# ctu-vras/pcl-augmentation

Hardware: NVIDIA B200
Metric: augmented scans/sec (120k-pt KITTI scan, placement + occlusion + insertion) (higher is better)
Workload: dtype f64

## Files before the change

### pcl_augmentation_b200/csrc/r3d_common.cuh

```cuda
#pragma once
#include <cuda_runtime.h>
#include <stdint.h>

#define R3D_EMPTY_U64 0xFFFFFFFFFFFFFFFFull
#define R3D_MAX_CLASSES 16
#define R3D_MAX_SURFACE 8
#define R3D_NUM_RADII 50

namespace r3d {

constexpr double kPi = 3.141592653589793;
constexpr double kTwoPi = 6.283185307179586;
constexpr double kEmptyRange = 500.0;

__device__ __forceinline__ double mul(double a, double b) { return __dmul_rn(a, b); }
__device__ __forceinline__ double add(double a, double b) { return __dadd_rn(a, b); }
__device__ __forceinline__ double sub(double a, double b) { return __dsub_rn(a, b); }

__device__ __forceinline__ double range3(double x, double y, double z) {
    return sqrt(add(add(mul(x, x), mul(y, y)), mul(z, z)));
}
__device__ __forceinline__ double azimuth(double x, double y) { return add(atan2(y, x), kPi); }
__device__ __forceinline__ double elevation(double z, double r) { return acos(__ddiv_rn(z, r)); }

__device__ __forceinline__ double az_mod(double az) { return az >= kTwoPi ? sub(az, kTwoPi) : az; }

struct ImageGeom {
    int rows, cols;
    int pix_stride;
    double min_el, max_el;
    double d_el, d_az;
};

__host__ __device__ __forceinline__ ImageGeom make_geom(int rows, int cols, int pix_stride, double max_el, double min_el) {
    ImageGeom g;
    g.rows = rows; g.cols = cols; g.pix_stride = pix_stride;
    g.min_el = min_el; g.max_el = max_el;
    g.d_el = (max_el - min_el) / (double)rows;
    g.d_az = kTwoPi / (double)cols;
    return g;
}

__device__ __forceinline__ int trunc_to_int(double v) {
    if (!(v > -2147483000.0 && v < 2147483000.0)) return INT_MIN;
    return (int)v;
}
__device__ __forceinline__ int bin_row(const ImageGeom& g, double el) {
    return trunc_to_int(__ddiv_rn(sub(sub(el, g.min_el), 0.00001), g.d_el));
}
__device__ __forceinline__ int bin_col(const ImageGeom& g, double az) {
    return trunc_to_int(__ddiv_rn(az_mod(az), g.d_az));
}

struct FastGeom { float inv_d_az, inv_d_el, el0, err_az, err_el; };
__device__ __forceinline__ FastGeom make_fast_geom(const ImageGeom& g) {
    FastGeom f;
    f.inv_d_az = (float)(1.0 / g.d_az); f.inv_d_el = (float)(1.0 / g.d_el);
    f.el0 = (float)(g.min_el + 0.00001);
    f.err_az = 6e-6f * f.inv_d_az + 5e-7f * (float)g.cols + 1e-5f;
    f.err_el = 6e-6f * f.inv_d_el + 5e-7f * (float)g.rows + 1e-5f;
    if (!(f.err_az < 0.25f)) f.err_az = 2.0f;
    if (!(f.err_el < 0.25f)) f.err_el = 2.0f;
    return f;
}
__device__ __forceinline__ bool fast_bin(float t, float err, int nbins, int& bin) {
    const float f = floorf(t), fr = t - f;
    if (!(fr > err && fr < 1.0f - err && t > err && t < (float)nbins - err)) return false;
    bin = (int)f;
    return true;
}
__device__ __forceinline__ bool fast_col(float inv_d_az, float err_az, int cols, float x, float y, int& col) {
    return fast_bin((atan2f(y, x) + 3.14159274f) * inv_d_az, err_az, cols, col);
}
__device__ __forceinline__ bool fast_row(const FastGeom& f, int rows, float z, float r, int& row) {
    const float t = z / r;
    if (!(fabsf(t) <= 0.9f)) return false;
    return fast_bin((acosf(t) - f.el0) * f.inv_d_el, f.err_el, rows, row);
}

struct Box {
    double cx, cy, cz;
    double m[9];
    double length, width, height;
    double reach;
};

struct BoxTest {
    double c0x, c0y, c0z, hi0, lo0;
    double c1x, c1y, c1z, hi1, lo1;
    double c2x, c2y, c2z, hi2, lo2;
};

__device__ __forceinline__ BoxTest make_box_test(const Box& b) {
    BoxTest t;
    const double* m = b.m;
    t.c0x = m[0]; t.c0y = m[3]; t.c0z = m[6];
    t.c1x = m[1]; t.c1y = m[4]; t.c1z = m[7];
    t.c2x = m[2]; t.c2y = m[5]; t.c2z = m[8];
    const double L = b.length, W = b.width, H = b.height;
    t.hi0 = add(add(mul(t.c0x, add(b.cx, __ddiv_rn(mul(t.c0x, L), 2.0))), mul(t.c0y, add(b.cy, __ddiv_rn(mul(t.c0y, L), 2.0)))),
                mul(t.c0z, add(b.cz, __ddiv_rn(mul(t.c0z, L), 2.0))));
    t.lo0 = add(add(mul(t.c0x, sub(b.cx, __ddiv_rn(mul(t.c0x, L), 2.0))), mul(t.c0y, sub(b.cy, __ddiv_rn(mul(t.c0y, L), 2.0)))),
                mul(t.c0z, sub(b.cz, __ddiv_rn(mul(t.c0z, L), 2.0))));
    t.hi1 = add(add(mul(t.c1x, add(b.cx, __ddiv_rn(mul(t.c1x, W), 2.0))), mul(t.c1y, add(b.cy, __ddiv_rn(mul(t.c1y, W), 2.0)))),
                mul(t.c1z, add(b.cz, __ddiv_rn(mul(t.c1z, W), 2.0))));
    t.lo1 = add(add(mul(t.c1x, sub(b.cx, __ddiv_rn(mul(t.c1x, W), 2.0))), mul(t.c1y, sub(b.cy, __ddiv_rn(mul(t.c1y, W), 2.0)))),
                mul(t.c1z, sub(b.cz, __ddiv_rn(mul(t.c1z, W), 2.0))));
    t.hi2 = add(add(mul(t.c2x, add(b.cx, mul(t.c2x, H))), mul(t.c2y, add(b.cy, mul(t.c2y, H)))),
                mul(t.c2z, add(b.cz, mul(t.c2z, H))));
    t.lo2 = add(add(mul(t.c2x, sub(b.cx, mul(t.c2x, 0.0))), mul(t.c2y, sub(b.cy, mul(t.c2y, 0.0)))),
                mul(t.c2z, sub(b.cz, mul(t.c2z, 0.0))));
    return t;
}

__device__ __forceinline__ bool inside_box(const BoxTest& t, double x, double y, double z) {
    const double a0 = add(add(mul(t.c0x, x), mul(t.c0y, y)), mul(t.c0z, z));
    if (!(a0 < t.hi0) || !(a0 > t.lo0)) return false;
    const double a1 = add(add(mul(t.c1x, x), mul(t.c1y, y)), mul(t.c1z, z));
    if (!(a1 < t.hi1) || !(a1 > t.lo1)) return false;
    const double a2 = add(add(mul(t.c2x, x), mul(t.c2y, y)), mul(t.c2z, z));
    return (a2 < t.hi2) && (a2 > t.lo2);
}

struct YawBox {
    double cx, cy;
    double m00, m10;
    double m01;
};

__device__ __forceinline__ YawBox make_yaw_box(double c0x, double c0y, double a, double b, double c, double s) {
    YawBox y;
    y.cx = sub(mul(c, c0x), mul(s, c0y));
    y.cy = add(mul(s, c0x), mul(c, c0y));
    y.m00 = sub(mul(a, c), mul(b, s));
    y.m10 = add(mul(b, c), mul(a, s));
    y.m01 = -add(mul(a, s), mul(b, c));
    return y;
}

__device__ __forceinline__ Box yaw_box_to_box(const YawBox& y, double cz, double L, double W, double H) {
    Box b;
    b.cx = y.cx; b.cy = y.cy; b.cz = cz;
    b.m[0] = y.m00; b.m[1] = y.m01; b.m[2] = 0.0;
    b.m[3] = y.m10; b.m[4] = y.m00; b.m[5] = 0.0;
    b.m[6] = 0.0;   b.m[7] = 0.0;   b.m[8] = 1.0;
    b.length = L; b.width = W; b.height = H; b.reach = 0.0;
    return b;
}

__device__ __forceinline__ unsigned long long dbl_bits(double v) { return (unsigned long long)__double_as_longlong(v); }
__device__ __forceinline__ double bits_dbl(unsigned long long b) { return __longlong_as_double((long long)b); }

__device__ __forceinline__ float4 ldg_f4(const float4* p) { return __ldg(p); }

}
```

### pcl_augmentation_b200/csrc/r3d_engine.cu

```cuda
#include "r3d_engine_kernels.cuh"
#include "r3d_host.h"
#include "r3d_resident.h"

#include <cmath>
#include <chrono>
#include <cstdlib>
#include <thread>
#include <cstring>
#include <map>
#include <string>
#include <vector>

using namespace r3d;

#define R3D_MAX_SUB 16

namespace {

enum KernelId {
    KID_INGEST, KID_CTRL, KID_UPDATE, KID_CLEAR, KID_PROJECT, KID_CLOSEFILL, KID_ADJUST, KID_ONMAP, KID_HEIGHT, KID_COLLIDE,
    KID_GRID, KID_OCCL, KID_SELECT, KID_OUT, KID_MINMAX, KID_PROJECT0, KID_CLOSEFILL0, KID_CLEAR0, KID_MINMAX0, KID_WALK, KID_PREP, KID_SCATTER,
    KID_COUNT
};
const char* kKernelNames[KID_COUNT] = {
    "ingest_spherical", "ctrl", "update_mask_patch", "clear_images", "project_zbuffer", "close_fill", "adjust_map",
    "onmap", "road_level", "collide", "index_build", "occlusion_count", "select_emit", "compact_output", "minmax_elevation",
    "project_zbuffer_full", "close_fill_full", "clear_images_full", "minmax_elevation_full",
    "scan_walk", "walk_prepare",
    "scatter_project"};

template <class T>
struct DevBuf {
    T* p = nullptr;
    size_t n = 0;
    int alloc(size_t count) {
        release();
        n = count;
        if (count == 0) return R3D_OK;
        cudaError_t err = cudaMalloc((void**)&p, count * sizeof(T));
        if (err != cudaSuccess) { p = nullptr; return r3d_fail_cuda(err, "cudaMalloc"); }
        return R3D_OK;
    }
    void release() { if (p) cudaFree(p); p = nullptr; n = 0; }
    ~DevBuf() { release(); }
};

}

struct r3d_engine {
    r3d_engine_cfg cfg;
    EngineDev dev;
    cudaStream_t stream = nullptr;
    int n_scans = 0;
    int max_n0 = 0;
    int n_sms = 148;
    int device = 0;
    int n_sub = 4;
    cudaStream_t sub_stream[R3D_MAX_SUB] = {nullptr};
    cudaEvent_t sub_done[R3D_MAX_SUB] = {nullptr};
    cudaEvent_t ev_armed = nullptr;
    cudaEvent_t ev_wait = nullptr;
    struct Sub { int b0, n, round; bool done; long long left; unsigned seq_base; EngineDev d; cudaStream_t st; };
    Sub sub[R3D_MAX_SUB];
    struct RoundGraph { cudaGraphExec_t exec = nullptr; EngineDev d; int ns = 0, chunks_all = 0, task_ctas = 0, sel_pts = 0, kernels = 0; };
    RoundGraph round_graph[R3D_MAX_SUB];
    bool use_graphs = true, capturing = false;
    bool fresh = false;
    bool walked = false;
    bool staged = false;
    bool run_active = false;
    int run_nsub = 0, run_done = 0, run_rounds = 0;
    bool objects_set = false, yaw_set = false, batch_loaded = false, ran = false;
    int last_rounds = 0;
    DevBuf<float4> xyzi, out_xyzi, gpts, apts;
    DevBuf<unsigned long long> sel_keys;
    DevBuf<double> sel_r, tail_x, tail_y, tail_z, r, el, smooth, poses, obj_x, obj_y, obj_z, cos_k, sin_k, radii_sq, cand_level,
        inserted_box;
    DevBuf<float> tail_i, obj_i, check, out_check;
    DevBuf<unsigned> label, dmask, vmask, occ_win, unplaceable, obj_label, out_label, tickets;
    DevBuf<unsigned short> col, cand_list, label16, out_label16;
    DevBuf<unsigned char> label1;
    DevBuf<long long> pt_off;
    DevBuf<int> chunk_cnt, pix, gate_update, gate_try, gate_apply, gate_full, gate_patch, cf_rect, col_off, col_idx, acell, active_count, far_arr, od_map_dims, counts, perms, class_list_off,
        class_list, radii_ok, cand_v, gcell, n_list, feas, occ_pix, sel_pix, inserted, n0_arr, nbox0_arr, work_cnt, full_list, cf_tasks, need2, occ_far;
    DevBuf<unsigned> occ_cnt;
    DevBuf<unsigned> round_ctl;
    DevBuf<unsigned char> alive, od_maps, ss_map, cand_flags, gnear, gscratch;
    DevBuf<unsigned long long> zraw, obj_raw, stats;
    DevBuf<long long> od_map_off, out_count, out_off, check_off;
    DevBuf<ScanState> st;
    DevBuf<Box> boxes, boxes0;
    DevBuf<BoxTest> box_tests;
    DevBuf<ObjBox> obj, try_obj;
    DevBuf<ClassCfg> classes;
    CUtensorMap zraw_tmap;
    bool zraw_tmap_ok = false;
    std::vector<Box> h_boxes;
    std::vector<int> h_nbox0;
    unsigned long long* h_words = nullptr;
    unsigned long long* d_words = nullptr;
    unsigned seq = 0;
    long long* h_offsets = nullptr;
    SchedulePolicy policy;
    bool policy_set = false;
    int* h_idx = nullptr;
    cudaEvent_t ev_idx = nullptr;
    DevBuf<int> idx_dev, n_ins_dev;
    DevBuf<float> box7;
    bool from_store = false;
    std::vector<int> batch_idx;
    r3d_world_aug world_pol;
    bool world_on = false, world_loaded = false;
    DevBuf<float> world;
    DevBuf<float> obj_dims3;
    DevBuf<int> class_target;
    const int* kept_src = nullptr;
    std::vector<int> kept;
    bool profile = false;
    double prof_ms[KID_COUNT] = {0};
    int64_t prof_launches[KID_COUNT] = {0};
    std::vector<std::pair<int, std::pair<cudaEvent_t, cudaEvent_t>>> pending_events;
    std::vector<cudaEvent_t> event_pool;
};

namespace {

__global__ void k_box_tests(const Box* boxes, BoxTest* tests, int n) {
    const int i = blockIdx.x * blockDim.x + threadIdx.x;
    if (i < n) tests[i] = make_box_test(boxes[i]);
}
__global__ void k_widen_labels(const unsigned short* src, const long long* pt_off, unsigned* label, int P, int n_scans) {
    const int b = blockIdx.y;
    if (b >= n_scans) return;
    const long long o = pt_off[b] - pt_off[0];
    const int cnt = (int)(pt_off[b + 1] - pt_off[b]);
    const int p0 = blockIdx.x * CHUNK;
    for (int p = p0 + threadIdx.x; p < min(p0 + CHUNK, cnt); p += blockDim.x) label[(size_t)b * P + p] = src[o + p];
}
__global__ void k_expand_label_bits(const unsigned char* bits, const long long* pt_off, unsigned* label, int P, int n_scans,
                                    unsigned road_label) {
    const int b = blockIdx.y;
    if (b >= n_scans) return;
    const long long o = pt_off[b] - pt_off[0];
    const int cnt = (int)(pt_off[b + 1] - pt_off[b]);
    const int p0 = blockIdx.x * CHUNK;
    const unsigned other = road_label == 1u ? 2u : 1u;
    for (int p = p0 + threadIdx.x; p < min(p0 + CHUNK, cnt); p += blockDim.x) {
        const long long i = o + p;
        label[(size_t)b * P + p] = ((bits[i >> 3] >> (i & 7)) & 1u) ? road_label : other;
    }
}
__global__ void k_narrow_labels(const unsigned* src, unsigned short* dst, long long n) {
    for (long long i = blockIdx.x * (long long)blockDim.x + threadIdx.x; i < n; i += (long long)gridDim.x * blockDim.x) dst[i] = (unsigned short)src[i];
}
__global__ void k_set_round(unsigned* round_ctl, unsigned seq_base) { round_ctl[0] = 0u; round_ctl[1] = seq_base; }
__global__ void k_fill_u64(unsigned long long* p, size_t n, unsigned long long v) {
    for (size_t i = blockIdx.x * (size_t)blockDim.x + threadIdx.x; i < n; i += (size_t)gridDim.x * blockDim.x) p[i] = v;
}

struct Launcher {
    r3d_engine* eng;
    int kid;
    cudaStream_t st;
    cudaEvent_t a = nullptr, b = nullptr;
    Launcher(r3d_engine* e, int k, cudaStream_t stream = nullptr) : eng(e), kid(k), st(stream ? stream : e->stream) {
        if (eng->profile) {
            a = get_event(); b = get_event();
            cudaEventRecord(a, st);
        }
    }
    cudaEvent_t get_event() {
        if (!eng->event_pool.empty()) { cudaEvent_t ev = eng->event_pool.back(); eng->event_pool.pop_back(); return ev; }
        cudaEvent_t ev; cudaEventCreate(&ev); return ev;
    }
    ~Launcher() {
        if (eng->capturing) return;
        r3d_count_launch();
        eng->prof_launches[kid] += 1;
        if (eng->profile) {
            cudaEventRecord(b, st);
            eng->pending_events.push_back({kid, {a, b}});
        }
    }
};

void drain_events(r3d_engine* eng) {
    for (auto& pe : eng->pending_events) {
        float ms = 0.f;
        cudaEventSynchronize(pe.second.second);
        cudaEventElapsedTime(&ms, pe.second.first, pe.second.second);
        eng->prof_ms[pe.first] += ms;
        eng->event_pool.push_back(pe.second.first);
        eng->event_pool.push_back(pe.second.second);
    }
    eng->pending_events.clear();
}

size_t occl_smem_bytes(const EngineDev& d) { return (size_t)d.dwords * sizeof(unsigned) + (size_t)(d.K + 2) * sizeof(unsigned short); }
constexpr int SEL_SMEM_PTS = 4096;
int next_pow2(int v) { int p = 1; while (p < v) p <<= 1; return p; }
size_t select_smem_bytes(int max_pts) {
    return (size_t)next_pow2(max_pts) * 8 + (size_t)max_pts * 8 + (size_t)SEL_TILE_PX * 8 + (size_t)max_pts * 4 +
           2 * (size_t)(SEL_TILE_PX / 32) * 4 + 16;
}

}

#define TRY(x) do { int _rc = (x); if (_rc != R3D_OK) return _rc; } while (0)

static cudaError_t engine_wait(r3d_engine* eng) {
    if (!eng->ev_wait) {
        cudaError_t e = cudaEventCreateWithFlags(&eng->ev_wait, cudaEventBlockingSync | cudaEventDisableTiming);
        if (e != cudaSuccess) return e;
    }
    cudaError_t e = cudaEventRecord(eng->ev_wait, eng->stream);
    if (e != cudaSuccess) return e;
    return cudaEventSynchronize(eng->ev_wait);
}

typedef CUresult (*EncodeTiledFn)(CUtensorMap*, CUtensorMapDataType, cuuint32_t, void*, const cuuint64_t*, const cuuint64_t*,
                                  const cuuint32_t*, const cuuint32_t*, CUtensorMapInterleave, CUtensorMapSwizzle,
                                  CUtensorMapL2promotion, CUtensorMapFloatOOBfill);
static bool make_zraw_tensor_map(CUtensorMap* tm, void* base, int W, int H, int B) {
    if (getenv("R3D_NO_TMA") || (W & 1) || ((uintptr_t)base & 15)) return false;
    void* fn = nullptr;
    cudaDriverEntryPointQueryResult q;
    if (cudaGetDriverEntryPoint("cuTensorMapEncodeTiled", &fn, cudaEnableDefault, &q) != cudaSuccess || q != cudaDriverEntryPointSuccess || !fn) {
        cudaGetLastError();
        return false;
    }
    const cuuint64_t dims[3] = {(cuuint64_t)W, (cuuint64_t)H, (cuuint64_t)B};
    const cuuint64_t strides[2] = {(cuuint64_t)W * 8, (cuuint64_t)W * H * 8};
    const cuuint32_t box[3] = {(cuuint32_t)CF_SW, (cuuint32_t)CF_SH, 1u};
    const cuuint32_t estr[3] = {1u, 1u, 1u};
    return ((EncodeTiledFn)fn)(tm, CU_TENSOR_MAP_DATA_TYPE_UINT64, 3, base, dims, strides, box, estr, CU_TENSOR_MAP_INTERLEAVE_NONE,
                               CU_TENSOR_MAP_SWIZZLE_NONE, CU_TENSOR_MAP_L2_PROMOTION_NONE, CU_TENSOR_MAP_FLOAT_OOB_FILL_NONE) == CUDA_SUCCESS;
}

extern "C" int r3d_engine_create(const r3d_engine_cfg* cfg, r3d_engine** out) {
    if (!cfg || !out) return r3d_fail(R3D_ERR_ARG, "r3d_engine_create: null argument");
    if (cfg->rows <= 0 || cfg->cols <= 0 || cfg->cols > 65535 || cfg->yaw_steps <= 0 || cfg->n_classes <= 0 ||
        cfg->n_classes > R3D_MAX_CLASSES || cfg->max_scans <= 0 || cfg->max_points <= 0 || cfg->max_inserted <= 0 ||
        cfg->max_tries <= 0 || cfg->max_events <= 0 || cfg->max_boxes <= 0 || (cfg->task != 0 && cfg->task != 1))
        return r3d_fail(R3D_ERR_ARG, "r3d_engine_create: bad configuration");
    if (cfg->task == 1 && (cfg->map_window <= 0 || cfg->map_window % 32 != 0))
        return r3d_fail(R3D_ERR_ARG, "r3d_engine_create: map_window must be a positive multiple of 32");
    int count = 0;
    if (cudaGetDeviceCount(&count) != cudaSuccess || count == 0)
        return r3d_fail(R3D_ERR_CUDA, "r3d_engine_create: no CUDA device (this library has no CPU fallback)");
    r3d_engine* eng = new r3d_engine();
    eng->cfg = *cfg;
    R3D_CUDA(cudaGetDevice(&eng->device));
    int prio_least = 0, prio_greatest = 0;
    R3D_CUDA(cudaDeviceGetStreamPriorityRange(&prio_least, &prio_greatest));
    R3D_CUDA(cudaStreamCreateWithPriority(&eng->stream, cudaStreamNonBlocking, prio_least));
    eng->n_sub = (cfg->flags >> 8) & 31;
    eng->use_graphs = !(cfg->flags & 2);
    eng->staged = (cfg->flags & 8) != 0;
    if (const char* env = getenv("R3D_STAGED")) eng->staged = atoi(env) != 0;
    if (const char* env = getenv("R3D_GRAPHS")) eng->use_graphs = atoi(env) != 0;
    if (const char* env = getenv("R3D_SUBBATCHES")) eng->n_sub = atoi(env);
    if (eng->n_sub <= 0) eng->n_sub = 4;
    eng->n_sub = std::min(eng->n_sub, R3D_MAX_SUB);
    for (int i = 0; i < R3D_MAX_SUB; ++i) {
        R3D_CUDA(cudaStreamCreateWithPriority(&eng->sub_stream[i], cudaStreamNonBlocking, prio_greatest));
        R3D_CUDA(cudaEventCreateWithFlags(&eng->sub_done[i], cudaEventDisableTiming));
    }
    R3D_CUDA(cudaEventCreateWithFlags(&eng->ev_armed, cudaEventDisableTiming));
    EngineDev& d = eng->dev;
    memset(&d, 0, sizeof(d));
    d.task = cfg->task; d.rows = cfg->rows; d.cols = cfg->cols; d.hw = cfg->rows * cfg->cols; d.K = cfg->yaw_steps;
    d.max_tries = cfg->max_tries; d.n_classes = cfg->n_classes; d.B = cfg->max_scans; d.max_points = cfg->max_points;
    d.max_inserted = cfg->max_inserted + (16 - (cfg->max_points + cfg->max_inserted) % 16) % 16;
    d.P = cfg->max_points + d.max_inserted; d.max_boxes = cfg->max_boxes;
    d.max_events = cfg->max_events; d.road_label = cfg->road_label; d.n_road_indexes = cfg->n_road_indexes;
    d.map_window = cfg->task == 1 ? cfg->map_window : 32; d.dwords = (d.hw + 31) / 32;
    for (int i = 0; i < R3D_MAX_SURFACE; ++i) d.road_indexes[i] = cfg->road_indexes[i];
    d.step_rad = 2.0 * 3.14159265358979323846 / (double)cfg->yaw_steps;
    d.grid_cell = cfg->grid_cell > 0 ? cfg->grid_cell : 0.5;
    d.grid_inv_cell = (float)(1.0 / d.grid_cell);
    d.G = 2 * (cfg->grid_half > 0 ? cfg->grid_half : 200);
    d.force_full = (cfg->flags & 1) ? 1 : 0;
    const size_t B = d.B, P = d.P, K1 = d.K + 1, HW = d.hw;
    TRY(eng->xyzi.alloc(B * d.max_points)); TRY(eng->tail_x.alloc(B * d.max_inserted)); TRY(eng->tail_y.alloc(B * d.max_inserted));
    TRY(eng->tail_z.alloc(B * d.max_inserted)); TRY(eng->tail_i.alloc(B * d.max_inserted)); TRY(eng->label.alloc(B * P));
    TRY(eng->r.alloc(B * P)); TRY(eng->el.alloc(B * P)); TRY(eng->col.alloc(B * P)); TRY(eng->pix.alloc(B * P));
    TRY(eng->alive.alloc(B * P)); TRY(eng->zraw.alloc(B * HW)); TRY(eng->obj_raw.alloc(B * HW)); TRY(eng->smooth.alloc(B * HW));
    eng->zraw_tmap_ok = make_zraw_tensor_map(&eng->zraw_tmap, eng->zraw.p, d.cols, d.rows, (int)B);
    TRY(eng->dmask.alloc(B * d.dwords)); TRY(eng->vmask.alloc(B * d.dwords)); TRY(eng->st.alloc(B));
    TRY(eng->gate_update.alloc(B)); TRY(eng->gate_try.alloc(B)); TRY(eng->gate_apply.alloc(B)); TRY(eng->gate_full.alloc(B));
    TRY(eng->gate_patch.alloc(B)); TRY(eng->cf_rect.alloc(B * 4)); TRY(eng->active_count.alloc(R3D_MAX_SUB * 64 * 2));
    TRY(eng->round_ctl.alloc(R3D_MAX_SUB * 32));
    d.cf_tiles_x = (d.cols + CF_TW - 1) / CF_TW;
    d.cf_tiles = d.cf_tiles_x * ((d.rows + CF_TH - 1) / CF_TH);
    TRY(eng->work_cnt.alloc(B * 4)); TRY(eng->full_list.alloc(B)); TRY(eng->cf_tasks.alloc(B * (size_t)d.cf_tiles));
    R3D_CUDA(cudaMemset(eng->work_cnt.p, 0, B * 4 * sizeof(int)));
    TRY(eng->need2.alloc(B));
    R3D_CUDA(cudaMemset(eng->need2.p, 0, B * sizeof(int)));
    d.cand_window = (cfg->flags & 4) ? 0 : 48;
    if (const char* env = getenv("R3D_WINDOW")) d.cand_window = std::max(0, atoi(env));
    if (d.task != 0) d.cand_window = 0;
    TRY(eng->far_arr.alloc(B)); TRY(eng->boxes.alloc(B * d.max_boxes)); TRY(eng->box_tests.alloc(B * d.max_boxes));
    TRY(eng->boxes0.alloc(B * d.max_boxes));
    TRY(eng->poses.alloc(B * 16)); TRY(eng->occ_win.alloc(B * ((size_t)d.map_window * d.map_window / 32)));
    TRY(eng->counts.alloc(B * d.n_classes)); TRY(eng->cos_k.alloc(K1)); TRY(eng->sin_k.alloc(K1));
    TRY(eng->radii_sq.alloc(R3D_NUM_RADII)); TRY(eng->radii_ok.alloc(R3D_NUM_RADII)); TRY(eng->classes.alloc(R3D_MAX_CLASSES));
    TRY(eng->cand_flags.alloc(B * K1)); TRY(eng->cand_level.alloc(B * K1)); TRY(eng->cand_v.alloc(B * K1));
    TRY(eng->cand_list.alloc(B * K1)); TRY(eng->n_list.alloc(B)); TRY(eng->tickets.alloc(B * 4));
    R3D_CUDA(cudaMemset(eng->tickets.p, 0, B * 4 * sizeof(unsigned)));
    TRY(eng->feas.alloc(B * d.K)); TRY(eng->inserted.alloc(B * d.max_events * 4)); TRY(eng->inserted_box.alloc(B * d.max_events * 8));
    TRY(eng->check.alloc(B * d.max_inserted * 5)); TRY(eng->out_count.alloc(B)); TRY(eng->out_off.alloc(B + 1));
    TRY(eng->check_off.alloc(B + 1)); TRY(eng->out_xyzi.alloc(B * P)); TRY(eng->out_label.alloc(B * P));
    TRY(eng->out_check.alloc(B * d.max_inserted * 5)); TRY(eng->n0_arr.alloc(B)); TRY(eng->nbox0_arr.alloc(B));
    TRY(eng->gcell.alloc(B * (size_t)d.G * d.G)); TRY(eng->gpts.alloc(B * d.max_points));
    TRY(eng->gnear.alloc(B * (size_t)d.G * d.G)); TRY(eng->gscratch.alloc(B * (size_t)d.G * d.G));
    TRY(eng->col_off.alloc(B * (size_t)(d.cols + 1))); TRY(eng->col_idx.alloc(B * d.max_points));
    TRY(eng->acell.alloc(B * (size_t)d.G * d.G)); TRY(eng->apts.alloc(B * d.max_points));
    TRY(eng->try_obj.alloc(B));
    d.max_chunks = (d.P + CHUNK - 1) / CHUNK;
    TRY(eng->chunk_cnt.alloc(B * (size_t)d.max_chunks));
    { int dev = 0; cudaGetDevice(&dev); cudaDeviceGetAttribute(&eng->n_sms, cudaDevAttrMultiProcessorCount, dev); }
    TRY(eng->od_map_off.alloc(B * 2 + 1)); TRY(eng->od_map_dims.alloc(B * 8)); TRY(eng->stats.alloc(R3D_N_STATS));
    R3D_CUDA(cudaMemset(eng->stats.p, 0, R3D_N_STATS * sizeof(unsigned long long)));
    TRY(eng->occ_far.alloc(B * (OCC_FAR_CAP + 1)));
    if (cfg->task == 1) TRY(eng->occ_cnt.alloc(B * (size_t)d.map_window * d.map_window));
    R3D_CUDA(cudaMemset(eng->occ_far.p, 0xFF, B * (OCC_FAR_CAP + 1) * sizeof(int)));
    R3D_CUDA(cudaHostAlloc((void**)&eng->h_words, R3D_MAX_SUB * 64 * sizeof(unsigned long long), cudaHostAllocMapped));
    memset(eng->h_words, 0, R3D_MAX_SUB * 64 * sizeof(unsigned long long));
    R3D_CUDA(cudaHostGetDevicePointer((void**)&eng->d_words, eng->h_words, 0));
    R3D_CUDA(cudaMallocHost((void**)&eng->h_offsets, (2 * (B + 1) + 1) * sizeof(long long)));
    std::vector<ClassCfg> cls(R3D_MAX_CLASSES);
    for (int c = 0; c < R3D_MAX_CLASSES; ++c) {
        const r3d_class_cfg& s = cfg->classes[c];
        cls[c].min_points = s.min_points; cls[c].map_sel = s.map_sel; cls[c].map_ok_mask = s.map_ok_mask;
        cls[c].pedestrian = s.pedestrian; cls[c].n_surface = std::min(std::max(s.n_surface, 0), R3D_MAX_SURFACE);
        for (int i = 0; i < R3D_MAX_SURFACE; ++i) cls[c].surface[i] = s.surface[i];
        cls[c].ok_slots = 0u;
    }
    d.n_surf_all = 0;
    for (int c = 0; c < cfg->n_classes; ++c)
        for (int i = 0; i < cls[c].n_surface; ++i) {
            int slot = -1;
            for (int j = 0; j < d.n_surf_all; ++j) if (d.surf_all[j] == cls[c].surface[i]) slot = j;
            if (slot < 0) {
                if (d.n_surf_all >= 15) return r3d_fail(R3D_ERR_CAPACITY, "r3d_engine_create: more than 15 distinct surface labels");
                slot = d.n_surf_all; d.surf_all[d.n_surf_all++] = cls[c].surface[i];
            }
            cls[c].ok_slots |= 1u << slot;
        }
    if (d.max_points + d.max_inserted > (1 << APT_IDX_BITS)) return r3d_fail(R3D_ERR_CAPACITY, "r3d_engine_create: more than 2^27 points per scan");
    R3D_CUDA(cudaMemcpy(eng->classes.p, cls.data(), cls.size() * sizeof(ClassCfg), cudaMemcpyHostToDevice));
    R3D_CUDA(cudaMemcpy(eng->radii_sq.p, cfg->radii_sq, sizeof(cfg->radii_sq), cudaMemcpyHostToDevice));
    R3D_CUDA(cudaMemcpy(eng->radii_ok.p, cfg->radii_ok, sizeof(cfg->radii_ok), cudaMemcpyHostToDevice));
    k_fill_u64<<<148 * 4, 256, 0, eng->stream>>>(eng->obj_raw.p, B * HW, R3D_EMPTY_U64); r3d_count_launch();
    R3D_CUDA(cudaMemsetAsync(eng->dmask.p, 0, B * d.dwords * sizeof(unsigned), eng->stream));
    R3D_CUDA(cudaStreamSynchronize(eng->stream));
    d.xyzi = eng->xyzi.p; d.tail_x = eng->tail_x.p; d.tail_y = eng->tail_y.p; d.tail_z = eng->tail_z.p; d.tail_i = eng->tail_i.p;
    d.label = eng->label.p; d.r = eng->r.p; d.el = eng->el.p; d.col = eng->col.p; d.pix = eng->pix.p; d.alive = eng->alive.p;
    d.zraw = eng->zraw.p; d.obj_raw = eng->obj_raw.p; d.smooth = eng->smooth.p; d.dmask = eng->dmask.p; d.vmask = eng->vmask.p;
    d.st = eng->st.p; d.gate_update = eng->gate_update.p; d.gate_try = eng->gate_try.p; d.gate_apply = eng->gate_apply.p;
    d.gate_full = eng->gate_full.p; d.gate_patch = eng->gate_patch.p; d.cf_rect = eng->cf_rect.p;
    d.work_cnt = eng->work_cnt.p; d.full_list = eng->full_list.p; d.cf_tasks = eng->cf_tasks.p; d.need2 = eng->need2.p;
    d.active_count = eng->active_count.p; d.far_arr = eng->far_arr.p; d.boxes = eng->boxes.p; d.box_tests = eng->box_tests.p;
    d.poses = eng->poses.p; d.occ_win = eng->occ_win.p; d.counts = eng->counts.p; d.cos_k = eng->cos_k.p; d.sin_k = eng->sin_k.p;
    d.radii_sq = eng->radii_sq.p; d.radii_ok = eng->radii_ok.p; d.classes = eng->classes.p; d.cand_flags = eng->cand_flags.p;
    d.cand_level = eng->cand_level.p; d.cand_list = eng->cand_list.p; d.n_list = eng->n_list.p; d.tickets = eng->tickets.p;
    d.cand_v = eng->cand_v.p; d.feas = eng->feas.p; d.inserted = eng->inserted.p; d.inserted_box = eng->inserted_box.p;
    d.check = eng->check.p; d.out_count = eng->out_count.p; d.out_off = eng->out_off.p; d.check_off = eng->check_off.p;
    d.out_xyzi = eng->out_xyzi.p; d.out_label = eng->out_label.p; d.out_check = eng->out_check.p;
    d.gcell = eng->gcell.p; d.gpts = eng->gpts.p; d.gnear = eng->gnear.p; d.gscratch = eng->gscratch.p;
    d.col_off = eng->col_off.p; d.col_idx = eng->col_idx.p; d.acell = eng->acell.p; d.apts = eng->apts.p;
    d.try_obj = eng->try_obj.p; d.chunk_cnt = eng->chunk_cnt.p;
    d.od_map_off = eng->od_map_off.p; d.od_map_dims = eng->od_map_dims.p; d.stats = eng->stats.p; d.occ_far = eng->occ_far.p; d.occ_cnt = eng->occ_cnt.p;
    *out = eng;
    return R3D_OK;
}

extern "C" int r3d_engine_destroy(r3d_engine* eng) {
    if (eng) cudaSetDevice(eng->device);
    if (!eng) return R3D_OK;
    cudaStreamSynchronize(eng->stream);
    drain_events(eng);
    for (cudaEvent_t ev : eng->event_pool) cudaEventDestroy(ev);
    if (eng->h_words) cudaFreeHost(eng->h_words);
    if (eng->h_offsets) cudaFreeHost(eng->h_offsets);
    for (int i = 0; i < R3D_MAX_SUB; ++i) {
        if (eng->sub_stream[i]) { cudaStreamSynchronize(eng->sub_stream[i]); cudaStreamDestroy(eng->sub_stream[i]); }
        if (eng->sub_done[i]) cudaEventDestroy(eng->sub_done[i]);
    }
    if (eng->ev_armed) cudaEventDestroy(eng->ev_armed);
    if (eng->ev_wait) cudaEventDestroy(eng->ev_wait);
    if (eng->ev_idx) cudaEventDestroy(eng->ev_idx);
    if (eng->h_idx) cudaFreeHost(eng->h_idx);
    for (int i = 0; i < R3D_MAX_SUB; ++i) if (eng->round_graph[i].exec) cudaGraphExecDestroy(eng->round_graph[i].exec);
    cudaStreamDestroy(eng->stream);
    delete eng;
    return R3D_OK;
}

extern "C" int r3d_engine_set_yaw_tables(r3d_engine* eng, const double* cos_k, const double* sin_k) {
    if (eng) cudaSetDevice(eng->device);
    if (!eng || !cos_k || !sin_k) return r3d_fail(R3D_ERR_ARG, "r3d_engine_set_yaw_tables: null argument");
    const size_t n = (size_t)eng->dev.K + 1;
    R3D_CUDA(cudaMemcpy(eng->cos_k.p, cos_k, n * sizeof(double), cudaMemcpyHostToDevice));
    R3D_CUDA(cudaMemcpy(eng->sin_k.p, sin_k, n * sizeof(double), cudaMemcpyHostToDevice));
    eng->yaw_set = true;
    return R3D_OK;
}

extern "C" int r3d_engine_set_objects(r3d_engine* eng, const r3d_object_db* db) {
    if (eng) cudaSetDevice(eng->device);
    if (!eng || !db || db->n_objects <= 0) return r3d_fail(R3D_ERR_ARG, "r3d_engine_set_objects: bad argument");
    EngineDev& d = eng->dev;
    const int n = db->n_objects;
    const int64_t total = db->point_offsets[n];
    std::vector<double> x(total), y(total), z(total);
    std::vector<float> in(total);
    std::vector<unsigned> lab(total);
    for (int64_t i = 0; i < total; ++i) {
        const double* p = db->points5 + i * 5;
        x[i] = p[0]; y[i] = p[1]; z[i] = p[2]; in[i] = (float)p[3]; lab[i] = (unsigned)p[4];
    }
    std::vector<ObjBox> ob(n);
    int max_pts = 1;
    for (int o = 0; o < n; ++o) {
        const double* bx = db->boxes + (size_t)o * 8;
        ObjBox& t = ob[o];
        t.cx = bx[0]; t.cy = bx[1]; t.cz = bx[2]; t.a = bx[3]; t.b = bx[4];
        t.length = bx[5]; t.width = bx[6]; t.height = bx[7];
        t.rho = std::hypot(t.cx, t.cy); t.psi0 = std::atan2(t.cy, t.cx);
        t.reach = 0.5 * std::hypot(t.length, t.width) + 0.05;
        t.cls = db->class_index[o];
        t.first = (int)db->point_offsets[o]; t.count = (int)(db->point_offsets[o + 1] - db->point_offsets[o]);
        t.pad = 0;
        t.eu0 = t.ev0 = t.ez0 = 1e300; t.eu1 = t.ev1 = t.ez1 = -1e300;
        for (int i = t.first; i < t.first + t.count; ++i) {
            const double dx = x[i] - t.cx, dy = y[i] - t.cy;
            const double u = dx * t.a + dy * t.b, v = -dx * t.b + dy * t.a, w = z[i] - t.cz;
            t.eu0 = std::min(t.eu0, u); t.eu1 = std::max(t.eu1, u); t.ev0 = std::min(t.ev0, v); t.ev1 = std::max(t.ev1, v);
            t.ez0 = std::min(t.ez0, w); t.ez1 = std::max(t.ez1, w);
        }
        t.eu0 -= 1e-6; t.ev0 -= 1e-6; t.ez0 -= 1e-6; t.eu1 += 1e-6; t.ev1 += 1e-6; t.ez1 += 1e-6;
        if (t.cls < 0 || t.cls >= d.n_classes) return r3d_fail(R3D_ERR_ARG, "r3d_engine_set_objects: class index out of range");
        max_pts = std::max(max_pts, t.count);
    }
    if (max_pts > 32768) return r3d_fail(R3D_ERR_CAPACITY, "r3d_engine_set_objects: a cut object has more than 32768 points");
    d.max_obj_points = max_pts; d.n_objects = n;
    TRY(eng->obj_x.alloc(total)); TRY(eng->obj_y.alloc(total)); TRY(eng->obj_z.alloc(total)); TRY(eng->obj_i.alloc(total));
    TRY(eng->obj_label.alloc(total)); TRY(eng->obj.alloc(n)); TRY(eng->class_list_off.alloc(d.n_classes + 1));
    const int nl = db->class_list_offsets[d.n_classes];
    TRY(eng->class_list.alloc(std::max(nl, 1)));
    TRY(eng->unplaceable.alloc((size_t)d.B * ((n + 31) / 32)));
    TRY(eng->occ_pix.alloc((size_t)d.B * OCC_G * max_pts)); TRY(eng->sel_pix.alloc((size_t)d.B * max_pts));
    R3D_CUDA(cudaMemcpy(eng->obj_x.p, x.data(), total * sizeof(double), cudaMemcpyHostToDevice));
    R3D_CUDA(cudaMemcpy(eng->obj_y.p, y.data(), total * sizeof(double), cudaMemcpyHostToDevice));
    R3D_CUDA(cudaMemcpy(eng->obj_z.p, z.data(), total * sizeof(double), cudaMemcpyHostToDevice));
    R3D_CUDA(cudaMemcpy(eng->obj_i.p, in.data(), total * sizeof(float), cudaMemcpyHostToDevice));
    R3D_CUDA(cudaMemcpy(eng->obj_label.p, lab.data(), total * sizeof(unsigned), cudaMemcpyHostToDevice));
    R3D_CUDA(cudaMemcpy(eng->obj.p, ob.data(), n * sizeof(ObjBox), cudaMemcpyHostToDevice));
    R3D_CUDA(cudaMemcpy(eng->class_list_off.p, db->class_list_offsets, (d.n_classes + 1) * sizeof(int), cudaMemcpyHostToDevice));
    R3D_CUDA(cudaMemcpy(eng->class_list.p, db->class_list, nl * sizeof(int), cudaMemcpyHostToDevice));
    d.obj_x = eng->obj_x.p; d.obj_y = eng->obj_y.p; d.obj_z = eng->obj_z.p; d.obj_i = eng->obj_i.p; d.obj_label = eng->obj_label.p;
    d.obj = eng->obj.p; d.class_list_off = eng->class_list_off.p; d.class_list = eng->class_list.p;
    d.unplaceable = eng->unplaceable.p; d.occ_pix = eng->occ_pix.p; d.sel_pix = eng->sel_pix.p;
    const size_t sel_smem = select_smem_bytes(std::min(max_pts, SEL_SMEM_PTS));
    d.sel_key_cap = next_pow2(max_pts);
    if (max_pts > std::min(SEL_SMEM_PTS, walk_od::WALK_SEL_PTS)) {
        TRY(eng->sel_keys.alloc((size_t)d.B * d.sel_key_cap)); TRY(eng->sel_r.alloc((size_t)d.B * max_pts));
    }
    d.sel_keys = eng->sel_keys.p; d.sel_r = eng->sel_r.p;
    R3D_CUDA(cudaFuncSetAttribute(k_select_emit, cudaFuncAttributeMaxDynamicSharedMemorySize, (int)sel_smem));
    R3D_CUDA(cudaFuncSetAttribute(k_occl_count, cudaFuncAttributeMaxDynamicSharedMemorySize, (int)occl_smem_bytes(d)));
    if (onmap_smem_bytes(d.K) > 100 * 1024) return r3d_fail(R3D_ERR_CAPACITY, "r3d_engine_set_objects: too many yaw steps for the placement kernel's shared memory");
    R3D_CUDA(cudaFuncSetAttribute(k_onmap, cudaFuncAttributeMaxDynamicSharedMemorySize, (int)onmap_smem_bytes(d.K)));
    if (grid_near_smem(d.G) > 200 * 1024) return r3d_fail(R3D_ERR_CAPACITY, "r3d_engine_set_objects: road-level grid too large for shared memory");
    R3D_CUDA(cudaFuncSetAttribute(k_grid_near_bits, cudaFuncAttributeMaxDynamicSharedMemorySize, (int)grid_near_smem(d.G)));
    if (std::max(walk_od::walk_smem_layout(d.K, d.dwords).total, walk_ss::walk_smem_layout(d.K, d.dwords).total) > 200 * 1024)
        return r3d_fail(R3D_ERR_CAPACITY, "r3d_engine_set_objects: range image / yaw steps too large for the walker's shared memory");
    R3D_CUDA(cudaFuncSetAttribute(walk_od::k_scan_walk, cudaFuncAttributeMaxDynamicSharedMemorySize, (int)walk_od::walk_smem_layout(d.K, d.dwords).total));
    R3D_CUDA(cudaFuncSetAttribute(walk_ss::k_scan_walk, cudaFuncAttributeMaxDynamicSharedMemorySize, (int)walk_ss::walk_smem_layout(d.K, d.dwords).total));
    eng->objects_set = true;
    return R3D_OK;
}

extern "C" int r3d_engine_set_ss_map(r3d_engine* eng, const uint8_t* map, int32_t size_x, int32_t size_y, int64_t move_x,
                                     int64_t move_y) {
    if (eng) cudaSetDevice(eng->device);
    if (!eng || !map || size_x <= 0 || size_y <= 0) return r3d_fail(R3D_ERR_ARG, "r3d_engine_set_ss_map: bad argument");
    TRY(eng->ss_map.alloc((size_t)size_x * size_y));
    R3D_CUDA(cudaMemcpy(eng->ss_map.p, map, (size_t)size_x * size_y, cudaMemcpyHostToDevice));
    eng->dev.ss_map = eng->ss_map.p; eng->dev.ss_sx = size_x; eng->dev.ss_sy = size_y;
    eng->dev.ss_move_x = move_x; eng->dev.ss_move_y = move_y;
    return R3D_OK;
}

static int arm_batch(r3d_engine* eng, bool ingest) {
    eng->run_active = false;
    EngineDev& d = eng->dev;
    const int n = eng->n_scans;
    cudaStream_t st = eng->stream;
    k_reset_state<<<(n + 127) / 128, 128, 0, st>>>(d, n, eng->n0_arr.p, eng->nbox0_arr.p); r3d_count_launch();
    R3D_CUDA(cudaMemsetAsync(eng->dmask.p, 0, (size_t)n * d.dwords * sizeof(unsigned), st));
    const int chunks = (eng->max_n0 + CHUNK - 1) / CHUNK;
    if (ingest) {
        R3D_CUDA(cudaMemsetAsync(eng->gcell.p, 0, (size_t)n * d.G * d.G * sizeof(int), st));
        R3D_CUDA(cudaMemsetAsync(eng->col_off.p, 0, (size_t)n * (d.cols + 1) * sizeof(int), st));
        R3D_CUDA(cudaMemsetAsync(eng->acell.p, 0, (size_t)n * d.G * d.G * sizeof(int), st));
        { Launcher l(eng, KID_INGEST); k_ingest_count<<<dim3(chunks, n), STREAM_THREADS, 0, st>>>(d, n); }
        {
            Launcher l(eng, KID_GRID);
            k_bucket_scan3<<<dim3(n, 3), 1024, 0, st>>>(d, n);
        }
        { Launcher l(eng, KID_SCATTER); k_scatter_project<<<dim3(chunks, n), STREAM_THREADS, 0, st>>>(d, n); }
        {
            Launcher l(eng, KID_GRID);
            k_grid_near_bits<<<n, NEAR_THREADS, grid_near_smem(d.G), st>>>(d, n);
        }
        eng->fresh = true;
    } else {
        eng->fresh = false;
        k_reset_alive<<<dim3(std::max(chunks, 1), n), 256, 0, st>>>(d, n); r3d_count_launch();
        const size_t slots = (size_t)n * d.max_boxes;
        R3D_CUDA(cudaMemcpyAsync(eng->boxes.p, eng->boxes0.p, slots * sizeof(Box), cudaMemcpyDeviceToDevice, st));
        k_box_tests<<<(int)((slots + 127) / 128), 128, 0, st>>>(eng->boxes.p, eng->box_tests.p, (int)slots);
        r3d_count_launch();
    }
    eng->ran = false;
    return r3d_check_launch("arm_batch");
}

extern "C" int r3d_engine_load_batch(r3d_engine* eng, const r3d_batch* bt) {
    if (eng) cudaSetDevice(eng->device);
    if (!eng || !bt) return r3d_fail(R3D_ERR_ARG, "r3d_engine_load_batch: null argument");
    if (!eng->objects_set || !eng->yaw_set) return r3d_fail(R3D_ERR_ARG, "r3d_engine_load_batch: set objects and yaw tables first");
    EngineDev& d = eng->dev;
    const int n = bt->n_scans;
    if (n <= 0 || n > d.B) return r3d_fail(R3D_ERR_CAPACITY, "r3d_engine_load_batch: n_scans exceeds max_scans");
    if (!bt->point_offsets || !bt->xyzi || (!bt->labels && !bt->labels16 && !bt->labels1) || !bt->counts || !bt->perms || bt->n_events <= 0)
        return r3d_fail(R3D_ERR_ARG, "r3d_engine_load_batch: missing arrays");
    if (d.task == 1 && (!bt->poses || !d.ss_map)) return r3d_fail(R3D_ERR_ARG, "r3d_engine_load_batch: semseg needs poses and the map");
    if (d.task == 0 && (!bt->maps || !bt->map_offsets || !bt->map_dims)) return r3d_fail(R3D_ERR_ARG, "r3d_engine_load_batch: OD needs maps");
    cudaStream_t st = eng->stream;
    std::vector<int> n0(n), nb(n);
    eng->max_n0 = 0;
    for (int s = 0; s < n; ++s) {
        const int64_t cnt = bt->point_offsets[s + 1] - bt->point_offsets[s];
        if (cnt <= 0 || cnt > d.max_points) return r3d_fail(R3D_ERR_CAPACITY, "r3d_engine_load_batch: scan larger than max_points (or empty)");
        n0[s] = (int)cnt; eng->max_n0 = std::max(eng->max_n0, (int)cnt);
        nb[s] = bt->box_offsets ? bt->box_offsets[s + 1] - bt->box_offsets[s] : 0;
        if (nb[s] > d.max_boxes) return r3d_fail(R3D_ERR_CAPACITY, "r3d_engine_load_batch: too many scene boxes");
    }
    eng->n_scans = n;
    eng->h_boxes.assign((size_t)n * d.max_boxes, Box());
    for (int s = 0; s < n; ++s)
        for (int j = 0; j < nb[s]; ++j) {
            const double* src = bt->boxes + ((size_t)bt->box_offsets[s] + j) * R3D_BOX_DOUBLES;
            Box& b = eng->h_boxes[(size_t)s * d.max_boxes + j];
            b.cx = src[0]; b.cy = src[1]; b.cz = src[2];
            for (int i = 0; i < 9; ++i) b.m[i] = src[3 + i];
            b.length = src[12]; b.width = src[13]; b.height = src[14]; b.reach = src[15];
        }
    eng->h_nbox0 = nb;
    R3D_CUDA(cudaMemcpyAsync(eng->boxes.p, eng->h_boxes.data(), eng->h_boxes.size() * sizeof(Box), cudaMemcpyHostToDevice, st));
    R3D_CUDA(cudaMemcpyAsync(eng->boxes0.p, eng->boxes.p, eng->h_boxes.size() * sizeof(Box), cudaMemcpyDeviceToDevice, st));
    k_box_tests<<<(int)((eng->h_boxes.size() + 127) / 128), 128, 0, st>>>(eng->boxes.p, eng->box_tests.p, (int)eng->h_boxes.size());
    r3d_count_launch();
    R3D_CUDA(cudaMemcpyAsync(eng->n0_arr.p, n0.data(), n * sizeof(int), cudaMemcpyHostToDevice, st));
    R3D_CUDA(cudaMemcpyAsync(eng->nbox0_arr.p, nb.data(), n * sizeof(int), cudaMemcpyHostToDevice, st));
    if (d.task == 0) {
        const int64_t bytes = bt->map_offsets[(size_t)n * 2];
        if ((size_t)bytes > eng->od_maps.n) TRY(eng->od_maps.alloc((size_t)bytes));
        R3D_CUDA(cudaMemcpyAsync(eng->od_maps.p, bt->maps, (size_t)bytes, cudaMemcpyHostToDevice, st));
        R3D_CUDA(cudaMemcpyAsync(eng->od_map_off.p, bt->map_offsets, ((size_t)n * 2 + 1) * sizeof(long long), cudaMemcpyHostToDevice, st));
        R3D_CUDA(cudaMemcpyAsync(eng->od_map_dims.p, bt->map_dims, (size_t)n * 8 * sizeof(int), cudaMemcpyHostToDevice, st));
        d.od_maps = eng->od_maps.p;
    } else {
        R3D_CUDA(cudaMemcpyAsync(eng->poses.p, bt->poses, (size_t)n * 16 * sizeof(double), cudaMemcpyHostToDevice, st));
    }
    for (int sc = 0; sc < n; ++sc) {
        long long want = 0;
        for (int c = 0; c < d.n_classes; ++c) want += std::max(bt->counts[(size_t)sc * d.n_classes + c], 0);
        if (want + 1 > d.max_events)
            return r3d_fail(R3D_ERR_CAPACITY, "r3d_engine_load_batch: a scan's schedule asks for more objects than max_events - 1 "
                                              "(create the engine with max_events = objects per scan + 1)");
    }
    R3D_CUDA(cudaMemcpyAsync(eng->counts.p, bt->counts, (size_t)n * d.n_classes * sizeof(int), cudaMemcpyHostToDevice, st));
    const size_t nperm = (size_t)n * bt->n_events * d.n_classes * d.max_tries;
    if (nperm > eng->perms.n) TRY(eng->perms.alloc(nperm));
    R3D_CUDA(cudaMemcpyAsync(eng->perms.p, bt->perms, nperm * sizeof(int), cudaMemcpyHostToDevice, st));
    d.perms = eng->perms.p; d.n_perm_events = bt->n_events;
    bool uniform = true;
    for (int s = 1; s < n; ++s) uniform &= n0[s] == n0[0];
    const bool packed = bt->labels == nullptr;
    const bool bits = packed && bt->labels16 == nullptr;
    if (bits && (d.task != 0 || bt->point_offsets[0] != 0))
        return r3d_fail(R3D_ERR_ARG, "r3d_engine_load_batch: labels1 (one Road bit per point) is for object detection batches that start at point 0");
    if (packed) {
        const size_t total = (size_t)(bt->point_offsets[n] - bt->point_offsets[0]);
        if ((size_t)n + 1 > eng->pt_off.n) TRY(eng->pt_off.alloc((size_t)d.B + 1));
        if (bits) {
            const size_t nbytes = (total + 7) / 8;
            if (nbytes > eng->label1.n) TRY(eng->label1.alloc(nbytes));
            R3D_CUDA(cudaMemcpyAsync(eng->label1.p, bt->labels1, nbytes, cudaMemcpyHostToDevice, st));
        } else {
            if (total > eng->label16.n) TRY(eng->label16.alloc(total));
            R3D_CUDA(cudaMemcpyAsync(eng->label16.p, bt->labels16 + bt->point_offsets[0], total * sizeof(unsigned short), cudaMemcpyHostToDevice, st));
        }
        R3D_CUDA(cudaMemcpyAsync(eng->pt_off.p, bt->point_offsets, ((size_t)n + 1) * sizeof(long long), cudaMemcpyHostToDevice, st));
    }
    if (uniform) {
        R3D_CUDA(cudaMemcpy2DAsync(eng->xyzi.p, (size_t)d.max_points * sizeof(float4), bt->xyzi + bt->point_offsets[0] * 4,
                                   (size_t)n0[0] * sizeof(float4), (size_t)n0[0] * sizeof(float4), n, cudaMemcpyHostToDevice, st));
        if (!packed)
            R3D_CUDA(cudaMemcpy2DAsync(eng->label.p, (size_t)d.P * sizeof(unsigned), bt->labels + bt->point_offsets[0],
                                       (size_t)n0[0] * sizeof(unsigned), (size_t)n0[0] * sizeof(unsigned), n, cudaMemcpyHostToDevice, st));
    } else {
        for (int s = 0; s < n; ++s) {
            const int64_t o = bt->point_offsets[s];
            R3D_CUDA(cudaMemcpyAsync(eng->xyzi.p + (size_t)s * d.max_points, bt->xyzi + o * 4, (size_t)n0[s] * sizeof(float4), cudaMemcpyHostToDevice, st));
            if (!packed)
                R3D_CUDA(cudaMemcpyAsync(eng->label.p + (size_t)s * d.P, bt->labels + o, (size_t)n0[s] * sizeof(unsigned), cudaMemcpyHostToDevice, st));
        }
    }
    if (packed) {
        const int chunks = (eng->max_n0 + CHUNK - 1) / CHUNK;
        if (bits) k_expand_label_bits<<<dim3(chunks, n), STREAM_THREADS, 0, st>>>(eng->label1.p, eng->pt_off.p, eng->label.p, d.P, n, (unsigned)d.road_label);
        else k_widen_labels<<<dim3(chunks, n), STREAM_THREADS, 0, st>>>(eng->label16.p, eng->pt_off.p, eng->label.p, d.P, n);
        r3d_count_launch();
    }
    eng->batch_loaded = true;
    eng->from_store = false;
    eng->world_loaded = false;
    d.world = nullptr;
    return arm_batch(eng, true);
}

extern "C" int r3d_engine_set_schedule_policy(r3d_engine* eng, int32_t random, int32_t number_of_object, const int32_t* fixed_counts) {
    if (eng) cudaSetDevice(eng->device);
    if (!eng || (random && number_of_object < 0) || (!random && !fixed_counts))
        return r3d_fail(R3D_ERR_ARG, "r3d_engine_set_schedule_policy: bad argument");
    SchedulePolicy p;
    memset(&p, 0, sizeof(p));
    p.random = random ? 1 : 0;
    p.number_of_object = random ? number_of_object : 0;
    for (int c = 0; !random && c < eng->dev.n_classes; ++c) {
        if (fixed_counts[c] < 0) return r3d_fail(R3D_ERR_ARG, "r3d_engine_set_schedule_policy: negative class count");
        p.fixed[c] = fixed_counts[c];
    }
    eng->policy = p;
    eng->policy_set = true;
    return R3D_OK;
}

extern "C" int r3d_engine_load_resident(r3d_engine* eng, const r3d_resident_store* s, const int32_t* indices, int32_t n,
                                        uint64_t seed, uint64_t epoch) {
    if (eng) cudaSetDevice(eng->device);
    if (!eng || !s || !indices) return r3d_fail(R3D_ERR_ARG, "r3d_engine_load_resident: null argument");
    if (!eng->objects_set || !eng->yaw_set) return r3d_fail(R3D_ERR_ARG, "r3d_engine_load_resident: set objects and yaw tables first");
    if (!eng->policy_set) return r3d_fail(R3D_ERR_ARG, "r3d_engine_load_resident: set the schedule policy first");
    EngineDev& d = eng->dev;
    if (n <= 0 || n > d.B) return r3d_fail(R3D_ERR_CAPACITY, "r3d_engine_load_resident: n_scans exceeds max_scans");
    if (s->n_scans <= 0 || !s->xyzi || ((uintptr_t)s->xyzi & 15) || !s->labels || !s->point_offsets || !s->box_offsets ||
        !s->h_point_offsets || !s->h_box_offsets || (!s->boxes && s->h_box_offsets[s->n_scans] > 0))
        return r3d_fail(R3D_ERR_ARG, "r3d_engine_load_resident: missing store arrays");
    if (d.task == 1 && (!s->poses || !d.ss_map)) return r3d_fail(R3D_ERR_ARG, "r3d_engine_load_resident: semseg needs poses and the map");
    if (d.task == 0 && (!s->maps || !s->map_offsets || !s->map_dims)) return r3d_fail(R3D_ERR_ARG, "r3d_engine_load_resident: OD needs maps");
    std::vector<int> nb(n);
    int max_n0 = 0;
    for (int b = 0; b < n; ++b) {
        const int i = indices[b];
        if (i < 0 || i >= s->n_scans) return r3d_fail(R3D_ERR_ARG, "r3d_engine_load_resident: index out of range");
        const int64_t cnt = s->h_point_offsets[i + 1] - s->h_point_offsets[i];
        if (cnt <= 0 || cnt > d.max_points) return r3d_fail(R3D_ERR_CAPACITY, "r3d_engine_load_resident: scan larger than max_points (or empty)");
        max_n0 = std::max(max_n0, (int)cnt);
        nb[b] = s->h_box_offsets[i + 1] - s->h_box_offsets[i];
        if (nb[b] > d.max_boxes) return r3d_fail(R3D_ERR_CAPACITY, "r3d_engine_load_resident: too many scene boxes");
    }
    long long want = eng->policy.number_of_object;
    if (!eng->policy.random) { want = 0; for (int c = 0; c < d.n_classes; ++c) want += eng->policy.fixed[c]; }
    if (want + 1 > d.max_events)
        return r3d_fail(R3D_ERR_CAPACITY, "r3d_engine_load_resident: a scan's schedule asks for more objects than max_events - 1 "
                                          "(create the engine with max_events = objects per scan + 1)");
    const size_t nperm = (size_t)d.B * d.max_events * d.n_classes * d.max_tries;
    if (nperm > eng->perms.n) TRY(eng->perms.alloc(nperm));
    if (!eng->h_idx) {
        R3D_CUDA(cudaMallocHost((void**)&eng->h_idx, (size_t)d.B * sizeof(int)));
        R3D_CUDA(cudaEventCreateWithFlags(&eng->ev_idx, cudaEventDisableTiming));
        TRY(eng->idx_dev.alloc(d.B));
    }
    if (eng->world_on && !eng->world.p) TRY(eng->world.alloc((size_t)d.B * 8));
    cudaStream_t st = eng->stream;
    R3D_CUDA(cudaEventSynchronize(eng->ev_idx));
    memcpy(eng->h_idx, indices, (size_t)n * sizeof(int));
    R3D_CUDA(cudaMemcpyAsync(eng->idx_dev.p, eng->h_idx, (size_t)n * sizeof(int), cudaMemcpyHostToDevice, st));
    R3D_CUDA(cudaEventRecord(eng->ev_idx, st));
    eng->n_scans = n;
    eng->max_n0 = max_n0;
    eng->h_nbox0 = nb;
    const int* idx = eng->idx_dev.p;
    const int od = d.task == 0;
    launch_gather_points(*s, idx, n, max_n0, eng->xyzi.p, d.max_points, eng->label.p, d.P, od, (unsigned)d.road_label, st);
    launch_gather_meta(*s, idx, n, od, eng->n0_arr.p, eng->nbox0_arr.p, eng->od_map_off.p, eng->od_map_dims.p, eng->poses.p,
                       eng->boxes.p, eng->boxes0.p, d.max_boxes, st);
    const int slots = n * d.max_boxes;
    k_box_tests<<<(slots + 127) / 128, 128, 0, st>>>(eng->boxes.p, eng->box_tests.p, slots);
    r3d_count_launch();
    if (od) d.od_maps = s->maps;
    d.perms = eng->perms.p; d.n_perm_events = d.max_events;
    launch_draw_schedule(idx, n, d.max_events, d.n_classes, d.max_tries, d.class_list_off, eng->policy, seed, epoch, eng->counts.p,
                         eng->perms.p, st);
    if (eng->world_on) launch_draw_world(idx, n, eng->world_pol, seed, epoch, eng->world.p, st);
    d.world = eng->world_on ? eng->world.p : nullptr;
    eng->world_loaded = eng->world_on;
    eng->from_store = true;
    eng->batch_idx.assign(indices, indices + n);
    TRY(r3d_check_launch("r3d_engine_load_resident"));
    eng->batch_loaded = true;
    return arm_batch(eng, true);
}

extern "C" int r3d_engine_set_ss_map_device(r3d_engine* eng, const uint8_t* map, int32_t size_x, int32_t size_y, int64_t move_x,
                                            int64_t move_y) {
    if (eng) cudaSetDevice(eng->device);
    if (!eng || !map || size_x <= 0 || size_y <= 0) return r3d_fail(R3D_ERR_ARG, "r3d_engine_set_ss_map_device: bad argument");
    eng->dev.ss_map = map; eng->dev.ss_sx = size_x; eng->dev.ss_sy = size_y;
    eng->dev.ss_move_x = move_x; eng->dev.ss_move_y = move_y;
    return R3D_OK;
}

extern "C" int r3d_engine_schedule_read(r3d_engine* eng, int32_t* counts, int32_t* perms, int32_t* n_events) {
    if (eng) cudaSetDevice(eng->device);
    if (!eng || !counts || !n_events || !eng->batch_loaded) return r3d_fail(R3D_ERR_ARG, "r3d_engine_schedule_read: bad argument or no batch");
    const EngineDev& d = eng->dev;
    R3D_CUDA(engine_wait(eng));
    const size_t n = (size_t)eng->n_scans;
    R3D_CUDA(cudaMemcpy(counts, d.counts, n * d.n_classes * sizeof(int), cudaMemcpyDeviceToHost));
    if (perms) R3D_CUDA(cudaMemcpy(perms, d.perms, n * d.n_perm_events * d.n_classes * d.max_tries * sizeof(int), cudaMemcpyDeviceToHost));
    *n_events = d.n_perm_events;
    return R3D_OK;
}

extern "C" int r3d_engine_reset_batch(r3d_engine* eng) {
    if (eng) cudaSetDevice(eng->device);
    if (!eng || !eng->batch_loaded) return r3d_fail(R3D_ERR_ARG, "r3d_engine_reset_batch: no batch loaded");
    return arm_batch(eng, false);
}

extern "C" int r3d_engine_rearm_batch(r3d_engine* eng, int from_raw_points) {
    if (eng) cudaSetDevice(eng->device);
    if (!eng || !eng->batch_loaded) return r3d_fail(R3D_ERR_ARG, "r3d_engine_rearm_batch: no batch loaded");
    if (!from_raw_points) return arm_batch(eng, false);
    const size_t slots = (size_t)eng->n_scans * eng->dev.max_boxes;
    R3D_CUDA(cudaMemcpyAsync(eng->boxes.p, eng->boxes0.p, slots * sizeof(Box), cudaMemcpyDeviceToDevice, eng->stream));
    k_box_tests<<<(int)((slots + 127) / 128), 128, 0, eng->stream>>>(eng->boxes.p, eng->box_tests.p, (int)slots);
    r3d_count_launch();
    return arm_batch(eng, true);
}

static EngineDev sub_view(const EngineDev& d, int b0) {
    if (b0 == 0) return d;
    EngineDev v = d;
    const size_t b = (size_t)b0;
    const size_t gg = (size_t)d.G * d.G, k1 = (size_t)d.K + 1, ww = (size_t)d.map_window * d.map_window / 32;
#define R3D_OFF(field, stride) if (d.field) v.field = d.field + b * (size_t)(stride)
    R3D_OFF(gcell, gg); R3D_OFF(gpts, d.max_points); R3D_OFF(gnear, gg); R3D_OFF(gscratch, gg); R3D_OFF(acell, gg); R3D_OFF(apts, d.max_points);
    R3D_OFF(xyzi, d.max_points); R3D_OFF(tail_x, d.max_inserted); R3D_OFF(tail_y, d.max_inserted);
    R3D_OFF(tail_z, d.max_inserted); R3D_OFF(tail_i, d.max_inserted); R3D_OFF(label, d.P); R3D_OFF(r, d.P); R3D_OFF(el, d.P);
    R3D_OFF(col, d.P); R3D_OFF(pix, d.P); R3D_OFF(alive, d.P); R3D_OFF(zraw, d.hw); R3D_OFF(obj_raw, d.hw);
    R3D_OFF(smooth, d.hw); R3D_OFF(dmask, d.dwords); R3D_OFF(vmask, d.dwords); R3D_OFF(st, 1); R3D_OFF(gate_update, 1);
    R3D_OFF(gate_try, 1); R3D_OFF(gate_apply, 1); R3D_OFF(gate_full, 1); R3D_OFF(gate_patch, 1); R3D_OFF(cf_rect, 4);
    R3D_OFF(work_cnt, 4); R3D_OFF(full_list, 1); R3D_OFF(cf_tasks, d.cf_tiles); R3D_OFF(need2, 1);
    R3D_OFF(col_off, d.cols + 1); R3D_OFF(col_idx, d.max_points); R3D_OFF(far_arr, 1); R3D_OFF(boxes, d.max_boxes);
    R3D_OFF(box_tests, d.max_boxes); R3D_OFF(od_map_off, 2); R3D_OFF(od_map_dims, 8); R3D_OFF(poses, 16); R3D_OFF(occ_win, ww);
    R3D_OFF(counts, d.n_classes); R3D_OFF(perms, (size_t)d.n_perm_events * d.n_classes * d.max_tries);
    R3D_OFF(unplaceable, (d.n_objects + 31) / 32); R3D_OFF(try_obj, 1); R3D_OFF(cand_flags, k1); R3D_OFF(cand_level, k1);
    R3D_OFF(cand_v, k1); R3D_OFF(cand_list, k1); R3D_OFF(n_list, 1); R3D_OFF(tickets, 4); R3D_OFF(feas, d.K);
    R3D_OFF(occ_pix, (size_t)OCC_G * d.max_obj_points); R3D_OFF(sel_pix, d.max_obj_points);
    R3D_OFF(sel_keys, d.sel_key_cap); R3D_OFF(sel_r, d.max_obj_points); R3D_OFF(inserted, (size_t)d.max_events * 4);
    R3D_OFF(inserted_box, (size_t)d.max_events * 8); R3D_OFF(check, (size_t)d.max_inserted * 5); R3D_OFF(chunk_cnt, d.max_chunks);
    R3D_OFF(out_count, 1); R3D_OFF(occ_far, OCC_FAR_CAP + 1); R3D_OFF(occ_cnt, (size_t)d.map_window * d.map_window);
#undef R3D_OFF
    return v;
}

extern "C" int r3d_engine_run_until(r3d_engine* eng, int stop_at, int* still_running);

extern "C" int r3d_engine_run(r3d_engine* eng) { return r3d_engine_run_until(eng, 0, nullptr); }

static int run_walker(r3d_engine* eng) {
    const EngineDev& d = eng->dev;
    const int n = eng->n_scans;
    cudaStream_t st = eng->stream;
    const int chunks0 = (eng->max_n0 + CHUNK - 1) / CHUNK;
    const int chunks_all = (eng->max_n0 + d.max_inserted + CHUNK - 1) / CHUNK;
#ifndef R3D_FULL_Y
#define R3D_FULL_Y 32
#endif
    const int full_y = std::min(n, R3D_FULL_Y);
    const bool fresh = eng->fresh;
    eng->fresh = false;
    { Launcher l(eng, KID_PREP); walk_od::k_walk_prepare<<<std::min((n * d.cf_tiles + 255) / 256, eng->n_sms * 4), 256, 0, st>>>(d, n, fresh ? 0 : 1); }
    if (!fresh) {
        { Launcher l(eng, KID_MINMAX0); k_minmax<<<dim3(chunks0, full_y), STREAM_THREADS, 0, st>>>(d, n); }
        { Launcher l(eng, KID_CLEAR0); k_clear_images<<<dim3(32, full_y), STREAM_THREADS, 0, st>>>(d, n); }
        { Launcher l(eng, KID_PROJECT0); k_project<<<dim3(chunks0, full_y), STREAM_THREADS, 0, st>>>(d, n); }
    }
    {
        Launcher l(eng, KID_CLOSEFILL0);
        const int cf_grid = std::min(n * d.cf_tiles, eng->n_sms * 4);
        if (eng->zraw_tmap_ok) {
            k_close_fill_tma<<<cf_grid, CF_THREADS, 0, st>>>(eng->zraw_tmap, d.rows, d.cols, (int64_t)d.hw, d.smooth, d.far_arr, d.cf_tasks,
                                                              d.work_cnt + 1);
        } else if ((d.cols & 1) == 0 && ((uintptr_t)d.zraw & 15) == 0) {
            k_close_fill_raw_pipelined<<<cf_grid, CF_THREADS, 0, st>>>(d.zraw, d.rows, d.cols, (int64_t)d.hw, d.smooth, d.far_arr, d.cf_tasks,
                                                                        d.work_cnt + 1);
        } else {
            RawImage in{d.zraw};
            k_close_fill_tasks<RawImage><<<cf_grid, CF_THREADS, 0, st>>>(in, d.rows, d.cols, (int64_t)d.hw, d.smooth, d.far_arr, d.cf_tasks,
                                                                         d.work_cnt + 1);
        }
    }
    if (d.task == 1) {
        R3D_CUDA(cudaMemsetAsync(eng->occ_win.p, 0, (size_t)n * ((size_t)d.map_window * d.map_window / 32) * sizeof(unsigned), st));
        R3D_CUDA(cudaMemsetAsync(eng->occ_cnt.p, 0, (size_t)n * (size_t)d.map_window * d.map_window * sizeof(unsigned), st));
        Launcher l(eng, KID_ADJUST); k_adjust_map<<<dim3(chunks0, n), STREAM_THREADS, 0, st>>>(d, n, 1);
    }
    {
        Launcher l(eng, KID_WALK);
        if (d.task == 1) walk_ss::k_scan_walk<<<n, walk_ss::WALK_THREADS, walk_ss::walk_smem_layout(d.K, d.dwords).total, st>>>(d, n);
        else walk_od::k_scan_walk<<<n, walk_od::WALK_THREADS, walk_od::walk_smem_layout(d.K, d.dwords).total, st>>>(d, n);
    }
    {
        Launcher l(eng, KID_OUT);
        k_out_count<<<dim3(chunks_all, n), STREAM_THREADS, 0, st>>>(d, n);
        k_out_offsets<<<1, 1024, 0, st>>>(d, n, chunks_all);
        if (d.world) k_out_write<true><<<dim3(chunks_all, n), STREAM_THREADS, 0, st>>>(d, n);
        else k_out_write<false><<<dim3(chunks_all, n), STREAM_THREADS, 0, st>>>(d, n);
        r3d_count_launch(2);
    }
    R3D_CUDA(cudaMemcpyAsync(eng->h_offsets, eng->out_off.p, (n + 1) * sizeof(long long), cudaMemcpyDeviceToHost, st));
    R3D_CUDA(cudaMemcpyAsync(eng->h_offsets + (d.B + 1), eng->check_off.p, (n + 1) * sizeof(long long), cudaMemcpyDeviceToHost, st));
    R3D_CUDA(cudaMemcpyAsync(eng->h_offsets + 2 * (d.B + 1), eng->stats.p + 8, sizeof(long long), cudaMemcpyDeviceToHost, st));
    eng->ran = true; eng->walked = true;
    return r3d_check_launch("r3d_engine_run");
}

extern "C" int r3d_engine_run_until(r3d_engine* eng, int stop_at, int* still_running) {
    if (eng) cudaSetDevice(eng->device);
    if (!eng || !eng->batch_loaded) return r3d_fail(R3D_ERR_ARG, "r3d_engine_run: no batch loaded");
    if (still_running) *still_running = 0;
    if (!eng->staged) return run_walker(eng);
    eng->walked = false;
    const EngineDev& d0 = eng->dev;
    const int n = eng->n_scans;
    cudaStream_t st = eng->stream;
    const int P_live = eng->max_n0 + d0.max_inserted;
    const int chunks_all = (P_live + CHUNK - 1) / CHUNK;
    const int sel_pts = std::min(d0.max_obj_points, SEL_SMEM_PTS);
    const size_t sel_smem = select_smem_bytes(sel_pts);
    const int key_cap = next_pow2(sel_pts);
    const size_t onmap_smem = onmap_smem_bytes(d0.K);
    const int max_rounds = d0.max_events * (3 * d0.max_tries + 2) + 8;
    typedef r3d_engine::Sub Sub;
    Sub* sub = eng->sub;
    if (!eng->run_active) {
        eng->run_nsub = std::max(1, std::min(eng->n_sub, n));
        eng->run_done = 0; eng->run_rounds = 0;
        R3D_CUDA(cudaEventRecord(eng->ev_armed, st));
        for (int i = 0; i < eng->run_nsub; ++i) {
            Sub& s = sub[i];
            s.b0 = (int)((long long)n * i / eng->run_nsub); s.n = (int)((long long)n * (i + 1) / eng->run_nsub) - s.b0;
            s.round = 0; s.done = false; s.left = s.n; s.d = sub_view(d0, s.b0); s.st = eng->sub_stream[i];
            s.d.active_count = eng->active_count.p + (size_t)i * 128;
            s.d.host_word = eng->d_words + (size_t)i * 64;
            s.d.round_ctl = eng->round_ctl.p + (size_t)i * 32;
            if (eng->seq > 0xF0000000u) eng->seq = 0;
            s.seq_base = eng->seq + 1; eng->seq += (unsigned)max_rounds + 8u;
            R3D_CUDA(cudaStreamWaitEvent(s.st, eng->ev_armed, 0));
            R3D_CUDA(cudaMemsetAsync(s.d.active_count, 0, 128 * sizeof(int), s.st));
            k_set_round<<<1, 1, 0, s.st>>>(s.d.round_ctl, s.seq_base); r3d_count_launch();
        }
        eng->run_active = true;
    }
    const int nsub = eng->run_nsub;
    int& n_done = eng->run_done;
    int& rounds_max = eng->run_rounds;
    const int task_ctas = std::max(eng->n_sms, eng->n_sms * TASK_CTAS_PER_SM / nsub);
    const int ahead = 3;
    auto poll_round = [&](int i, int round, long long& left) -> int {
        volatile unsigned long long* w = eng->h_words + (size_t)i * 64 + (round & 63);
        const unsigned long long v = *w;
        if ((unsigned)(v >> 32) == sub[i].seq_base + (unsigned)round) { left = (long long)(v & 0xffffffffull); return 1; }
        return 0;
    };
    auto launch_round = [&](const EngineDev& d, int ns, cudaStream_t ss, bool r0) {
        const size_t pref_smem = (size_t)(ns + 1) * sizeof(int);
#ifndef R3D_FULL_Y
#define R3D_FULL_Y 32
#endif
        const int full_y = std::min(ns, R3D_FULL_Y);
        const int cf_grid = std::min(ns * d.cf_tiles, eng->n_sms * 8);
        { Launcher l(eng, KID_CTRL, ss); k_ctrl<<<ns, 32, 0, ss>>>(d, ns); }
        { Launcher l(eng, KID_UPDATE, ss); k_update<<<dim3(UPDATE_G, ns), UPDATE_THREADS, 0, ss>>>(d, ns); }
        { Launcher l(eng, r0 ? KID_MINMAX0 : KID_MINMAX, ss); k_minmax<<<dim3(chunks_all, full_y), STREAM_THREADS, 0, ss>>>(d, ns); }
        { Launcher l(eng, r0 ? KID_CLEAR0 : KID_CLEAR, ss); k_clear_images<<<dim3(32, full_y), STREAM_THREADS, 0, ss>>>(d, ns); }
        { Launcher l(eng, r0 ? KID_PROJECT0 : KID_PROJECT, ss); k_project<<<dim3(chunks_all, full_y), STREAM_THREADS, 0, ss>>>(d, ns); }
        {
            Launcher l(eng, r0 ? KID_CLOSEFILL0 : KID_CLOSEFILL, ss);
            if ((d.cols & 1) == 0 && ((uintptr_t)d.zraw & 15) == 0) {
                k_close_fill_raw_pipelined<<<std::min(cf_grid, eng->n_sms * 4), CF_THREADS, 0, ss>>>(d.zraw, d.rows, d.cols, (int64_t)d.hw, d.smooth, d.far_arr,
                                                                           d.cf_tasks, d.work_cnt + 1);
            } else {
                RawImage in{d.zraw};
                k_close_fill_tasks<RawImage><<<cf_grid, CF_THREADS, 0, ss>>>(in, d.rows, d.cols, (int64_t)d.hw, d.smooth, d.far_arr,
                                                                             d.cf_tasks, d.work_cnt + 1);
            }
        }
        if (d.task == 1) { Launcher l(eng, KID_ADJUST, ss); k_adjust_map<<<dim3(chunks_all, ns), STREAM_THREADS, 0, ss>>>(d, ns); }
        { Launcher l(eng, KID_ONMAP, ss); k_onmap<<<ns, TRY_THREADS, onmap_smem, ss>>>(d, ns); }
        const int ph = d.cand_window > 0 ? 1 : 0;
// ... 457 lines not shown
```

### pcl_augmentation_b200/csrc/r3d_engine.cuh

```cuda
#pragma once
#include "r3d_common.cuh"
#include "../../include/real3d_b200.h"

namespace r3d {

enum : int { PH_INIT = 0, PH_AFTER_TRY = 1, PH_DONE = 2, PH_ERROR = 3 };
enum : unsigned { CF_ONMAP = 1u, CF_HOK = 2u };
constexpr int APT_IDX_BITS = 27;
constexpr unsigned APT_IDX_MASK = (1u << APT_IDX_BITS) - 1u, APT_SLOT_NONE = 15u;

struct ClassCfg {
    int min_points, map_sel;
    unsigned map_ok_mask;
    int pedestrian, n_surface;
    int surface[R3D_MAX_SURFACE];
    unsigned ok_slots;
};

struct ObjBox {
    double cx, cy, cz;
    double a, b;
    double length, width, height;
    double rho, psi0;
    double reach;
    double eu0, eu1, ev0, ev1, ez0, ez1;
    int cls, first, count, pad;
};

struct ScanState {
    int n0, n_tail, tail_before, n_boxes;
    int phase, status;
    int remaining[R3D_MAX_CLASSES];
    int inserted_class, timeout, start_idx, end_idx, s_idx, event;
    int cur_class, cur_obj;
    int try_active, need_project, apply_flag, dirty, scene_changed;
    int n_feasible, found_rank, chosen_rot, accepted, chosen_v;
    int n_inserted, n_check;
    int far_flag;
    int first, extreme_removed;
    int d_r0, d_r1, d_c0, d_c1;
    unsigned long long new_min_bits, new_max_bits;
    int win_x0, win_y0;
    unsigned long long min_el_bits, max_el_bits;
    ImageGeom geom;
    long long walk_cycles;
    int walk_tries, walk_pad;
};

struct EngineDev {
    int task, rows, cols, hw, K, max_tries, n_classes;
    int B, max_points, max_inserted, P, max_boxes, max_events, max_obj_points;
    int road_label, n_road_indexes, map_window, dwords, n_objects, n_perm_events;
    int road_indexes[R3D_MAX_SURFACE];
    int n_surf_all, surf_all[15];
    double step_rad;
    int G;
    float grid_inv_cell;
    double grid_cell;
    int* gcell;
    float4* gpts;
    unsigned char* gnear;
    unsigned char* gscratch;
    int* acell;
    float4* apts;
    const float4* xyzi;
    double *tail_x, *tail_y, *tail_z;
    float* tail_i;
    unsigned* label;
    double *r, *el;
    unsigned short* col;
    int* pix;
    unsigned char* alive;
    unsigned long long *zraw, *obj_raw;
    double* smooth;
    unsigned *dmask, *vmask;
    ScanState* st;
    int *gate_update, *gate_try, *gate_apply, *gate_full, *gate_patch;
    int* cf_rect;
    int cand_window;
    int* need2;
    int* work_cnt;
    int* full_list;
    int* cf_tasks;
    int cf_tiles, cf_tiles_x;
    int force_full;
    int *col_off, *col_idx;
    int* active_count;
    unsigned long long* host_word;
    unsigned* round_ctl;
    unsigned long long* stats;
    int* far_arr;
    Box* boxes;
    BoxTest* box_tests;
    const unsigned char* od_maps;
    const long long* od_map_off;
    const int* od_map_dims;
    const unsigned char* ss_map;
    int ss_sx, ss_sy;
    long long ss_move_x, ss_move_y;
    const double* poses;
    unsigned* occ_win;
    unsigned* occ_cnt;
    int* occ_far;
    const int* counts;
    const int* perms;
    unsigned* unplaceable;
    const ObjBox* obj;
    ObjBox* try_obj;
    const double *obj_x, *obj_y, *obj_z;
    const float* obj_i;
    const unsigned* obj_label;
    const int* class_list_off;
    const int* class_list;
    const double *cos_k, *sin_k;
    const double* radii_sq;
    const int* radii_ok;
    const ClassCfg* classes;
    unsigned char* cand_flags;
    double* cand_level;
    int* cand_v;
    unsigned short* cand_list;
    int* n_list;
    unsigned* tickets;
    int* feas;
    int* occ_pix;
    int* sel_pix;
    unsigned long long* sel_keys;
    double* sel_r;
    int sel_key_cap;
    int* inserted;
    double* inserted_box;
    float* check;
    int* chunk_cnt;
    int max_chunks;
    long long* out_count;
    long long* out_off;
    long long* check_off;
    float4* out_xyzi;
    unsigned* out_label;
    float* out_check;
    const float* world;
};

struct WorldXf { bool fx, fy; float c, s, k; };
__device__ __forceinline__ WorldXf world_xf(const float* w) {
    return WorldXf{w[0] != 0.f, w[1] != 0.f, w[3], w[4], w[5]};
}
__device__ __forceinline__ void world_point(const WorldXf& t, float& x, float& y, float& z) {
    const float x1 = t.fy ? -x : x, y1 = t.fx ? -y : y;
    x = __fmul_rn(__fsub_rn(__fmul_rn(t.c, x1), __fmul_rn(t.s, y1)), t.k);
    y = __fmul_rn(__fadd_rn(__fmul_rn(t.s, x1), __fmul_rn(t.c, y1)), t.k);
    z = __fmul_rn(z, t.k);
}

#define R3D_N_STATS 40
#ifndef R3D_OCC_G
#define R3D_OCC_G 8
#endif
constexpr int OCC_G = R3D_OCC_G;
constexpr int OCC_FAR_CAP = 63;
constexpr double kFix = 1099511627776.0;

__device__ __forceinline__ void occ_far_clear(const EngineDev& e, int b, int tid) {
    if (tid <= OCC_FAR_CAP) e.occ_far[(size_t)b * (OCC_FAR_CAP + 1) + tid] = tid == 0 ? 0 : -1;
}

__device__ __forceinline__ void load_xyz(const EngineDev& e, int b, int p, int n0, double& x, double& y, double& z) {
    if (p < n0) {
        const float4 v = __ldg(&e.xyzi[(size_t)b * e.max_points + p]);
        x = (double)v.x; y = (double)v.y; z = (double)v.z;
    } else {
        const size_t t = (size_t)b * e.max_inserted + (p - n0);
        x = e.tail_x[t]; y = e.tail_y[t]; z = e.tail_z[t];
    }
}

}
```

### pcl_augmentation_b200/csrc/r3d_k_ingest.cuh

```cuda
__global__ void k_reset_alive(EngineDev e, int n_scans) {
    const int b = blockIdx.y;
    if (b >= n_scans) return;
    const int n0 = e.st[b].n0;
    const size_t base = (size_t)b * e.P;
    for (int p = blockIdx.x * blockDim.x + threadIdx.x; p < n0; p += gridDim.x * blockDim.x) e.alive[base + p] = 1;
}

__global__ void k_reset_state(EngineDev e, int n_scans, const int* n0_arr, const int* nbox0_arr) {
    const int b = blockIdx.x * blockDim.x + threadIdx.x;
    if (b >= n_scans) return;
    ScanState& s = e.st[b];
    s.n0 = n0_arr[b]; s.n_tail = 0; s.tail_before = 0; s.n_boxes = nbox0_arr[b];
    s.phase = PH_INIT; s.status = 0;
    s.inserted_class = -1;
    for (int c = 0; c < R3D_MAX_CLASSES; ++c) s.remaining[c] = c < e.n_classes ? e.counts[b * e.n_classes + c] : 0;
    for (int c = e.n_classes - 1; c >= 0; --c) if (s.remaining[c] > 0) s.inserted_class = c;
    s.timeout = 0; s.start_idx = 0; s.end_idx = 0; s.s_idx = 0; s.event = 0;
    s.cur_class = 0; s.cur_obj = -1;
    s.try_active = 0; s.need_project = 0; s.apply_flag = 0; s.dirty = 0; s.scene_changed = 1;
    s.n_feasible = 0; s.found_rank = INT_MAX; s.chosen_rot = 0; s.accepted = 0; s.chosen_v = 0;
    s.n_inserted = 0; s.n_check = 0; s.far_flag = 0;
    s.first = 1; s.extreme_removed = 0; s.d_r0 = 0; s.d_r1 = -1; s.d_c0 = 0; s.d_c1 = -1;
    s.new_min_bits = R3D_EMPTY_U64; s.new_max_bits = 0ull;
    s.min_el_bits = R3D_EMPTY_U64; s.max_el_bits = 0ull;
    if (e.task == 1) {
        const double* T = e.poses + (size_t)b * 16;
        s.win_x0 = (int)(T[3] - (double)e.ss_move_x) - e.map_window / 2;
        s.win_y0 = (int)(T[7] - (double)e.ss_move_y) - e.map_window / 2;
    } else { s.win_x0 = 0; s.win_y0 = 0; }
    const int uw = (e.n_objects + 31) / 32;
    for (int w = 0; w < uw; ++w) e.unplaceable[(size_t)b * uw + w] = 0u;
}
```

### pcl_augmentation_b200/csrc/r3d_k_occlusion.cuh

```cuda
struct ObjProj { double x, y, z, r, el; int pix, col; };
__device__ __forceinline__ ObjProj project_obj_point(const EngineDev& e, const ObjBox& ob, const ImageGeom& g, int i,
                                                     double c, double sn, double dz, ScanState& s) {
    ObjProj o;
    const double x0 = e.obj_x[ob.first + i], y0 = e.obj_y[ob.first + i];
    o.x = sub(mul(c, x0), mul(sn, y0));
    o.y = add(mul(sn, x0), mul(c, y0));
    o.z = add(e.obj_z[ob.first + i], dz);
    o.r = range3(o.x, o.y, o.z);
    o.el = elevation(o.z, o.r);
    const int row = bin_row(g, o.el);
    o.col = bin_col(g, azimuth(o.x, o.y));
    o.pix = -1;
    if (row >= 0 && row < g.rows) {
        if (o.col < 0 || o.col >= g.cols) set_error(s, R3D_ERR_ASSERT);
        else o.pix = row * g.cols + o.col;
    }
    return o;
}

struct ObjPix { double r; int pix; };
__device__ __forceinline__ ObjPix project_obj_pix(const EngineDev& e, const ObjBox& ob, const ImageGeom& g, const FastGeom& fg, int i,
                                                  double c, double sn, double dz, ScanState& s) {
    ObjPix o;
    const double x0 = e.obj_x[ob.first + i], y0 = e.obj_y[ob.first + i];
// ... 185 lines not shown
    const double level = e.cand_level[cb + k];
    const double dz = sub(level, ob.cz);
    unsigned* dm = e.dmask + (size_t)b * e.dwords;
    const double* smooth = e.smooth + (size_t)b * e.hw;
    const int t0 = s.n_tail, chk0 = s.n_check, nbox0 = s.n_boxes, nins0 = s.n_inserted, n0 = s.n0;
    if (s.d_r1 >= s.d_r0 && s.d_c1 >= s.d_c0) {
        const int nw = (s.d_c1 >> 5) - (s.d_c0 >> 5) + 2, nrow = s.d_r1 - s.d_r0 + 1;
        for (int i = threadIdx.x; i < nrow * nw; i += blockDim.x) {
            const int r = s.d_r0 + i / nw;
            const int w = ((r * e.cols + s.d_c0) >> 5) + i % nw;
            if (w <= ((r * e.cols + s.d_c1) >> 5)) dm[w] = 0u;
        }
    }
    __syncthreads();
    {
        int r_lo = INT_MAX, r_hi = -1, c_lo = INT_MAX, c_hi = -1;
        for (int i = threadIdx.x; i < ob.count; i += blockDim.x) {
            const ObjProj o = project_obj_point(e, ob, g, i, c, sn, dz, s);
            s_pix[i] = o.pix; s_r[i] = o.r;
            if (o.pix < 0) continue;
            const int pr = o.pix / W, pc = o.pix % W;
            r_lo = min(r_lo, pr); r_hi = max(r_hi, pr); c_lo = min(c_lo, pc); c_hi = max(c_hi, pc);
        }
        for (int o = 16; o > 0; o >>= 1) {
            r_lo = min(r_lo, __shfl_xor_sync(0xffffffffu, r_lo, o)); r_hi = max(r_hi, __shfl_xor_sync(0xffffffffu, r_hi, o));
            c_lo = min(c_lo, __shfl_xor_sync(0xffffffffu, c_lo, o)); c_hi = max(c_hi, __shfl_xor_sync(0xffffffffu, c_hi, o));
        }
        if ((threadIdx.x & 31) == 0) {
            atomicMin(&s_rect[0], r_lo); atomicMax(&s_rect[1], r_hi); atomicMin(&s_rect[2], c_lo); atomicMax(&s_rect[3], c_hi);
        }
    }
    __syncthreads();
    const bool any_px = s_rect[1] >= 0;
    const int wr0 = any_px ? max(s_rect[0] - 2, 0) : 0, wr1 = any_px ? min(s_rect[1] + 2, H - 1) : -1;
    const int wc0 = any_px ? max(s_rect[2] - 1, 0) : 0, wc1 = any_px ? min(s_rect[3] + 1, W - 1) : -1;
    const int nr = wr1 - wr0 + 1, nc = wc1 - wc0 + 1;
    const bool in_smem = any_px && nr * nc <= SEL_TILE_PX;
    if (threadIdx.x == 0 && any_px) atomicAdd(&e.stats[in_smem ? 4 : 5], 1ull);
    if (in_smem) {
        const int npx = nr * nc;
        for (int i = threadIdx.x; i < npx; i += blockDim.x) s_tile[i] = R3D_EMPTY_U64;
        for (int i = threadIdx.x; i < (npx + 31) / 32; i += blockDim.x) { s_dil[i] = 0u; s_vis[i] = 0u; }
        __syncthreads();
        for (int i = threadIdx.x; i < ob.count; i += blockDim.x) {
            const int pix = s_pix[i];
            if (pix < 0) continue;
            const int pr = pix / W, pc = pix % W;
            atomicMin(&s_tile[(pr - wr0) * nc + (pc - wc0)], dbl_bits(s_r[i]));
            for (int dr = -2; dr <= 2; ++dr)
                for (int dc = -1; dc <= 1; ++dc) {
                    const int r1 = pr + dr, c1 = pc + dc;
                    if (r1 < 0 || r1 >= H || c1 < 0 || c1 >= W) continue;
                    const int q = (r1 - wr0) * nc + (c1 - wc0);
                    atomicOr(&s_dil[q >> 5], 1u << (q & 31));
                }
        }
        __syncthreads();
        for (int lq = threadIdx.x; lq < npx; lq += blockDim.x) {
            if (!(s_dil[lq >> 5] & (1u << (lq & 31)))) continue;
            const int r = wr0 + lq / nc, cc = wc0 + lq % nc;
            double val;
            if (tile_pixel_value(s_tile, s_dil, H, W, wr0, wc0, nr, nc, r, cc, val) && val < smooth[r * W + cc]) {
                atomicOr(&s_vis[lq >> 5], 1u << (lq & 31));
                const int q = r * W + cc;
                atomicOr(&dm[q >> 5], 1u << (q & 31));
            }
        }
        __syncthreads();
        for (int i = threadIdx.x; i < ob.count; i += blockDim.x) {
            const int pix = s_pix[i];
            if (pix < 0) continue;
            const int lq = (pix / W - wr0) * nc + (pix % W - wc0);
            if (s_vis[lq >> 5] & (1u << (lq & 31))) {
                const int slot = atomicAdd(&s_nvis, 1);
                s_keys[slot] = ((unsigned long long)(unsigned)pix << 32) | (unsigned)i;
            }
        }
    } else if (any_px) {
        unsigned long long* raw = e.obj_raw + (size_t)b * e.hw;
        unsigned* vm = e.vmask + (size_t)b * e.dwords;
        for (int i = threadIdx.x; i < e.dwords; i += blockDim.x) vm[i] = 0u;
        __syncthreads();
        for (int i = threadIdx.x; i < ob.count; i += blockDim.x) {
            const int pix = s_pix[i];
            if (pix < 0) continue;
            atomicMin(&raw[pix], dbl_bits(s_r[i]));
            const int pr = pix / W, pc = pix % W;
            for (int dr = -2; dr <= 2; ++dr)
                for (int dc = -1; dc <= 1; ++dc) {
                    const int r1 = pr + dr, c1 = pc + dc;
                    if (r1 < 0 || r1 >= H || c1 < 0 || c1 >= W) continue;
                    const int q = r1 * W + c1;
                    atomicOr(&vm[q >> 5], 1u << (q & 31));
                }
        }
        __threadfence_block();
        __syncthreads();
        for (int t = threadIdx.x; t < ob.count * 15; t += blockDim.x) {
            const int i = t / 15, o = t % 15;
            const int pix = s_pix[i];
            if (pix < 0) continue;
            const int r = pix / W + (o / 3 - 2), cc = pix % W + (o % 3 - 1);
            if (r < 0 || r >= H || cc < 0 || cc >= W) continue;
            const int q = r * W + cc;
            double val;
            if (obj_pixel_value(raw, vm, H, W, r, cc, val) && val < smooth[q]) atomicOr(&dm[q >> 5], 1u << (q & 31));
        }
        __threadfence_block();
        __syncthreads();
        for (int i = threadIdx.x; i < ob.count; i += blockDim.x) {
            const int pix = s_pix[i];
            if (pix >= 0 && (dm[pix >> 5] & (1u << (pix & 31)))) {
                const int slot = atomicAdd(&s_nvis, 1);
                s_keys[slot] = ((unsigned long long)(unsigned)pix << 32) | (unsigned)i;
            }
            if (pix >= 0) raw[pix] = R3D_EMPTY_U64;
        }
    }
    __syncthreads();
    const int nvis = s_nvis;
    if (accepted) {
        if (e.try_obj[b].count <= q.pts) {
            unsigned long long* sorted = reinterpret_cast<unsigned long long*>(s_r);
            for (int j = threadIdx.x; j < nvis; j += blockDim.x) {
                const unsigned long long key = s_keys[j];
                int rank = 0;
                for (int i = 0; i < nvis; ++i) rank += s_keys[i] < key;
                sorted[rank] = key;
            }
            __syncthreads();
            s_keys = sorted;
        } else {
            int np2 = 1;
            while (np2 < nvis) np2 <<= 1;
            for (int i = nvis + threadIdx.x; i < np2; i += blockDim.x) s_keys[i] = R3D_EMPTY_U64;
            __syncthreads();
            bitonic_sort_u64(s_keys, np2);
        }
        if (t0 + nvis > e.max_inserted || nbox0 + 1 > e.max_boxes || nins0 + 1 > e.max_events) {
            __syncthreads();
            if (threadIdx.x == 0) { set_error(s, R3D_ERR_CAPACITY); s.phase = PH_ERROR; }
        } else {
            const size_t base = (size_t)b * e.P + n0 + t0;
            const size_t tb = (size_t)b * e.max_inserted + t0;
            const size_t chk = ((size_t)b * e.max_inserted + chk0) * 5;
            for (int j = threadIdx.x; j < nvis; j += blockDim.x) {
                const int i = (int)(s_keys[j] & 0xffffffffull);
                const ObjProj o = project_obj_point(e, ob, g, i, c, sn, dz, s);
                e.tail_x[tb + j] = o.x; e.tail_y[tb + j] = o.y; e.tail_z[tb + j] = o.z;
                const float inten = e.obj_i[ob.first + i];
                const unsigned lab = e.obj_label[ob.first + i];
                e.tail_i[tb + j] = inten;
                e.label[base + j] = lab;
                e.r[base + j] = o.r; e.el[base + j] = o.el;
                atomicMin(&s_el[0], dbl_bits(o.el)); atomicMax(&s_el[1], dbl_bits(o.el));
                e.col[base + j] = (unsigned short)o.col;
                e.pix[base + j] = o.pix;
                e.alive[base + j] = 1;
                float* ck = e.check + chk + (size_t)j * 5;
                ck[0] = (float)o.x; ck[1] = (float)o.y; ck[2] = (float)o.z; ck[3] = inten; ck[4] = (float)lab;
            }
            __syncthreads();
            if (threadIdx.x == 0) {
                int* rec = e.inserted + ((size_t)b * e.max_events + nins0) * 4;
                rec[0] = s.cur_obj; rec[1] = k; rec[2] = ob.cls; rec[3] = nvis;
                const YawBox yb = make_yaw_box(ob.cx, ob.cy, ob.a, ob.b, c, sn);
                double* ib = e.inserted_box + ((size_t)b * e.max_events + nins0) * 8;
                ib[0] = yb.cx; ib[1] = yb.cy; ib[2] = level; ib[3] = yb.m00; ib[4] = yb.m10;
                ib[5] = ob.length; ib[6] = ob.width; ib[7] = ob.height;
                Box bx = yaw_box_to_box(yb, level, ob.length, ob.width, ob.height);
                bx.reach = ob.reach;
                e.boxes[(size_t)b * e.max_boxes + nbox0] = bx;
                e.box_tests[(size_t)b * e.max_boxes + nbox0] = make_box_test(bx);
                s.n_boxes = nbox0 + 1; s.n_inserted = nins0 + 1;
                s.tail_before = t0; s.n_tail = t0 + nvis; s.n_check = chk0 + nvis;
                s.new_min_bits = s_el[0]; s.new_max_bits = s_el[1];
            }
        }
    }
    if (threadIdx.x == 0) {
        s.accepted = accepted ? 1 : 0; s.chosen_rot = k; s.chosen_v = nvis;
        s.d_r0 = wr0; s.d_r1 = wr1; s.d_c0 = wc0; s.d_c1 = wc1;
        if (!accepted) { s.new_min_bits = R3D_EMPTY_U64; s.new_max_bits = 0ull; }
    }
}

__global__ void __launch_bounds__(512) k_select_emit(EngineDev e, int n_scans, int key_cap, int smem_pts) {
    const int b = blockIdx.x;
    if (b >= n_scans || !e.gate_try[b]) return;
    ScanState& s = e.st[b];
    const int nf = s.n_feasible;
    if (nf == 0) return;
    extern __shared__ unsigned long long s_dyn[];
    const bool accepted = s.found_rank < nf;
    const int rank = accepted ? s.found_rank : nf - 1;
    select_emit_body(e, b, s, e.feas[(size_t)b * e.K + rank], accepted, sel_scratch(s_dyn, key_cap, smem_pts, SEL_TILE_PX));
}
```

### pcl_augmentation_b200/csrc/r3d_k_prepass.cuh

```cuda
__device__ __forceinline__ void agg_count(int* arr, int key, bool active) {
    const unsigned act = __ballot_sync(0xffffffffu, active);
    if (!active) return;
    const unsigned peers = __match_any_sync(act, key);
    if ((int)(threadIdx.x & 31) == __ffs(peers) - 1) atomicAdd(&arr[key], __popc(peers));
}
__device__ __forceinline__ int agg_slot(int* arr, int key, bool active) {
    const unsigned act = __ballot_sync(0xffffffffu, active);
    if (!active) return -1;
    const unsigned peers = __match_any_sync(act, key);
    const int lane = threadIdx.x & 31, leader = __ffs(peers) - 1;
    int base = 0;
    if (lane == leader) base = atomicAdd(&arr[key], __popc(peers));
    base = __shfl_sync(peers, base, leader);
    return base + __popc(peers & ((1u << lane) - 1u));
}

struct AggTicket { unsigned peers; int base; };
__device__ __forceinline__ AggTicket agg_issue(int* arr, int key, bool active) {
    AggTicket t{0u, 0};
    const unsigned act = __ballot_sync(0xffffffffu, active);
    if (active) {
        t.peers = __match_any_sync(act, key);
        if ((int)(threadIdx.x & 31) == __ffs(t.peers) - 1) t.base = atomicAdd(&arr[key], __popc(t.peers));
    }
    return t;
}
__device__ __forceinline__ int agg_finish(const AggTicket& t) {
    if (!t.peers) return -1;
    const int base = __shfl_sync(t.peers, t.base, __ffs(t.peers) - 1);
    return base + __popc(t.peers & ((1u << (threadIdx.x & 31)) - 1u));
}

__device__ __forceinline__ bool grids_exclusive(const EngineDev& e) {
    return e.task == 0 && e.n_surf_all == 1 && e.surf_all[0] == e.road_label;
}
__device__ __forceinline__ void agg_count2(int* arr_a, int* arr_g, int gc, int which) {
    const unsigned act = __ballot_sync(0xffffffffu, which >= 0);
    if (which < 0) return;
    const unsigned peers = __match_any_sync(act, gc * 2 + which);
    if ((int)(threadIdx.x & 31) == __ffs(peers) - 1) atomicAdd(&(which ? arr_g : arr_a)[gc], __popc(peers));
}
__device__ __forceinline__ AggTicket agg_issue2(int* arr_a, int* arr_g, int gc, int which) {
    AggTicket t{0u, 0};
    const unsigned act = __ballot_sync(0xffffffffu, which >= 0);
    if (which >= 0) {
        t.peers = __match_any_sync(act, gc * 2 + which);
        if ((int)(threadIdx.x & 31) == __ffs(t.peers) - 1) t.base = atomicAdd(&(which ? arr_g : arr_a)[gc], __popc(t.peers));
    }
    return t;
}

__global__ void __launch_bounds__(STREAM_THREADS) k_ingest_count(EngineDev e, int n_scans) {
    const int b = blockIdx.y;
    if (b >= n_scans) return;
    ScanState& s = e.st[b];
    const int n0 = s.n0;
    const int p0 = blockIdx.x * CHUNK;
    {
        unsigned long long* z = e.zraw + (size_t)b * e.hw;
        const int per = (e.hw + gridDim.x - 1) / gridDim.x;
        for (int i = blockIdx.x * per + threadIdx.x; i < min((int)(blockIdx.x + 1) * per, e.hw); i += STREAM_THREADS) z[i] = R3D_EMPTY_U64;
    }
    if (p0 >= n0) return;
    const double d_az = kTwoPi / (double)e.cols;
    const float inv_d_az = (float)(1.0 / d_az);
    float err_az = 6e-6f * inv_d_az + 5e-7f * (float)e.cols + 1e-5f;
    if (!(err_az < 0.25f)) err_az = 2.0f;
    const size_t base = (size_t)b * e.P;
    int* cell = e.gcell + (size_t)b * e.G * e.G;
    int* acell = e.acell + (size_t)b * e.G * e.G;
    int* coff = e.col_off + (size_t)b * (e.cols + 1);
    unsigned long long lmin = R3D_EMPTY_U64, lmax = 0ull;
    const bool excl = grids_exclusive(e);
    const float4* __restrict__ src = e.xyzi + (size_t)b * e.max_points;
    const int q_end = min(p0 + CHUNK, n0);
    float4 vn = make_float4(1.f, 0.f, 0.f, 0.f);
    unsigned labn = 0u;
    if (p0 + (int)threadIdx.x < n0) { vn = __ldg(&src[p0 + threadIdx.x]); labn = e.label[base + p0 + threadIdx.x]; }
    for (int q = p0; q < q_end; q += STREAM_THREADS) {
        const int p = q + threadIdx.x;
        const bool in = p < n0;
        const float4 v = vn;
        const unsigned lab = labn;
        {
            const int pn = p + STREAM_THREADS;
            vn = make_float4(1.f, 0.f, 0.f, 0.f); labn = 0u;
            if (q + STREAM_THREADS < q_end && pn < n0) { vn = __ldg(&src[pn]); labn = e.label[base + pn]; }
        }
        const double x = v.x, y = v.y, z = v.z;
        const double r = range3(x, y, z);
        const double el = elevation(z, r);
        int c;
        if (!fast_col(inv_d_az, err_az, e.cols, v.x, v.y, c)) c = trunc_to_int(__ddiv_rn(az_mod(azimuth(x, y)), d_az));
        const int cc = max(0, min(c, e.cols - 1));
        if (in) {
            if (!(r > 0.0) || c < 0 || c >= e.cols) set_error(s, R3D_ERR_ASSERT);
            e.r[base + p] = r;
            e.el[base + p] = el;
            e.col[base + p] = (unsigned short)cc;
            e.alive[base + p] = 1;
            const unsigned long long bits = dbl_bits(el);
            lmin = min(lmin, bits); lmax = max(lmax, bits);
        }
        const int gc = grid_coord(e, v.y) * e.G + grid_coord(e, v.x);
        const bool in_a = in && !(e.task == 0 && lab == (unsigned)e.road_label);
        const bool in_g = in && (double)v.z > -3.0 && any_surface_label(e, lab);
        if (excl) agg_count2(acell, cell, gc, in_g ? 1 : (in_a ? 0 : -1));
        else { agg_count(acell, gc, in_a); agg_count(cell, gc, in_g); }
        agg_count(coff, cc, in);
    }
    __shared__ unsigned long long s_min[STREAM_THREADS / 32], s_max[STREAM_THREADS / 32];
    for (int o = 16; o > 0; o >>= 1) {
        lmin = min(lmin, __shfl_xor_sync(0xffffffffu, lmin, o));
        lmax = max(lmax, __shfl_xor_sync(0xffffffffu, lmax, o));
    }
    if ((threadIdx.x & 31) == 0) { s_min[threadIdx.x >> 5] = lmin; s_max[threadIdx.x >> 5] = lmax; }
    __syncthreads();
    if (threadIdx.x == 0) {
        for (int w = 1; w < STREAM_THREADS / 32; ++w) { lmin = min(lmin, s_min[w]); lmax = max(lmax, s_max[w]); }
        if (lmax >= lmin) { atomicMin(&s.min_el_bits, lmin); atomicMax(&s.max_el_bits, lmax); }
    }
}

__global__ void __launch_bounds__(1024) k_bucket_scan3(EngineDev e, int n_scans) {
    const size_t gg = (size_t)e.G * e.G;
    if (blockIdx.y == 0) bucket_scan_body(e.gcell, gg, (int)gg, n_scans);
    else if (blockIdx.y == 1) bucket_scan_body(e.acell, gg, (int)gg, n_scans);
    else bucket_scan_body(e.col_off, (size_t)e.cols + 1, e.cols, n_scans);
}

__global__ void __launch_bounds__(STREAM_THREADS) k_scatter_project(EngineDev e, int n_scans) {
    const int b = blockIdx.y;
    if (b >= n_scans) return;
    ScanState& s = e.st[b];
    const int n0 = s.n0;
    const int p0 = blockIdx.x * CHUNK;
    if (blockIdx.x == 0 && threadIdx.x == 0) {
        e.far_arr[b] = 0;
        if (s.min_el_bits == R3D_EMPTY_U64) set_error(s, R3D_ERR_ASSERT);
        s.geom = make_geom(e.rows, e.cols, e.cols, bits_dbl(s.max_el_bits), bits_dbl(s.min_el_bits));
    }
    if (p0 >= n0) return;
    const ImageGeom g = make_geom(e.rows, e.cols, e.cols, bits_dbl(s.max_el_bits), bits_dbl(s.min_el_bits));
    const size_t base = (size_t)b * e.P;
    int* cell = e.gcell + (size_t)b * e.G * e.G;
    int* acell = e.acell + (size_t)b * e.G * e.G;
    int* coff = e.col_off + (size_t)b * (e.cols + 1);
    float4* out = e.gpts + (size_t)b * e.max_points;
    float4* aout = e.apts + (size_t)b * e.max_points;
    int* cidx = e.col_idx + (size_t)b * e.max_points;
    unsigned long long* z = e.zraw + (size_t)b * e.hw;
    static_assert(CHUNK % (2 * STREAM_THREADS) == 0, "two points per thread and iteration");
    const bool excl = grids_exclusive(e);
    for (int q = p0; q < min(p0 + CHUNK, n0); q += 2 * STREAM_THREADS) {
        int p[2], col[2], gc[2], which[2];
        bool in[2];
        float4 v[2];
        unsigned lab[2];
        double el[2], r[2];
#pragma unroll
        for (int u = 0; u < 2; ++u) {
            p[u] = q + u * STREAM_THREADS + threadIdx.x;
            in[u] = p[u] < n0;
            v[u] = make_float4(1.f, 0.f, 0.f, 0.f); lab[u] = 0u; col[u] = 0; el[u] = 0.0; r[u] = 0.0;
            if (in[u]) {
                v[u] = __ldg(&e.xyzi[(size_t)b * e.max_points + p[u]]); lab[u] = e.label[base + p[u]]; col[u] = e.col[base + p[u]];
                el[u] = e.el[base + p[u]]; r[u] = e.r[base + p[u]];
            }
        }
        AggTicket ta[2], tg[2], tc[2];
#pragma unroll
        for (int u = 0; u < 2; ++u) {
            gc[u] = grid_coord(e, v[u].y) * e.G + grid_coord(e, v[u].x);
            const bool in_a = in[u] && !(e.task == 0 && lab[u] == (unsigned)e.road_label);
            const bool in_g = in[u] && (double)v[u].z > -3.0 && any_surface_label(e, lab[u]);
            if (excl) {
                which[u] = in_g ? 1 : (in_a ? 0 : -1);
                ta[u] = agg_issue2(acell, cell, gc[u], which[u]);
                tg[u] = AggTicket{0u, 0};
            } else {
                which[u] = -1;
                ta[u] = agg_issue(acell, gc[u], in_a);
                tg[u] = agg_issue(cell, gc[u], in_g);
            }
            tc[u] = agg_issue(coff, col[u], in[u]);
        }
#pragma unroll
        for (int u = 0; u < 2; ++u) {
            int pix = -1;
            if (in[u]) {
                const int row = bin_row(g, el[u]);
                if (row < 0 || row >= g.rows) set_error(s, R3D_ERR_ASSERT);
                else { pix = row * g.cols + col[u]; atomicMin(&z[pix], dbl_bits(r[u])); }
                e.pix[base + p[u]] = pix;
            }
        }
#pragma unroll
        for (int u = 0; u < 2; ++u) {
            const int sa = agg_finish(ta[u]);
            if (sa >= 0) {
                if (which[u] == 1) out[sa] = make_float4(v[u].x, v[u].y, v[u].z, __uint_as_float(lab[u]));
                else aout[sa] = make_float4(v[u].x, v[u].y, v[u].z, apt_tag(e, lab[u], p[u]));
            }
            const int sg = agg_finish(tg[u]);
            if (sg >= 0) out[sg] = make_float4(v[u].x, v[u].y, v[u].z, __uint_as_float(lab[u]));
            const int sc = agg_finish(tc[u]);
            if (sc >= 0) cidx[sc] = p[u];
        }
    }
}

constexpr int NEAR_THREADS = 1024;
__host__ __device__ __forceinline__ size_t grid_near_smem(int G) {
    const int wpr = (G + 31) / 32;
    return (size_t)G * G + 2 * (size_t)(G + 2) * wpr * 4;
}
__global__ void __launch_bounds__(NEAR_THREADS) k_grid_near_bits(EngineDev e, int n_scans) {
    const int b = blockIdx.x, G = e.G;
    if (b >= n_scans) return;
    extern __shared__ __align__(16) unsigned char s_near[];
    const int wpr = (G + 31) / 32, nwords = G * wpr;
    unsigned char* s_dist = s_near;
    unsigned* s_a = reinterpret_cast<unsigned*>(s_near + (((size_t)G * G + 15) & ~(size_t)15));
    unsigned* s_b = s_a + (size_t)(G + 2) * wpr;
    const int* cell = e.gcell + (size_t)b * G * G;
    const int tid = threadIdx.x, lane = tid & 31, warp = tid >> 5, nwarps = NEAR_THREADS / 32;
    for (int i = tid; i < (G + 2) * wpr; i += NEAR_THREADS) { s_a[i] = 0u; s_b[i] = 0u; }
    for (int i = tid; i < G * G / 4; i += NEAR_THREADS) reinterpret_cast<unsigned*>(s_dist)[i] = 0x01010101u * (unsigned)NEAR_CAP;
    for (int i = (G * G / 4) * 4 + tid; i < G * G; i += NEAR_THREADS) s_dist[i] = (unsigned char)NEAR_CAP;
    __syncthreads();
    for (int u = warp; u < nwords; u += nwarps) {
        const int y = u / wpr, x = (u % wpr) * 32 + lane;
        bool occ = false;
        if (x < G) { const int q = y * G + x; occ = cell[q] > (q > 0 ? cell[q - 1] : 0); }
        const unsigned m = __ballot_sync(0xffffffffu, occ);
        if (lane == 0) s_a[(size_t)(y + 1) * wpr + u % wpr] = m;
        if (occ) s_dist[y * G + x] = 0;
    }
    __syncthreads();
    unsigned* cur = s_a;
    unsigned* nxt = s_b;
    for (int d = 1; d < NEAR_CAP; ++d) {
        for (int u = tid; u < nwords; u += NEAR_THREADS) {
            const int y = u / wpr, w = u % wpr;
            unsigned acc = 0u;
#pragma unroll
            for (int dy = 0; dy <= 2; ++dy) {
                const unsigned* row = cur + (size_t)(y + dy) * wpr;
                const unsigned m = row[w];
                acc |= m | (m << 1) | (m >> 1) | (w > 0 ? row[w - 1] >> 31 : 0u) | (w + 1 < wpr ? row[w + 1] << 31 : 0u);
            }
            if (w == wpr - 1 && (G & 31)) acc &= (1u << (G & 31)) - 1u;
            const unsigned old = cur[(size_t)(y + 1) * wpr + w];
            nxt[(size_t)(y + 1) * wpr + w] = acc;
            unsigned fresh = acc & ~old;
            while (fresh) {
                const int bit = __ffs(fresh) - 1; fresh &= fresh - 1;
                const int x = w * 32 + bit;
                if (x < G) s_dist[y * G + x] = (unsigned char)d;
            }
        }
        __syncthreads();
        unsigned* t = cur; cur = nxt; nxt = t;
    }
    unsigned char* out = e.gnear + (size_t)b * G * G;
    if ((((size_t)b * G * G) & 15) == 0 && (G * G) % 16 == 0) {
        for (int i = tid; i < G * G / 16; i += NEAR_THREADS) reinterpret_cast<uint4*>(out)[i] = reinterpret_cast<const uint4*>(s_dist)[i];
    } else {
        for (int i = tid; i < G * G; i += NEAR_THREADS) out[i] = s_dist[i];
    }
}
```

### pcl_augmentation_b200/csrc/r3d_k_update_project.cuh

```cuda
__device__ __forceinline__ bool pix_removed(const EngineDev& e, int b, const ScanState& s, int pix) {
    if (pix < 0) return false;
    if (e.dmask[(size_t)b * e.dwords + (pix >> 5)] & (1u << (pix & 31))) return true;
    return e.far_arr[b] && e.smooth[(size_t)b * e.hw + pix] > kEmptyRange;
}

constexpr int UPDATE_THREADS = 256;
#ifndef R3D_UPDATE_G
#define R3D_UPDATE_G 8
#endif
constexpr int UPDATE_G = R3D_UPDATE_G;
__device__ __forceinline__ bool last_block_done(unsigned* ticket, unsigned n_blocks) {
    __shared__ bool s_last;
    __threadfence();
    __syncthreads();
    if (threadIdx.x == 0) s_last = atomicAdd(ticket, 1u) == n_blocks - 1;
    __syncthreads();
    if (s_last) __threadfence();
    return s_last;
}

__device__ __forceinline__ void adjust_map_point(const EngineDev& e, int b, ScanState& s, const double* T, int p, int delta = 0,
                                                 bool ignore_alive = false);

template <bool OCC_COUNTS = false>
__device__ __forceinline__ bool apply_vis_mask(const EngineDev& e, int b, ScanState& s, int tid, int nthr) {
    const double* T = e.poses + (size_t)b * 16;
    const size_t base = (size_t)b * e.P;
    bool extreme = false;
    const int* off = e.col_off + (size_t)b * (e.cols + 1);
    const int* idx = e.col_idx + (size_t)b * e.max_points;
    int c0 = s.d_c0, c1 = s.d_c1;
    if (e.far_arr[b]) { c0 = 0; c1 = e.cols - 1; }
    const unsigned long long lo = s.min_el_bits, hi = s.max_el_bits;
    if (c1 >= c0) {
        const int beg = c0 > 0 ? off[c0 - 1] : 0, end = off[c1];
        for (int i = beg + tid; i < end; i += 4 * nthr) {
            int p[4], px[4];
#pragma unroll
            for (int u = 0; u < 4; ++u) p[u] = i + u * nthr < end ? idx[i + u * nthr] : -1;
#pragma unroll
            for (int u = 0; u < 4; ++u) px[u] = (p[u] >= 0 && e.alive[base + p[u]]) ? e.pix[base + p[u]] : -1;
#pragma unroll
            for (int u = 0; u < 4; ++u)
                if (px[u] >= 0 && pix_removed(e, b, s, px[u])) {
                    e.alive[base + p[u]] = 0;
                    if (OCC_COUNTS) adjust_map_point(e, b, s, T, p[u], -1, true);
                    const unsigned long long bits = dbl_bits(e.el[base + p[u]]);
                    extreme |= bits == lo || bits == hi;
                }
        }
    }
    for (int t = tid; t < s.tail_before; t += nthr) {
        const int p = s.n0 + t;
        if (e.alive[base + p] && pix_removed(e, b, s, e.pix[base + p])) {
            e.alive[base + p] = 0;
            if (OCC_COUNTS) adjust_map_point(e, b, s, T, p, -1, true);
            const unsigned long long bits = dbl_bits(e.el[base + p]);
            extreme |= bits == lo || bits == hi;
        }
    }
    return extreme;
}

__global__ void __launch_bounds__(UPDATE_THREADS) k_update(EngineDev e, int n_scans) {
    const int b = blockIdx.y;
    if (b >= n_scans) return;
    const int do_apply = e.gate_apply[b], do_update = e.gate_update[b];
    if (!do_apply && !do_update) {
        if (blockIdx.x == 0 && threadIdx.x == 0) {
            e.gate_full[b] = 0; e.gate_patch[b] = 0;
            int* r = e.cf_rect + (size_t)b * 4; r[0] = 0; r[1] = -1; r[2] = 0; r[3] = -1;
        }
        return;
    }
    ScanState& s = e.st[b];
    const size_t base = (size_t)b * e.P;
    const int tid = blockIdx.x * UPDATE_THREADS + threadIdx.x, nthr = UPDATE_G * UPDATE_THREADS;
    const bool extreme = do_apply && apply_vis_mask(e, b, s, tid, nthr);
    if (__syncthreads_or(extreme) && threadIdx.x == 0) atomicOr(&s.extreme_removed, 1);
    if (!last_block_done(&e.tickets[(size_t)b * 4 + 0], UPDATE_G)) return;
    __shared__ int s_patch;
    if (threadIdx.x == 0) {
        int full = 0, patch = 0;
        int* rect = e.cf_rect + (size_t)b * 4;
        rect[0] = 0; rect[1] = -1; rect[2] = 0; rect[3] = -1;
        if (do_update) {
            const bool extended = s.new_min_bits < s.min_el_bits || s.new_max_bits > s.max_el_bits;
            full = s.first || *(volatile int*)&s.extreme_removed || extended || e.far_arr[b] || e.force_full;
            patch = !full;
            if (full) {
                s.min_el_bits = R3D_EMPTY_U64; s.max_el_bits = 0ull;
                rect[0] = 0; rect[1] = e.rows - 1; rect[2] = 0; rect[3] = e.cols - 1;
            } else {
                rect[0] = max(s.d_r0 - 4, 0); rect[1] = min(s.d_r1 + 4, e.rows - 1);
                rect[2] = max(s.d_c0 - 2, 0); rect[3] = min(s.d_c1 + 2, e.cols - 1);
            }
            s.first = 0;
            s.new_min_bits = R3D_EMPTY_U64; s.new_max_bits = 0ull;
            atomicAdd(&e.stats[full ? 0 : 3], 1ull);
        }
        s.extreme_removed = 0;
        e.gate_full[b] = full; e.gate_patch[b] = patch;
        s_patch = patch;
        if (full) e.full_list[atomicAdd(&e.work_cnt[0], 1)] = b;
        if (rect[1] >= rect[0] && rect[3] >= rect[2]) {
            const int ty0 = rect[0] / CF_TH, ty1 = rect[1] / CF_TH, tx0 = rect[2] / CF_TW, tx1 = rect[3] / CF_TW;
            const int nt = (ty1 - ty0 + 1) * (tx1 - tx0 + 1);
            int* task = e.cf_tasks + atomicAdd(&e.work_cnt[1], nt);
            for (int ty = ty0; ty <= ty1; ++ty)
                for (int tx = tx0; tx <= tx1; ++tx) *task++ = b * e.cf_tiles + ty * e.cf_tiles_x + tx;
        }
    }
    __syncthreads();
    if (do_update && e.task == 1) {
        const int ww = e.map_window * e.map_window / 32;
        unsigned* o = e.occ_win + (size_t)b * ww;
        for (int i = threadIdx.x; i < ww; i += UPDATE_THREADS) o[i] = 0u;
        occ_far_clear(e, b, threadIdx.x);
    }
    if (!s_patch) return;
    unsigned long long* z = e.zraw + (size_t)b * e.hw;
    const unsigned* dm = e.dmask + (size_t)b * e.dwords;
    if (s.d_r1 >= s.d_r0 && s.d_c1 >= s.d_c0) {
        const int nw = (s.d_c1 >> 5) - (s.d_c0 >> 5) + 2, nrow = s.d_r1 - s.d_r0 + 1;
        for (int i = threadIdx.x; i < nrow * nw; i += UPDATE_THREADS) {
            const int r = s.d_r0 + i / nw;
            const int w = ((r * e.cols + s.d_c0) >> 5) + i % nw;
            if (w > ((r * e.cols + s.d_c1) >> 5)) continue;
            unsigned m = dm[w];
            while (m) { const int bit = __ffs(m) - 1; m &= m - 1; z[(w << 5) + bit] = R3D_EMPTY_U64; }
        }
    }
    __syncthreads();
    if (s.apply_flag)
        for (int p = s.n0 + s.tail_before + threadIdx.x; p < s.n0 + s.n_tail; p += UPDATE_THREADS)
            if (e.alive[base + p]) atomicMin(&z[e.pix[base + p]], dbl_bits(e.r[base + p]));
}

__global__ void __launch_bounds__(STREAM_THREADS) k_minmax(EngineDev e, int n_scans) {
    __shared__ unsigned long long s_min[STREAM_THREADS / 32], s_max[STREAM_THREADS / 32];
    const int n_full = e.work_cnt[0];
    for (int li = blockIdx.y; li < n_full; li += gridDim.y) {
    const int b = e.full_list[li];
    ScanState& s = e.st[b];
    const int n = s.n0 + s.n_tail;
    const int p0 = blockIdx.x * CHUNK;
    if (p0 >= n) continue;
    const size_t base = (size_t)b * e.P;
    unsigned long long lmin = R3D_EMPTY_U64, lmax = 0ull;
    for (int p = p0 + threadIdx.x; p < min(p0 + CHUNK, n); p += STREAM_THREADS) {
        if (e.alive[base + p]) {
            const unsigned long long bits = dbl_bits(e.el[base + p]);
            lmin = min(lmin, bits); lmax = max(lmax, bits);
        }
    }
    for (int o = 16; o > 0; o >>= 1) {
        lmin = min(lmin, __shfl_xor_sync(0xffffffffu, lmin, o));
        lmax = max(lmax, __shfl_xor_sync(0xffffffffu, lmax, o));
    }
    if ((threadIdx.x & 31) == 0) { s_min[threadIdx.x >> 5] = lmin; s_max[threadIdx.x >> 5] = lmax; }
    __syncthreads();
    if (threadIdx.x == 0) {
        for (int w = 1; w < STREAM_THREADS / 32; ++w) { lmin = min(lmin, s_min[w]); lmax = max(lmax, s_max[w]); }
        if (lmax >= lmin) { atomicMin(&s.min_el_bits, lmin); atomicMax(&s.max_el_bits, lmax); }
    }
    __syncthreads();
    }
}

__global__ void __launch_bounds__(STREAM_THREADS) k_clear_images(EngineDev e, int n_scans) {
    const int n_full = e.work_cnt[0];
    for (int li = blockIdx.y; li < n_full; li += gridDim.y) {
        const int b = e.full_list[li];
        ScanState& s = e.st[b];
        if (blockIdx.x == 0 && threadIdx.x == 0) {
            e.far_arr[b] = 0;
            if (s.min_el_bits == R3D_EMPTY_U64) { set_error(s, R3D_ERR_ASSERT); }
            s.geom = make_geom(e.rows, e.cols, e.cols, bits_dbl(s.max_el_bits), bits_dbl(s.min_el_bits));
        }
        unsigned long long* z = e.zraw + (size_t)b * e.hw;
        for (int i = blockIdx.x * blockDim.x + threadIdx.x; i < e.hw; i += gridDim.x * blockDim.x) z[i] = R3D_EMPTY_U64;
    }
}

__global__ void __launch_bounds__(STREAM_THREADS) k_project(EngineDev e, int n_scans) {
    const int n_full = e.work_cnt[0];
    for (int li = blockIdx.y; li < n_full; li += gridDim.y) {
    const int b = e.full_list[li];
    ScanState& s = e.st[b];
    const int n = s.n0 + s.n_tail;
    const int p0 = blockIdx.x * CHUNK;
    if (p0 >= n) continue;
    const ImageGeom g = make_geom(e.rows, e.cols, e.cols, bits_dbl(s.max_el_bits), bits_dbl(s.min_el_bits));
    const size_t base = (size_t)b * e.P;
    unsigned long long* z = e.zraw + (size_t)b * e.hw;
    auto one = [&](bool alive, double el, unsigned col, double r) -> int {
        if (!alive) return -1;
        const int row = bin_row(g, el);
        if (row < 0 || row >= g.rows) { set_error(s, R3D_ERR_ASSERT); return -1; }
        const int pix = row * g.cols + (int)col;
        atomicMin(&z[pix], dbl_bits(r));
        return pix;
    };
#pragma unroll 2
    for (int it = 0; it < CHUNK / (STREAM_THREADS * 4); ++it) {
        const int p = p0 + it * STREAM_THREADS * 4 + threadIdx.x * 4;
        if (p >= n) break;
        if (p + 3 < n) {
            const uchar4 a = *reinterpret_cast<const uchar4*>(e.alive + base + p);
            if (!(a.x | a.y | a.z | a.w)) continue;
            const double2 e01 = *reinterpret_cast<const double2*>(e.el + base + p);
            const double2 e23 = *reinterpret_cast<const double2*>(e.el + base + p + 2);
            const ushort4 c = *reinterpret_cast<const ushort4*>(e.col + base + p);
            const double2 r01 = *reinterpret_cast<const double2*>(e.r + base + p);
            const double2 r23 = *reinterpret_cast<const double2*>(e.r + base + p + 2);
            int4 px;
            px.x = one(a.x, e01.x, c.x, r01.x); px.y = one(a.y, e01.y, c.y, r01.y);
            px.z = one(a.z, e23.x, c.z, r23.x); px.w = one(a.w, e23.y, c.w, r23.y);
            *reinterpret_cast<int4*>(e.pix + base + p) = px;
        } else {
            for (int q = p; q < n; ++q) e.pix[base + q] = one(e.alive[base + q], e.el[base + q], e.col[base + q], e.r[base + q]);
        }
    }
    }
}

struct RawImage {
    const unsigned long long* raw;
    __device__ void load(int64_t i, double& v, uint8_t& o) const {
        const unsigned long long b = raw[i];
        const bool hit = b != R3D_EMPTY_U64;
        v = hit ? bits_dbl(b) : kEmptyRange;
        o = hit ? 3 : 0;
    }
    __device__ double lab(int64_t i) const { return raw[i] != R3D_EMPTY_U64 ? 1.0 : -1.0; }
};

__device__ __forceinline__ void adjust_map_point(const EngineDev& e, int b, ScanState& s, const double* T, int p, int delta,
                                                 bool ignore_alive) {
    const size_t base = (size_t)b * e.P;
    if (!ignore_alive && !e.alive[base + p]) return;
    const unsigned lab = e.label[base + p];
    bool ground = false;
    for (int i = 0; i < e.n_road_indexes; ++i) ground |= lab == (unsigned)e.road_indexes[i];
    if (ground) return;
    double x, y, z;
    load_xyz(e, b, p, s.n0, x, y, z);
    if (!(z < 1.5)) return;
    const double wx = add(add(add(mul(T[0], x), mul(T[1], y)), mul(T[2], z)), T[3]);
    const double wy = add(add(add(mul(T[4], x), mul(T[5], y)), mul(T[6], z)), T[7]);
    int ix = trunc_to_int(sub(wx, (double)e.ss_move_x));
    int iy = trunc_to_int(sub(wy, (double)e.ss_move_y));
    if (ix >= e.ss_sx || iy >= e.ss_sy || ix < -e.ss_sx || iy < -e.ss_sy) { if (delta >= 0) set_error(s, R3D_ERR_INDEX); return; }
    if (ix < 0) ix += e.ss_sx;
    if (iy < 0) iy += e.ss_sy;
    if (e.ss_map[(size_t)ix * e.ss_sy + iy] == 0) return;
    const int lx = ix - s.win_x0, ly = iy - s.win_y0;
    if (lx < 0 || ly < 0 || lx >= e.map_window || ly >= e.map_window) {
        if (delta < 0) return;
        int* far = e.occ_far + (size_t)b * (OCC_FAR_CAP + 1);
        const int cell = ix * e.ss_sy + iy;
        far[0] = 1;
        for (int i = 0; i < OCC_FAR_CAP; ++i) {
            const int old = atomicCAS(&far[1 + (cell + i) % OCC_FAR_CAP], -1, cell);
            if (old == -1 || old == cell) return;
        }
        set_error(s, R3D_ERR_CAPACITY);
        return;
    }
    const int bit = lx * e.map_window + ly;
    unsigned* word = &e.occ_win[(size_t)b * (e.map_window * e.map_window / 32) + (bit >> 5)];
    if (delta == 0) { atomicOr(word, 1u << (bit & 31)); return; }
    unsigned* cnt = &e.occ_cnt[(size_t)b * e.map_window * e.map_window + bit];
    if (delta > 0) { atomicAdd(cnt, 1u); atomicOr(word, 1u << (bit & 31)); }
    else if (atomicSub(cnt, 1u) == 1u) atomicAnd(word, ~(1u << (bit & 31)));
}

__global__ void __launch_bounds__(STREAM_THREADS) k_adjust_map(EngineDev e, int n_scans, int count_too = 0) {
    const int b = blockIdx.y;
    if (b >= n_scans || !e.gate_update[b]) return;
    ScanState& s = e.st[b];
    const int n = s.n0 + s.n_tail;
    const int p0 = blockIdx.x * CHUNK;
    if (p0 >= n) return;
    const double* T = e.poses + (size_t)b * 16;
    for (int p = p0 + threadIdx.x; p < min(p0 + CHUNK, n); p += STREAM_THREADS) adjust_map_point(e, b, s, T, p, count_too ? 1 : 0);
}
```

### pcl_augmentation_b200/csrc/r3d_k_walk.cuh

```cuda
#ifdef R3D_WALK_NOINLINE
#define R3D_WALK_FN __noinline__
#else
#define R3D_WALK_FN
#endif
constexpr int WALK_THREADS = R3D_WALK_THREADS;
constexpr int WALK_CTAS_PER_SM = R3D_WALK_CTAS_PER_SM;
constexpr int WALK_W = WALK_THREADS / GRP;
constexpr int WALK_Q = WALK_W + WALK_THREADS / 32;
constexpr int WALK_SEL_PTS = 1024;
#ifndef R3D_WALK_SEL_TILE
#define R3D_WALK_SEL_TILE 4096
#endif
constexpr int WALK_SEL_TILE = R3D_WALK_SEL_TILE;
constexpr int WALK_SEL_KEYS = 1024;
constexpr int WALK_OCC_LANES = 64;
constexpr int WALK_OCC_PAR = WALK_THREADS / WALK_OCC_LANES;
constexpr int WALK_NWARPS = WALK_THREADS / 32;


struct WalkSmem { size_t list_off, flags_off, scratch_off, total; };
__host__ __device__ __forceinline__ size_t walk_sel_bytes() {
    return (size_t)WALK_SEL_KEYS * 8 + (size_t)WALK_SEL_PTS * 8 + (size_t)WALK_SEL_TILE * 8 + (size_t)WALK_SEL_PTS * 4 +
           2 * (size_t)(WALK_SEL_TILE / 32) * 4 + 16;
}
__host__ __device__ __forceinline__ WalkSmem walk_smem_layout(int K, int dwords) {
    WalkSmem L;
    size_t o = (size_t)3 * OBJ_SMEM_PTS * 8;
    L.list_off = o; o += ((size_t)(K + 1) * 2 + 15) & ~(size_t)15;
    L.flags_off = o; o += ((size_t)(K + 1) + 15) & ~(size_t)15;
    L.scratch_off = o;
    const size_t occ = (size_t)dwords * 4;
    const size_t cf = (size_t)CF_SH * CF_SW * 8 + 4 * (size_t)CF_SH * CF_WORDS * 4;
    o += occ > cf ? occ : cf;
    const size_t sel = walk_sel_bytes();
    L.total = o > sel ? o : sel;
    if (L.total < sizeof(CfPipeSmem)) L.total = sizeof(CfPipeSmem);
    return L;
}

enum : int { WT_CTRL = 0, WT_UPDATE, WT_SETUP, WT_PLACE, WT_OCCL, WT_SELECT, WT_TOTAL, WT_ONMAP, WT_LEVEL_WARP, WT_COLLIDE_WARP,
              WT_N_LEVEL, WT_N_COLLIDE, WT_APPLY, WT_PATCH, WT_CLOSEFILL, WT_SS_RESWEEP, WT_SS_LEVEL, WT_COUNT };
constexpr int WALK_T0 = 16;
struct WalkClock {
    long long t;
    __device__ __forceinline__ void start() { if (threadIdx.x == 0) t = clock64(); }
    __device__ __forceinline__ void lap(const EngineDev& e, int phase) {
        if (threadIdx.x == 0) { const long long n = clock64(); atomicAdd(&e.stats[WALK_T0 + phase], (unsigned long long)(n - t)); t = n; }
    }
};

struct WalkCtl {
    int apply, project, tryact;
    int n_list, nfw, n_feas, found;
    int found_k, last_k;
    double found_level, last_level;
    double dz_run, dz_next;
    int changed;
    int cnt_lo[WALK_OCC_PAR], cnt_hi[WALK_OCC_PAR];
    int exact_cnt;
    int wk[WALK_Q];
    unsigned char wflag[WALK_Q];
    double wlevel[WALK_Q];
    int wfeas[WALK_W];
    int won[WALK_W];
    int wsub[WALK_W];
    int n_sub;
    int next;
    double wcx[WALK_Q], wcy[WALK_Q];
    int a_k[WALK_W];
    unsigned char a_on[WALK_W];
    double a_cx[WALK_W], a_cy[WALK_W];
    int wlist[WALK_THREADS / 32];
    unsigned surf[R3D_MAX_SURFACE];
    int n_surf;
    double wdz[WALK_W];
    double wtol[WALK_W];
    unsigned long long wtolp[WALK_W], wtolb[WALK_W];
    int wbad[WALK_W];
    int whit[WALK_Q];
    int witness;
    unsigned char wpass[WALK_W], wtodo[WALK_W], whok[WALK_W], whas[WALK_W];
    ObjBox ob;
    int s_warp[WALK_NWARPS];
    int upd_full, upd_patch, rect[4];
    unsigned long long el_min, el_max;
    __align__(16) float wclip[WALK_NWARPS][8];
};

__device__ R3D_WALK_FN void walk_close_fill(const EngineDev& e, int b, const int* rect, unsigned char* scratch) {
    unsigned long long (*s_raw)[CF_SW] = reinterpret_cast<unsigned long long (*)[CF_SW]>(scratch);
    unsigned (*s_one)[CF_WORDS] = reinterpret_cast<unsigned (*)[CF_WORDS]>(scratch + (size_t)CF_SH * CF_SW * 8);
    unsigned (*s_in)[CF_WORDS] = s_one + CF_SH;
    unsigned (*s_dil)[CF_WORDS] = s_in + CF_SH;
    unsigned (*s_ero)[CF_WORDS] = s_dil + CF_SH;
    const int H = e.rows, W = e.cols, tid = threadIdx.x, nt = blockDim.x, lane = tid & 31, warp = tid >> 5, nwarps = nt >> 5;
    const unsigned long long* raw = e.zraw + (size_t)b * e.hw;
    double* out = e.smooth + (size_t)b * e.hw;
    auto left = [](const unsigned* a, int w) { return (a[w] << 1) | (w > 0 ? a[w - 1] >> 31 : 0u); };
    auto right = [](const unsigned* a, int w) { return (a[w] >> 1) | (a[w + 1] << 31); };
    bool far = false;
    for (int r0 = rect[0]; r0 <= rect[1]; r0 += CF_TH)
        for (int c0 = rect[2]; c0 <= rect[3]; c0 += CF_TW) {
            const int th = min(CF_TH, rect[1] - r0 + 1), tw = min(CF_TW, rect[3] - c0 + 1);
            const int sh = th + 2 * CF_HR, sw = tw + 2 * CF_HC;
            for (int i = tid; i < sh * sw; i += nt) {
                const int lr = i / sw, lc = i % sw;
                const int r = r0 - CF_HR + lr, c = c0 - CF_HC + lc;
                s_raw[lr][lc] = (r >= 0 && r < H && c >= 0 && c < W) ? raw[(size_t)r * W + c] : R3D_EMPTY_U64;
            }
            if (tid < sh) { s_one[tid][3] = 0u; s_in[tid][3] = 0u; s_dil[tid][3] = ~0u; }
            __syncthreads();
            for (int u = warp; u < sh * 3; u += nwarps) {
                const int lr = u / 3, w = u % 3, lc = w * 32 + lane;
                const int r = r0 - CF_HR + lr, c = c0 - CF_HC + lc;
                const bool inside = lc < sw && r >= 0 && r < H && c >= 0 && c < W;
                const bool hit = inside && s_raw[lr][min(lc, sw - 1)] != R3D_EMPTY_U64;
                const unsigned b_one = __ballot_sync(0xffffffffu, hit), b_in = __ballot_sync(0xffffffffu, inside);
                if (lane == 0) { s_one[lr][w] = b_one; s_in[lr][w] = b_in; }
            }
            __syncthreads();
            for (int t = tid; t < (sh - 4) * 3; t += nt) {
                const int lr = 2 + t / 3, w = t % 3;
                unsigned d = 0u;
#pragma unroll
                for (int dr = -2; dr <= 2; ++dr) { const unsigned* a = s_one[lr + dr]; d |= a[w] | left(a, w) | right(a, w); }
                s_dil[lr][w] = d | ~s_in[lr][w];
            }
            __syncthreads();
            for (int t = tid; t < th * 3; t += nt) {
                const int lr = CF_HR + t / 3, w = t % 3;
                unsigned er = ~0u;
#pragma unroll
                for (int dr = -2; dr <= 2; ++dr) { const unsigned* a = s_dil[lr + dr]; er &= a[w] & left(a, w) & right(a, w); }
                s_ero[lr][w] = er;
            }
            __syncthreads();
            for (int i = tid; i < th * tw; i += nt) {
                const int lr = i / tw, lc = i % tw;
                const int r = r0 + lr, c = c0 + lc;
                if (r >= H || c >= W) continue;
                const int sr = lr + CF_HR, sc = lc + CF_HC;
                const bool er = (s_ero[sr][sc >> 5] >> (sc & 31)) & 1u;
                const bool one = (s_one[sr][sc >> 5] >> (sc & 31)) & 1u;
                double tv = one ? bits_dbl(s_raw[sr][sc]) : kEmptyRange;
                if (er && !one) {
                    int neighbors = 0;
                    double sum = 0.0;
                    const int q = sc - 1, qw = q >> 5, qb = q & 31;
#pragma unroll
                    for (int dr = -2; dr <= 2; ++dr) {
                        const unsigned m = __funnelshift_r(s_one[sr + dr][qw], s_one[sr + dr][qw + 1], qb) & 7u;
                        if (m & 1u) { neighbors += 1; sum = add(sum, bits_dbl(s_raw[sr + dr][sc - 1])); }
                        if (m & 2u) { neighbors += 1; sum = add(sum, bits_dbl(s_raw[sr + dr][sc])); }
                        if (m & 4u) { neighbors += 1; sum = add(sum, bits_dbl(s_raw[sr + dr][sc + 1])); }
                    }
                    if (neighbors > 0) tv = __ddiv_rn(sum, (double)neighbors);
                }
                out[(size_t)r * W + c] = tv;
                far |= tv > kEmptyRange;
            }
            __syncthreads();
        }
    if (far) atomicOr(&e.far_arr[b], 1);
}

__device__ R3D_WALK_FN void walk_full_reproject(const EngineDev& e, int b, ScanState& s, WalkCtl& c) {
    const int tid = threadIdx.x, nt = blockDim.x;
    const size_t base = (size_t)b * e.P;
    const int n = s.n0 + s.n_tail, n4 = (n + 3) >> 2;
    const unsigned* __restrict__ alive4 = reinterpret_cast<const unsigned*>(e.alive + base);
    const double2* __restrict__ el2 = reinterpret_cast<const double2*>(e.el + base);
    if (tid == 0) { c.el_min = R3D_EMPTY_U64; c.el_max = 0ull; }
    unsigned long long* z = e.zraw + (size_t)b * e.hw;
    if ((reinterpret_cast<size_t>(z) & 15) == 0) {
        ulonglong2* z2 = reinterpret_cast<ulonglong2*>(z);
        for (int i = tid; i < e.hw / 2; i += nt) z2[i] = make_ulonglong2(R3D_EMPTY_U64, R3D_EMPTY_U64);
        if ((e.hw & 1) && tid == 0) z[e.hw - 1] = R3D_EMPTY_U64;
    } else {
        for (int i = tid; i < e.hw; i += nt) z[i] = R3D_EMPTY_U64;
    }
    __syncthreads();
    unsigned long long lmin = R3D_EMPTY_U64, lmax = 0ull;
#pragma unroll 2
    for (int q = tid; q < n4; q += nt) {
        const unsigned a = alive4[q];
        if (!a) continue;
        const double2 lo = el2[2 * q], hi = el2[2 * q + 1];
        const double ev[4] = {lo.x, lo.y, hi.x, hi.y};
#pragma unroll
        for (int u = 0; u < 4; ++u)
            if (((a >> (8 * u)) & 0xFFu) && 4 * q + u < n) { const unsigned long long bits = dbl_bits(ev[u]); lmin = min(lmin, bits); lmax = max(lmax, bits); }
    }
    for (int o = 16; o > 0; o >>= 1) {
        lmin = min(lmin, __shfl_xor_sync(0xffffffffu, lmin, o));
        lmax = max(lmax, __shfl_xor_sync(0xffffffffu, lmax, o));
    }
    if ((tid & 31) == 0 && lmax >= lmin) { atomicMin(&c.el_min, lmin); atomicMax(&c.el_max, lmax); }
    __syncthreads();
    const unsigned long long mn = c.el_min, mx = c.el_max;
    if (tid == 0) {
        s.min_el_bits = mn; s.max_el_bits = mx;
        e.far_arr[b] = 0;
        if (mn == R3D_EMPTY_U64) set_error(s, R3D_ERR_ASSERT);
        s.geom = make_geom(e.rows, e.cols, e.cols, bits_dbl(mx), bits_dbl(mn));
        atomicAdd(&e.stats[11], 1ull);
    }
    const ImageGeom g = make_geom(e.rows, e.cols, e.cols, bits_dbl(mx), bits_dbl(mn));
    const double2* __restrict__ r2 = reinterpret_cast<const double2*>(e.r + base);
    const ushort4* __restrict__ col4 = reinterpret_cast<const ushort4*>(e.col + base);
    int4* pix4 = reinterpret_cast<int4*>(e.pix + base);
#pragma unroll 2
    for (int q = tid; q < n4; q += nt) {
        const unsigned a = alive4[q];
        int px[4] = {-1, -1, -1, -1};
        if (a) {
            const double2 lo = el2[2 * q], hi = el2[2 * q + 1], rl = r2[2 * q], rh = r2[2 * q + 1];
            const ushort4 cc = col4[q];
            const double ev[4] = {lo.x, lo.y, hi.x, hi.y}, rv[4] = {rl.x, rl.y, rh.x, rh.y};
            const int cv[4] = {cc.x, cc.y, cc.z, cc.w};
#pragma unroll
            for (int u = 0; u < 4; ++u)
                if (((a >> (8 * u)) & 0xFFu) && 4 * q + u < n) {
                    const int row = bin_row(g, ev[u]);
                    if (row < 0 || row >= g.rows) set_error(s, R3D_ERR_ASSERT);
                    else { px[u] = row * g.cols + cv[u]; atomicMin(&z[px[u]], dbl_bits(rv[u])); }
                }
        }
        pix4[q] = make_int4(px[0], px[1], px[2], px[3]);
    }
}

__device__ R3D_WALK_FN void walk_adjust_map(const EngineDev& e, int b, ScanState& s) {
    const int n = s.n0 + s.n_tail;
    const double* T = e.poses + (size_t)b * 16;
    for (int p = threadIdx.x; p < n; p += blockDim.x) adjust_map_point(e, b, s, T, p);
}

__device__ R3D_WALK_FN void walk_update(const EngineDev& e, int b, ScanState& s, WalkCtl& c, int do_apply, int do_update,
                            unsigned char* scratch, unsigned char* dyn) {
    long long ut = clock64();
    auto ulap = [&](int phase) {
        if (threadIdx.x == 0) { const long long n = clock64(); atomicAdd(&e.stats[WALK_T0 + phase], (unsigned long long)(n - ut)); ut = n; }
    };
    const int tid = threadIdx.x, nt = blockDim.x;
    const size_t base = (size_t)b * e.P;
    const bool ext = do_apply && (e.task == 1 ? apply_vis_mask<true>(e, b, s, tid, nt) : apply_vis_mask<false>(e, b, s, tid, nt));
    const int extreme = __syncthreads_or(ext);
    ulap(WT_APPLY);
    if (tid == 0) {
        int full = 0, patch = 0;
        int* rect = c.rect;
        rect[0] = 0; rect[1] = -1; rect[2] = 0; rect[3] = -1;
        if (do_update) {
            const bool extended = s.new_min_bits < s.min_el_bits || s.new_max_bits > s.max_el_bits;
            full = s.first || extreme || extended || e.far_arr[b] || e.force_full;
            patch = !full;
            if (full) {
                rect[0] = 0; rect[1] = e.rows - 1; rect[2] = 0; rect[3] = e.cols - 1;
            } else {
                rect[0] = max(s.d_r0 - 4, 0); rect[1] = min(s.d_r1 + 4, e.rows - 1);
                rect[2] = max(s.d_c0 - 2, 0); rect[3] = min(s.d_c1 + 2, e.cols - 1);
            }
            s.first = 0;
            s.new_min_bits = R3D_EMPTY_U64; s.new_max_bits = 0ull;
            atomicAdd(&e.stats[full ? 0 : 3], 1ull);
        }
        s.extreme_removed = 0;
        c.upd_full = full; c.upd_patch = patch;
    }
    __syncthreads();
    const bool rebuild_marks = do_update && e.task == 1 && s.far_flag;
    if (rebuild_marks) {
        const int ww = e.map_window * e.map_window / 32;
        unsigned* o = e.occ_win + (size_t)b * ww;
        for (int i = tid; i < ww; i += nt) o[i] = 0u;
        occ_far_clear(e, b, tid);
        __syncthreads();
    }
    if (c.upd_patch) {
        unsigned long long* z = e.zraw + (size_t)b * e.hw;
        const unsigned* dm = e.dmask + (size_t)b * e.dwords;
        if (s.d_r1 >= s.d_r0 && s.d_c1 >= s.d_c0) {
            const int nw = (s.d_c1 >> 5) - (s.d_c0 >> 5) + 2, nrow = s.d_r1 - s.d_r0 + 1;
            for (int i = tid; i < nrow * nw; i += nt) {
                const int r = s.d_r0 + i / nw;
                const int w = ((r * e.cols + s.d_c0) >> 5) + i % nw;
                if (w > ((r * e.cols + s.d_c1) >> 5)) continue;
                unsigned m = dm[w];
                while (m) { const int bit = __ffs(m) - 1; m &= m - 1; z[(w << 5) + bit] = R3D_EMPTY_U64; }
            }
        }
        __syncthreads();
        if (s.apply_flag)
            for (int p = s.n0 + s.tail_before + tid; p < s.n0 + s.n_tail; p += nt)
                if (e.alive[base + p]) atomicMin(&z[e.pix[base + p]], dbl_bits(e.r[base + p]));
    } else if (c.upd_full) {
        walk_full_reproject(e, b, s, c);
    }
    __syncthreads();
    ulap(WT_PATCH);
    if (c.upd_full && !(e.cols & 1)) {
        const int tiles = e.cf_tiles;
        cf_pipelined_tiles<WALK_THREADS>(*reinterpret_cast<CfPipeSmem*>(dyn), e.zraw, e.rows, e.cols, (int64_t)e.hw, e.smooth, e.far_arr,
                                         0, tiles, 1, [&](int t) { return b * tiles + t; });
    } else if (c.rect[1] >= c.rect[0] && c.rect[3] >= c.rect[2]) walk_close_fill(e, b, c.rect, scratch);
    ulap(WT_CLOSEFILL);
    if (rebuild_marks) { __syncthreads(); walk_adjust_map(e, b, s); }
    __syncthreads();
}

template <class P>
__device__ __forceinline__ int walk_window_list(WalkCtl& c, int nw, int* out, P pred) {
    const int tid = threadIdx.x, lane = tid & 31, w = tid >> 5;
    constexpr int NWW = (WALK_W + 31) / 32;
    bool on = false;
    unsigned m = 0u;
    if (w < NWW) {
        on = tid < nw && pred(tid);
        m = __ballot_sync(0xffffffffu, on);
        if (lane == 0) c.s_warp[w] = __popc(m);
    }
    __syncthreads();
    int off = 0, tot = 0;
#pragma unroll
    for (int i = 0; i < NWW; ++i) { if (i < w) off += c.s_warp[i]; tot += c.s_warp[i]; }
    if (on) out[off + __popc(m & ((1u << lane) - 1u))] = tid;
    if (tid == 0) c.next = 0;
    __syncthreads();
    return tot;
}

__device__ __forceinline__ bool walk_onmap_od(const EngineDev& e, int b, const ObjBox& ob, const ClassCfg& cc, const double* ox,
                                              const double* oy, int k, int gl, unsigned gm) {
    const int count = ob.count, msel = cc.map_sel;
    const int* dims = e.od_map_dims + ((size_t)b * 2 + msel) * 4;
    const int sx = dims[0], sy = dims[1];
    const double mx = (double)dims[2], my = (double)dims[3];
    const unsigned char* map = e.od_maps + e.od_map_off[(size_t)b * 2 + msel];
    const double c = e.cos_k[k], sn = e.sin_k[k];
    bool any_in = false, bad = false;
    for (int i0 = 0; i0 < count; i0 += 4 * GRP) {
        double x[4], y[4];
#pragma unroll
        for (int u = 0; u < 4; ++u) {
            const int i = min(i0 + u * GRP + gl, count - 1);
            x[u] = ox[i]; y[u] = oy[i];
        }
        unsigned char v[4];
#pragma unroll
        for (int u = 0; u < 4; ++u) {
            v[u] = 1;
            const double gx = sub(sub(mul(c, x[u]), mul(sn, y[u])), mx), gy = sub(add(mul(sn, x[u]), mul(c, y[u])), my);
            if (!(gx < 0.0 || gx >= (double)sx || gy < 0.0 || gy >= (double)sy)) {
                any_in = true; v[u] = __ldg(&map[(size_t)((int)gx) * sy + (int)gy]);
            }
        }
        bad = v[0] != 1 || v[1] != 1 || v[2] != 1 || v[3] != 1;
        if (__ballot_sync(gm, bad) & gm) { bad = true; break; }
    }
    return (__ballot_sync(gm, any_in) & gm) != 0u && !bad;
}

__device__ R3D_WALK_FN void walk_levels(const EngineDev& e, int b, WalkCtl& c, const int* list, int n) {
    const int lane = threadIdx.x & 31;
    for (;;) {
        int t = 0;
        if (lane == 0) t = atomicAdd(&c.next, 1);
        t = __shfl_sync(0xffffffffu, t, 0);
        if (t >= n) break;
        const int i = list[t];
        double level = 0.0;
        const long long t0 = clock64();
        const bool ok = e.task == 0 ? warp_road_level<false>(e, b, c.surf, c.n_surf, c.wcx[i], c.wcy[i], lane, level)
                                    : warp_road_level<true>(e, b, c.surf, c.n_surf, c.wcx[i], c.wcy[i], lane, level);
        if (lane == 0) {
            c.wflag[i] = (unsigned char)(ok ? (CF_ONMAP | CF_HOK) : CF_ONMAP);
            c.wlevel[i] = level;
            atomicAdd(&e.stats[WALK_T0 + WT_LEVEL_WARP], (unsigned long long)(clock64() - t0)); atomicAdd(&e.stats[WALK_T0 + WT_N_LEVEL], 1ull);
        }
    }
}

__device__ R3D_WALK_FN void walk_collides(const EngineDev& e, int b, const ScanState& s, WalkCtl& c, const int* list, int n) {
    const int lane = threadIdx.x & 31, warp = threadIdx.x >> 5;
    const ObjBox& ob = c.ob;
    const ClassCfg& cc = e.classes[ob.cls];
    if (n <= 0) return;
    const int wpc = max(1, WALK_NWARPS / n);
    const int t = warp / wpc, part = warp % wpc;
    if (t >= n) return;
    const int i = list[t], k = c.wk[i];
    const long long t0 = clock64();
    const bool hit = warp_collides(e, b, s, ob, cc, e.cos_k[k], e.sin_k[k], c.wlevel[i], lane, part, wpc, &c.whit[i], &c.witness,
                                   c.wclip[warp]);
    if (lane == 0) {
        if (hit && atomicExch(&c.whit[i], 1) == 0) c.wflag[i] = (unsigned char)(CF_ONMAP | CF_HOK | CF_COLLIDE);
        if (part == 0) { atomicAdd(&e.stats[WALK_T0 + WT_COLLIDE_WARP], (unsigned long long)(clock64() - t0)); atomicAdd(&e.stats[WALK_T0 + WT_N_COLLIDE], 1ull); }
    }
}

__device__ R3D_WALK_FN int walk_window_ss(const EngineDev& e, int b, ScanState& s, WalkCtl& c, const double* ox, const double* oy,
                              const double* oz, int base, int nw) {
    const int tid = threadIdx.x, g = tid / GRP, gl = tid % GRP;
    const unsigned gm = group_mask();
    const ObjBox& ob = c.ob;
    const ClassCfg& cc = e.classes[ob.cls];
    if (tid < nw) {
        const int kk = base + tid + 1;
        const double ck = e.cos_k[kk], sk = e.sin_k[kk];
        c.wk[tid] = kk; c.wdz[tid] = c.dz_run; c.wpass[tid] = 0; c.wtodo[tid] = 1; c.whas[tid] = 0; c.whok[tid] = 0;
        c.wlevel[tid] = 0.0; c.wflag[tid] = 0; c.won[tid] = tid;
        c.wcx[tid] = sub(mul(ck, c.ob.cx), mul(sk, c.ob.cy)); c.wcy[tid] = add(mul(sk, c.ob.cx), mul(ck, c.ob.cy));
    }
    __syncthreads();
    const double* T = e.poses + (size_t)b * 16;
    SsMapTest m;
    m.t00 = T[0]; m.t01 = T[1]; m.t02 = T[2]; m.t03 = T[3]; m.t10 = T[4]; m.t11 = T[5]; m.t12 = T[6]; m.t13 = T[7];
    m.okmask = cc.map_ok_mask;
    m.occ = e.occ_win + (size_t)b * (e.map_window * e.map_window / 32);
    m.far = e.occ_far + (size_t)b * (OCC_FAR_CAP + 1);
    m.inv02 = m.t02 != 0.0 ? 1.0 / fabs(m.t02) : 1e300;
    m.inv12 = m.t12 != 0.0 ? 1.0 / fabs(m.t12) : 1e300;
    const int k = base + g + 1;
    const double cs = g < nw ? e.cos_k[k] : 1.0, sn = g < nw ? e.sin_k[k] : 0.0;
    const int warp = tid >> 5, lane = tid & 31;
    constexpr int ITEM_PTS = 128;
    const int n_items_per = ob.count > 4 * GRP ? (ob.count - 4 * GRP + ITEM_PTS - 1) / ITEM_PTS : 0;
    for (int sweep = 0; sweep <= nw; ++sweep) {
        long long t_ph = clock64();
        if (g < nw && c.wtodo[g]) {
            const double dz = c.wdz[g];
            bool off = false;
            double tol_pass = 1e300, tol_bad = 0.0;
#pragma unroll
            for (int u = 0; u < 4; ++u) {
                const int i = min(u * GRP + gl, ob.count - 1);
                double tol;
                const bool o = ss_point_off_map_t<true>(e, s, m, ox[i], oy[i], oz[i], cs, sn, dz, tol);
                tol = fmax(tol, 0.0);
                off |= o;
                if (o) tol_bad = fmax(tol_bad, tol); else tol_pass = fmin(tol_pass, tol);
            }
            const bool bad = (__ballot_sync(gm, off) & gm) != 0u;
            double tol = bad ? tol_bad : tol_pass;
#pragma unroll
            for (int o = GRP / 2; o > 0; o >>= 1) {
                const double other = __shfl_xor_sync(gm, tol, o);
                tol = bad ? fmax(tol, other) : fmin(tol, other);
// ... 195 lines not shown
        } else {
            while (ss_c0 >= ss_n && base < n_list) {
                ss_n = walk_window_ss(e, b, s, c, ox, oy, oz, base, min(WALK_W, n_list - base));
                ss_c0 = 0;
                base += WALK_W;
                if (tid == 0) atomicAdd(&e.stats[9], 1ull);
            }
            if (ss_c0 >= ss_n) break;
            nch = min(WALK_NWARPS, ss_n - ss_c0);
            chunk = c.won + ss_c0;
        }
        {
            if (e.task == 0) {
                walk_levels(e, b, c, chunk, nch);
                __syncthreads();
            }
            if (tid == 0) {
                int n = 0;
                for (int t = 0; t < nch; ++t)
                    if ((c.wflag[chunk[t]] & (CF_ONMAP | CF_HOK)) == (CF_ONMAP | CF_HOK)) { c.whit[chunk[t]] = 0; c.wsub[n++] = chunk[t]; }
                c.n_sub = n; c.next = 0;
            }
            __syncthreads();
            walk_collides(e, b, s, c, c.wsub, c.n_sub);
            __syncthreads();
            clk.lap(e, WT_PLACE);
            if (tid == 0) {
                int n = 0;
                for (int t = 0; t < c.n_sub; ++t)
                    if ((c.wflag[c.wsub[t]] & (CF_ONMAP | CF_HOK | CF_COLLIDE)) == (CF_ONMAP | CF_HOK)) c.wfeas[n++] = c.wsub[t];
                c.nfw = n; c.next = 0;
                if (n) { c.last_k = c.wk[c.wfeas[n - 1]]; c.last_level = c.wlevel[c.wfeas[n - 1]]; }
                c.n_feas += n;
            }
            __syncthreads();
            const int nfw = c.nfw;
            for (int j0 = 0, npar = 1; j0 < nfw && c.found < 0; j0 += npar) {
                npar = 1;
                while (npar < min(nfw - j0, WALK_OCC_PAR) || WALK_NWARPS % npar != 0) ++npar;
                const int lanes = WALK_THREADS / npar, sg = tid / lanes, sl = tid % lanes;
                if (tid < WALK_OCC_PAR) { c.cnt_lo[tid] = 0; c.cnt_hi[tid] = 0; }
                __syncthreads();
                const int j = j0 + sg;
                if (j < nfw) {
                    const int i = c.wfeas[j], k = c.wk[i];
                    const double cs = e.cos_k[k], sn = e.sin_k[k], dz = sub(c.wlevel[i], ob.cz);
                    int lo = 0, hi = 0;
                    for (int p = sl; p < ob.count; p += lanes) {
                        const ObjPix o = project_obj_pix(e, ob, geom, fgeom, p, cs, sn, dz, s);
                        if (o.pix >= 0) { ++hi; if (o.r < smooth[o.pix]) ++lo; }
                    }
                    for (int o = 16; o > 0; o >>= 1) { lo += __shfl_xor_sync(0xffffffffu, lo, o); hi += __shfl_xor_sync(0xffffffffu, hi, o); }
                    if ((tid & 31) == 0) { if (lo) atomicAdd(&c.cnt_lo[sg], lo); if (hi) atomicAdd(&c.cnt_hi[sg], hi); }
                }
                __syncthreads();
                int found = -1;
                for (int q = 0; q < npar && j0 + q < nfw; ++q) {
                    const int lo = c.cnt_lo[q], hi = c.cnt_hi[q];
                    bool ok = lo >= min_pts;
                    if (!ok && lo > 0 && hi >= min_pts) {
                        const int i = c.wfeas[j0 + q];
                        ok = walk_exact_visible(e, b, s, c, c.wk[i], c.wlevel[i], reinterpret_cast<unsigned*>(scratch)) >= min_pts;
                    }
                    if (ok) { found = j0 + q; break; }
                }
                if (found >= 0 && tid == 0) {
                    const int i = c.wfeas[found];
                    c.found = found; c.found_k = c.wk[i]; c.found_level = c.wlevel[i];
                }
                __syncthreads();
            }
            clk.lap(e, WT_OCCL);
        }
        if (c.found >= 0) break;
        if (e.task == 0) { q_head = (q_head + nch) % WALK_Q; q_n -= nch; first_chunk = false; }
        else ss_c0 += nch;
    }
    const int n_feas = c.n_feas;
    if (tid == 0) s.n_feasible = n_feas;
    if (n_feas > 0) {
        const bool accepted = c.found >= 0;
        const int k = accepted ? c.found_k : c.last_k;
        if (tid == 0) e.cand_level[(size_t)b * (K + 1) + k] = accepted ? c.found_level : c.last_level;
        __syncthreads();
        select_emit_body(e, b, s, k, accepted,
                         sel_scratch(reinterpret_cast<unsigned long long*>(dyn), WALK_SEL_KEYS, WALK_SEL_PTS, WALK_SEL_TILE));
    }
    __syncthreads();
    if (e.task == 1 && n_feas > 0 && c.found >= 0) {
        const double* T = e.poses + (size_t)b * 16;
        for (int p = s.n0 + s.tail_before + tid; p < s.n0 + s.n_tail; p += nt) adjust_map_point(e, b, s, T, p, 1, true);
        __syncthreads();
    }
    clk.lap(e, WT_SELECT);
}

__global__ void __launch_bounds__(WALK_THREADS, WALK_CTAS_PER_SM) k_scan_walk(const __grid_constant__ EngineDev e, int n_scans) {
    const int b = blockIdx.x;
    if (b >= n_scans) return;
    extern __shared__ __align__(16) unsigned char w_dyn[];
    __shared__ WalkCtl c;
    __shared__ ScanState s;
    {
        const int* src = reinterpret_cast<const int*>(&e.st[b]);
        int* dst = reinterpret_cast<int*>(&s);
        for (int i = threadIdx.x; i < (int)(sizeof(ScanState) / sizeof(int)); i += blockDim.x) dst[i] = src[i];
    }
    if (threadIdx.x == 0) s.far_flag = e.task == 1 && e.occ_far[(size_t)b * (OCC_FAR_CAP + 1)] != 0;
    __syncthreads();
    const WalkSmem L = walk_smem_layout(e.K, e.dwords);
    int steps = 0;
    WalkClock clk;
    clk.start();
    const long long t_begin = clk.t;
    for (;;) {
        if (threadIdx.x == 0) {
            int apply = 0, project = 0, tryact = 0;
            ctrl_advance(e, b, s, apply, project, tryact);
            c.apply = apply; c.project = project; c.tryact = tryact;
            if (apply) atomicAdd(&e.stats[2], 1ull);
        }
        __syncthreads();
        const int apply = c.apply, project = c.project, tryact = c.tryact;
        clk.lap(e, WT_CTRL);
        if (apply || project) walk_update(e, b, s, c, apply, project, w_dyn + L.scratch_off, w_dyn);
        clk.lap(e, WT_UPDATE);
        if (!tryact) break;
        walk_try(e, b, s, c, w_dyn, L, clk);
        ++steps;
    }
    if (threadIdx.x == 0) {
        const long long lived = clock64() - t_begin;
        atomicAdd(&e.stats[WALK_T0 + WT_TOTAL], (unsigned long long)lived);
        s.walk_cycles = lived; s.walk_tries = steps;
    }
    __syncthreads();
    {
        const int* src = reinterpret_cast<const int*>(&s);
        int* dst = reinterpret_cast<int*>(&e.st[b]);
        for (int i = threadIdx.x; i < (int)(sizeof(ScanState) / sizeof(int)); i += blockDim.x) dst[i] = src[i];
    }
    if (threadIdx.x == 0) atomicMax(&e.stats[8], (unsigned long long)steps);
}

__global__ void k_walk_prepare(EngineDev e, int n_scans, int reset_range) {
    const int tiles = e.cf_tiles;
    for (int i = blockIdx.x * blockDim.x + threadIdx.x; i < n_scans * tiles; i += gridDim.x * blockDim.x) e.cf_tasks[i] = i;
    for (int b = blockIdx.x * blockDim.x + threadIdx.x; b < n_scans; b += gridDim.x * blockDim.x) {
        e.full_list[b] = b;
        e.gate_update[b] = 1;
        if (e.task == 1) for (int i = 0; i <= OCC_FAR_CAP; ++i) occ_far_clear(e, b, i);
        ScanState& s = e.st[b];
        s.first = 0; s.scene_changed = 0;
        if (reset_range) { s.min_el_bits = R3D_EMPTY_U64; s.max_el_bits = 0ull; }
        atomicAdd(&e.stats[0], 1ull);
    }
    if (blockIdx.x == 0 && threadIdx.x == 0) { e.work_cnt[0] = n_scans; e.work_cnt[1] = n_scans * tiles; e.stats[8] = 0ull; }
}
```

### pcl_augmentation_b200/engine.py

```python
from __future__ import annotations

import ctypes as C
from dataclasses import dataclass, field

import numpy as np

from . import _lib
from . import boxes as bx

ROAD_INDEXES = [40, 44, 48]
MAX_NUM_TRIES = 100


@dataclass
class ScanInput:
    xyzi: np.ndarray
    labels: np.ndarray
    box_lines: list
    counts: np.ndarray
    perms: np.ndarray
    maps: dict | None = None
    pose: np.ndarray | None = None
    box_dicts: list | None = None

# ... 317 lines not shown
        _lib.check(self.lib.r3d_engine_set_schedule_policy(self.handle, int(rand), int(ins.get('number_of_object', 0)),
                                                           fixed.ctypes.data), "set_schedule_policy")
        self._policy_set = True

    def load_resident(self, store, indices, seed, epoch):
        if not self._policy_set:
            self.set_schedule_policy()
        idx = np.ascontiguousarray(np.asarray(indices, dtype=np.int64).astype(np.int32))
        self._keep = [store, idx]
        self._n_scans = len(idx)
        mask = (1 << 64) - 1
        _lib.check(self.lib.r3d_engine_load_resident(self.handle, C.byref(store.abi), idx.ctypes.data, len(idx),
                                                     int(seed) & mask, int(epoch) & mask), "load_resident")

    def set_ss_map_device(self, map_u8, move_x, move_y):
        _lib.check(self.lib.r3d_engine_set_ss_map_device(self.handle, map_u8.data_ptr(), int(map_u8.shape[0]),
                                                         int(map_u8.shape[1]), int(move_x), int(move_y)), "set_ss_map_device")

    def schedule_read(self):
        n, nc = self._n_scans, len(self.classes)
        counts, ne = np.zeros((n, nc), dtype=np.int32), C.c_int32()
        _lib.check(self.lib.r3d_engine_schedule_read(self.handle, counts.ctypes.data, None, C.byref(ne)), "schedule_read")
        perms = np.zeros((n, ne.value, nc, self.max_tries), dtype=np.int32)
        _lib.check(self.lib.r3d_engine_schedule_read(self.handle, counts.ctypes.data, perms.ctypes.data, C.byref(ne)),
                   "schedule_read")
        return counts, perms

    def inserted_device(self):
        import torch
        n, e = self._n_scans, self.max_events
        pn, pi, pb, p7 = C.c_void_p(), C.c_void_p(), C.c_void_p(), C.c_void_p()
        _lib.check(self.lib.r3d_engine_inserted_device(self.handle, C.byref(pn), C.byref(pi), C.byref(pb), C.byref(p7)),
                   "inserted_device")
        return {"n_inserted": _cuda_tensor(pn.value, (n,), "<i4", torch.int32),
                "inserted": _cuda_tensor(pi.value, (n, e, 4), "<i4", torch.int32),
                "boxes": _cuda_tensor(p7.value, (n, e, 7), "<f4", torch.float32)}

    def set_world_aug(self, policy):
        if policy is None:
            _lib.check(self.lib.r3d_engine_set_world_aug(self.handle, None), "set_world_aug")
            return
        w = _lib.WorldAug(float(policy.flip_x_prob), float(policy.flip_y_prob), float(policy.rot_max),
                          float(policy.scale_lo), float(policy.scale_hi))
        _lib.check(self.lib.r3d_engine_set_world_aug(self.handle, C.byref(w)), "set_world_aug")

    def world_device(self):
        import torch
        p = C.c_void_p()
        _lib.check(self.lib.r3d_engine_world_device(self.handle, C.byref(p)), "world_device")
        return _cuda_tensor(p.value, (self._n_scans, 8), "<f4", torch.float32)

    def set_target_classes(self, target_classes):
        if self.task != 'od':
            raise _lib.Real3DError("detection targets need an object detection engine")
        target_classes = list(target_classes)
        missing = [c for c in self.classes if c not in target_classes]
        if missing:
            raise _lib.Real3DError(f"insertion classes {missing} are not in target_classes {target_classes}")
        dims = np.zeros((max(len(self.obj_strings), 1), 3), dtype=np.float32)
        for i, s in enumerate(self.obj_strings):
            items = (s.item() if hasattr(s, 'item') else str(s)).split(' ')
            dims[i] = (float(items[10]), float(items[9]), float(items[8]))
        class_target = np.array([target_classes.index(c) + 1 for c in self.classes], dtype=np.int32)
        _lib.check(self.lib.r3d_engine_set_object_targets(self.handle, dims.ctypes.data, class_target.ctypes.data),
                   "set_object_targets")
        self.target_classes = target_classes

    def targets_device(self, store, out):
        if self.task != 'od':
            raise _lib.Real3DError("targets_device: detection targets need an object detection engine")
        if getattr(self, 'target_classes', None) is None:
            raise _lib.Real3DError("targets_device: call set_target_classes first")
        box7, cls = store.scene_targets(self.target_classes)
        gb, gc, ng = out['gt_boxes'], out['gt_classes'], out['n_gt']
        n, m = self._n_scans, int(gb.shape[1])
        assert gb.is_contiguous() and gc.is_contiguous() and ng.is_contiguous()
        assert gb.shape[0] >= n and gb.shape[2] == 7 and tuple(gc.shape[1:]) == (m,) and gc.shape[0] >= n and ng.shape[0] >= n
        ptr = lambda t: t.data_ptr() if t.numel() else None
        _lib.check(self.lib.r3d_engine_targets_device(self.handle, C.byref(store.abi), ptr(box7), ptr(cls), m,
                                                      gb.data_ptr(), gc.data_ptr(), ng.data_ptr()), "targets_device")

    def unpack(self, buffers, raise_on_error=True):
        out = []
        ss = self.task == 'ss'
        n_ins = [int(v) for v in buffers['n_inserted'][:self._n_scans]]
        placed = [(s, j) for s in range(self._n_scans) for j in range(n_ins[s])]
        all_boxes = iter(bx.placed_box_dictionaries(
            [buffers['inserted_box'][s, j] for s, j in placed],
            [(str(c) if ss else c) for c in (self.classes[int(buffers['inserted'][s, j, 2])] for s, j in placed)], ss))
        for s in range(self._n_scans):
            st = int(buffers['status'][s])
            if st != 0 and raise_on_error:
                _lib.check(st, f"scan {s}")
            a, b = buffers['out_off'][s], buffers['out_off'][s + 1]
            ca, cb = buffers['check_off'][s], buffers['check_off'][s + 1]
            inserted, lines, boxes, visible = [], [], [], []
            for j in range(n_ins[s]):
                obj, rot, ci, nvis = (int(v) for v in buffers['inserted'][s, j])
                cls = self.classes[ci]
                box = next(all_boxes)
                inserted.append((self.obj_names[obj], rot, cls))
                boxes.append(box)
                visible.append(nvis)
                if not ss:
                    lines.append(bx.create_annotation_line(self.obj_strings[obj], box, rot * (360.0 / self.yaw_steps)))
            chk = np.array(buffers['check'][ca:cb])
            out.append(ScanResult(velodyne=np.array(buffers['xyzi'][a:b]),
                                  labels=(np.array(buffers['labels'][a:b]).view(np.uint16).astype(np.uint32) if self.fetch_labels
                                          else np.zeros(0, dtype=np.uint32)),
                                  check=chk if ss else chk[:, :4], inserted=inserted, lines=lines, boxes=boxes,
                                  visible=visible, status=st, extra={'rounds': int(buffers['rounds'][0])}))
        return out

    def augment_batch(self, scans):
        self.load(self.stage(scans))
        self.run()
        return self.unpack(self.fetch_raw())

    def probe_places(self, scan, object_id, scene_rows9, want_points=True):
        k1 = self.yaw_steps + 1
        rows = np.ascontiguousarray(scene_rows9, dtype=np.float64)
        flags = np.zeros(k1, dtype=np.uint8)
        boxes = np.zeros((k1, 5), dtype=np.float64)
        m = int(self._db_offsets[object_id + 1] - self._db_offsets[object_id])
        xyz = np.zeros((self.yaw_steps, m, 3), dtype=np.float64) if want_points else None
        nf = C.c_int32()
        _lib.check(self.lib.r3d_engine_probe_places(self.handle, scan, object_id, rows.ctypes.data, len(rows),
                                                    flags.ctypes.data, boxes.ctypes.data,
                                                    xyz.ctypes.data if want_points else None, self.yaw_steps,
                                                    C.byref(nf)), "probe_places")
        rots = [k for k in range(1, k1) if flags[k] == 3]
        assert len(rots) == nf.value
        return flags, boxes, (xyz[:nf.value] if want_points else None), rots

    def profile(self, on=True):
        _lib.check(self.lib.r3d_engine_profile_enable(self.handle, 1 if on else 0), "profile_enable")

    def profile_read(self):
        names = C.create_string_buffer(4096)
        ms = (C.c_double * 64)()
        launches = (C.c_int64 * 64)()
        n = C.c_int()
        _lib.check(self.lib.r3d_engine_profile_read(self.handle, names, 4096, ms, launches, 64, C.byref(n)), "profile_read")
        ks = names.value.decode().split('\n')
        return {ks[i]: {'ms': ms[i], 'launches': int(launches[i])} for i in range(n.value)}

    def stats(self):
        out = np.zeros(40, dtype=np.uint64)
        _lib.check(self.lib.r3d_engine_stats_ex(self.handle, out.ctypes.data, 40), "stats")
        return {'projected_scans': int(out[0]), 'tried_objects': int(out[1]), 'masked_scans': int(out[2]),
                'patched_scans': int(out[3]), 'select_tile': int(out[4]), 'select_global': int(out[5]),
                'prefilter_survivors': int(out[6]), 'onmap_rotations': int(out[7]), 'max_steps_per_scan': int(out[8]),
                'candidate_windows': int(out[9]), 'exact_occlusion_counts': int(out[10]),
                'walker_full_reprojections': int(out[11]),
                'walker_cycles': {k: int(out[16 + i]) for i, k in enumerate(
                    ('schedule', 'update', 'setup_prefilter', 'placement', 'occlusion', 'select_insert', 'total'))},
                'walker_detail': {k: int(out[16 + 7 + i]) for i, k in enumerate(
                    ('onmap_cycles', 'level_warp_cycles', 'collide_warp_cycles', 'n_level', 'n_collide', 'apply_cycles',
                     'patch_cycles', 'closefill_cycles', 'ss_resweeps', 'ss_level_cycles'))}}

    def walk_profile(self):
        n = self._n_scans
        cycles, tries = np.zeros(n, dtype=np.int64), np.zeros(n, dtype=np.int32)
        _lib.check(self.lib.r3d_engine_walk_profile(self.handle, cycles.ctypes.data, tries.ctypes.data, n), "walk_profile")
        return cycles, tries

    def surface_labels(self):
        if self.task == 'od':
            return [int(self.config['labels']['Road'])]
        ins = self.config['insertion']
        out = set()
        for cls in self.classes:
            for v in ins['placement'][cls]:
                out.update(int(x) for x in ins['placement_labels'][v])
        return sorted(out)

    def cuda_stream(self):
        import torch
        return torch.cuda.ExternalStream(int(self.lib.r3d_engine_stream(self.handle)))

    def launch_count(self):
        return int(self.lib.r3d_launch_count())

    def debug_image(self, scan):
        out = np.zeros((self.rows, self.cols), dtype=np.float64)
        _lib.check(self.lib.r3d_engine_debug_image(self.handle, scan, out.ctypes.data), "debug_image")
        return out

    def debug_candidates(self, scan):
        k1 = self.yaw_steps + 1
        flags, level, vis = np.zeros(k1, np.uint8), np.zeros(k1, np.float64), np.zeros(k1, np.int32)
        _lib.check(self.lib.r3d_engine_debug_candidates(self.handle, scan, flags.ctypes.data, level.ctypes.data,
                                                        vis.ctypes.data), "debug_candidates")
        return flags, level, vis

    def close(self):
        if getattr(self, 'handle', None):
            self.lib.r3d_engine_destroy(self.handle)
            self.handle = None

    def __del__(self):
        try:
            self.close()
        except Exception:
            pass


def scan_input_from_case(case, pose=None):
    return ScanInput(xyzi=np.ascontiguousarray(case.pcl5[:, :4].astype(np.float32)),
                     labels=case.pcl5[:, 4].astype(np.uint32), box_lines=list(case.box_lines),
                     counts=case.schedule.counts, perms=case.schedule.perms, maps=case.maps,
                     pose=case.pose if pose is None else pose)
```

Before: 85720.

## Drop per-point range/elevation arrays; recompute from xyz with float screening

Removes the per-point double r and el arrays for original points and keeps them only for inserted tail points. Original-point elevation and range are recomputed from xyzi in the reprojection, using a float screen of z/r and falling back to exact math near bin edges. The elevation min and max are derived from extreme z/r keys through a monotonic acos window check, with a full-scan fallback when that check fails. This cuts global memory writes and reads of two f64 arrays per point, at the cost of extra transcendental compute and more complex exactness logic.

Measured after the change: 84310, median of 6. 1.6% lower.

```diff
diff --git a/pcl_augmentation_b200/csrc/r3d_common.cuh b/pcl_augmentation_b200/csrc/r3d_common.cuh
--- a/pcl_augmentation_b200/csrc/r3d_common.cuh
+++ b/pcl_augmentation_b200/csrc/r3d_common.cuh
@@ -12,6 +12,9 @@
 constexpr double kPi = 3.141592653589793;
 constexpr double kTwoPi = 6.283185307179586;
 constexpr double kEmptyRange = 500.0;
+
+__device__ __forceinline__ unsigned long long dbl_bits(double v) { return (unsigned long long)__double_as_longlong(v); }
+__device__ __forceinline__ double bits_dbl(unsigned long long b) { return __longlong_as_double((long long)b); }
 
 __device__ __forceinline__ double mul(double a, double b) { return __dmul_rn(a, b); }
 __device__ __forceinline__ double add(double a, double b) { return __dadd_rn(a, b); }
@@ -72,10 +75,74 @@
 __device__ __forceinline__ bool fast_col(float inv_d_az, float err_az, int cols, float x, float y, int& col) {
     return fast_bin((atan2f(y, x) + 3.14159274f) * inv_d_az, err_az, cols, col);
 }
-__device__ __forceinline__ bool fast_row(const FastGeom& f, int rows, float z, float r, int& row) {
-    const float t = z / r;
+__device__ __forceinline__ bool fast_row_t(const FastGeom& f, int rows, float t, int& row) {
     if (!(fabsf(t) <= 0.9f)) return false;
     return fast_bin((acosf(t) - f.el0) * f.inv_d_el, f.err_el, rows, row);
+}
+__device__ __forceinline__ bool fast_row(const FastGeom& f, int rows, float z, float r, int& row) {
+    return fast_row_t(f, rows, z / r, row);
+}
+
+constexpr float kTScreen = 1e-6f;
+constexpr double kTSlack = 1.7763568394002505e-15;
+constexpr unsigned long long kTWindowCap = 2048;
+
+__device__ __forceinline__ unsigned long long t_key(double t) {
+    const unsigned long long u = dbl_bits(t);
+    return (u >> 63) ? ~u : (u | 0x8000000000000000ull);
+}
+__device__ __forceinline__ double key_t(unsigned long long k) {
+    return bits_dbl((k >> 63) ? (k & 0x7FFFFFFFFFFFFFFFull) : ~k);
+}
+__device__ __forceinline__ double t_exact(double x, double y, double z) { return __ddiv_rn(z, range3(x, y, z)); }
+
+__device__ __forceinline__ bool t_screen(float x, float y, float z, float& tf) {
+    const float s = __fadd_rn(__fadd_rn(__fmul_rn(x, x), __fmul_rn(y, y)), __fmul_rn(z, z));
+    tf = __fmul_rn(z, rsqrtf(s));
+    return s >= 0x1p-60f && s <= 0x1p100f;
+}
+
+struct TExt {
+    float hi = -2.0f, lo = 2.0f;
+    unsigned long long kmax = 0ull, kmin = R3D_EMPTY_U64;
+};
+__device__ __forceinline__ void t_ext_add(TExt& a, bool in, float x, float y, float z) {
+    float tf;
+    const bool ok = t_screen(x, y, z, tf);
+    float h = in && ok ? tf : -2.0f, l = in && ok ? tf : 2.0f;
+#pragma unroll
+    for (int o = 16; o > 0; o >>= 1) {
+        h = fmaxf(h, __shfl_xor_sync(0xffffffffu, h, o));
+        l = fminf(l, __shfl_xor_sync(0xffffffffu, l, o));
+    }
+    a.hi = fmaxf(a.hi, h); a.lo = fminf(a.lo, l);
+    if (in && (!ok || tf >= a.hi - 2.0f * kTScreen || tf <= a.lo + 2.0f * kTScreen)) {
+        const unsigned long long k = t_key(t_exact(x, y, z));
+        a.kmax = max(a.kmax, k); a.kmin = min(a.kmin, k);
+    }
+}
+__device__ __forceinline__ bool t_near_max(float tf, unsigned long long kmax) {
+    return (double)tf + (double)kTScreen >= key_t(kmax) - 2.0 * kTSlack;
+}
+__device__ __forceinline__ bool t_near_min(float tf, unsigned long long kmin) {
+    return (double)tf - (double)kTScreen <= key_t(kmin) + 2.0 * kTSlack;
+}
+
+__device__ __forceinline__ bool el_from_t_extremes(unsigned long long kmin, unsigned long long kmax,
+                                                   unsigned long long& min_el_bits, unsigned long long& max_el_bits) {
+    min_el_bits = R3D_EMPTY_U64; max_el_bits = 0ull;
+    if (kmin > kmax) return true;
+    const int lane = threadIdx.x & 31;
+    const double tmax = key_t(kmax), tmin = key_t(kmin);
+    const double emin = acos(tmax), emax = acos(tmin);
+    const unsigned long long a0 = t_key(__dsub_rd(tmax, kTSlack)), b1 = t_key(__dadd_ru(tmin, kTSlack));
+    bool ok = a0 <= kmax && kmax - a0 < kTWindowCap && b1 >= kmin && b1 - kmin < kTWindowCap;
+    if (ok) {
+        for (unsigned long long k = a0 + lane; k <= kmax; k += 32) ok &= acos(key_t(k)) >= emin;
+        for (unsigned long long k = kmin + lane; k <= b1; k += 32) ok &= acos(key_t(k)) <= emax;
+    }
+    min_el_bits = dbl_bits(emin); max_el_bits = dbl_bits(emax);
+    return __all_sync(0xffffffffu, ok);
 }
 
 struct Box {
@@ -148,8 +215,6 @@
     return b;
 }
 
-__device__ __forceinline__ unsigned long long dbl_bits(double v) { return (unsigned long long)__double_as_longlong(v); }
-__device__ __forceinline__ double bits_dbl(unsigned long long b) { return __longlong_as_double((long long)b); }
 
 __device__ __forceinline__ float4 ldg_f4(const float4* p) { return __ldg(p); }
 
diff --git a/pcl_augmentation_b200/csrc/r3d_engine.cu b/pcl_augmentation_b200/csrc/r3d_engine.cu
--- a/pcl_augmentation_b200/csrc/r3d_engine.cu
+++ b/pcl_augmentation_b200/csrc/r3d_engine.cu
@@ -74,7 +74,7 @@
     int last_rounds = 0;
     DevBuf<float4> xyzi, out_xyzi, gpts, apts;
     DevBuf<unsigned long long> sel_keys;
-    DevBuf<double> sel_r, tail_x, tail_y, tail_z, r, el, smooth, poses, obj_x, obj_y, obj_z, cos_k, sin_k, radii_sq, cand_level,
+    DevBuf<double> sel_r, tail_x, tail_y, tail_z, tail_r, tail_el, smooth, poses, obj_x, obj_y, obj_z, cos_k, sin_k, radii_sq, cand_level,
         inserted_box;
     DevBuf<float> tail_i, obj_i, check, out_check;
     DevBuf<unsigned> label, dmask, vmask, occ_win, unplaceable, obj_label, out_label, tickets;
@@ -284,7 +284,7 @@
     const size_t B = d.B, P = d.P, K1 = d.K + 1, HW = d.hw;
     TRY(eng->xyzi.alloc(B * d.max_points)); TRY(eng->tail_x.alloc(B * d.max_inserted)); TRY(eng->tail_y.alloc(B * d.max_inserted));
     TRY(eng->tail_z.alloc(B * d.max_inserted)); TRY(eng->tail_i.alloc(B * d.max_inserted)); TRY(eng->label.alloc(B * P));
-    TRY(eng->r.alloc(B * P)); TRY(eng->el.alloc(B * P)); TRY(eng->col.alloc(B * P)); TRY(eng->pix.alloc(B * P));
+    TRY(eng->tail_r.alloc(B * d.max_inserted)); TRY(eng->tail_el.alloc(B * d.max_inserted)); TRY(eng->col.alloc(B * P)); TRY(eng->pix.alloc(B * P));
     TRY(eng->alive.alloc(B * P)); TRY(eng->zraw.alloc(B * HW)); TRY(eng->obj_raw.alloc(B * HW)); TRY(eng->smooth.alloc(B * HW));
     eng->zraw_tmap_ok = make_zraw_tensor_map(&eng->zraw_tmap, eng->zraw.p, d.cols, d.rows, (int)B);
     TRY(eng->dmask.alloc(B * d.dwords)); TRY(eng->vmask.alloc(B * d.dwords)); TRY(eng->st.alloc(B));
@@ -356,7 +356,7 @@
     R3D_CUDA(cudaMemsetAsync(eng->dmask.p, 0, B * d.dwords * sizeof(unsigned), eng->stream));
     R3D_CUDA(cudaStreamSynchronize(eng->stream));
     d.xyzi = eng->xyzi.p; d.tail_x = eng->tail_x.p; d.tail_y = eng->tail_y.p; d.tail_z = eng->tail_z.p; d.tail_i = eng->tail_i.p;
-    d.label = eng->label.p; d.r = eng->r.p; d.el = eng->el.p; d.col = eng->col.p; d.pix = eng->pix.p; d.alive = eng->alive.p;
+    d.label = eng->label.p; d.tail_r = eng->tail_r.p; d.tail_el = eng->tail_el.p; d.col = eng->col.p; d.pix = eng->pix.p; d.alive = eng->alive.p;
     d.zraw = eng->zraw.p; d.obj_raw = eng->obj_raw.p; d.smooth = eng->smooth.p; d.dmask = eng->dmask.p; d.vmask = eng->vmask.p;
     d.st = eng->st.p; d.gate_update = eng->gate_update.p; d.gate_try = eng->gate_try.p; d.gate_apply = eng->gate_apply.p;
     d.gate_full = eng->gate_full.p; d.gate_patch = eng->gate_patch.p; d.cf_rect = eng->cf_rect.p;
@@ -509,7 +509,7 @@
         { Launcher l(eng, KID_INGEST); k_ingest_count<<<dim3(chunks, n), STREAM_THREADS, 0, st>>>(d, n); }
         {
             Launcher l(eng, KID_GRID);
-            k_bucket_scan3<<<dim3(n, 3), 1024, 0, st>>>(d, n);
+            k_bucket_scan3<<<dim3(n, 4), 1024, 0, st>>>(d, n);
         }
         { Launcher l(eng, KID_SCATTER); k_scatter_project<<<dim3(chunks, n), STREAM_THREADS, 0, st>>>(d, n); }
         {
@@ -765,7 +765,7 @@
 #define R3D_OFF(field, stride) if (d.field) v.field = d.field + b * (size_t)(stride)
     R3D_OFF(gcell, gg); R3D_OFF(gpts, d.max_points); R3D_OFF(gnear, gg); R3D_OFF(gscratch, gg); R3D_OFF(acell, gg); R3D_OFF(apts, d.max_points);
     R3D_OFF(xyzi, d.max_points); R3D_OFF(tail_x, d.max_inserted); R3D_OFF(tail_y, d.max_inserted);
-    R3D_OFF(tail_z, d.max_inserted); R3D_OFF(tail_i, d.max_inserted); R3D_OFF(label, d.P); R3D_OFF(r, d.P); R3D_OFF(el, d.P);
+    R3D_OFF(tail_z, d.max_inserted); R3D_OFF(tail_i, d.max_inserted); R3D_OFF(label, d.P); R3D_OFF(tail_r, d.max_inserted); R3D_OFF(tail_el, d.max_inserted);
     R3D_OFF(col, d.P); R3D_OFF(pix, d.P); R3D_OFF(alive, d.P); R3D_OFF(zraw, d.hw); R3D_OFF(obj_raw, d.hw);
     R3D_OFF(smooth, d.hw); R3D_OFF(dmask, d.dwords); R3D_OFF(vmask, d.dwords); R3D_OFF(st, 1); R3D_OFF(gate_update, 1);
     R3D_OFF(gate_try, 1); R3D_OFF(gate_apply, 1); R3D_OFF(gate_full, 1); R3D_OFF(gate_patch, 1); R3D_OFF(cf_rect, 4);
diff --git a/pcl_augmentation_b200/csrc/r3d_engine.cuh b/pcl_augmentation_b200/csrc/r3d_engine.cuh
--- a/pcl_augmentation_b200/csrc/r3d_engine.cuh
+++ b/pcl_augmentation_b200/csrc/r3d_engine.cuh
@@ -42,6 +42,7 @@
     unsigned long long new_min_bits, new_max_bits;
     int win_x0, win_y0;
     unsigned long long min_el_bits, max_el_bits;
+    unsigned long long t_min_key, t_max_key;
     ImageGeom geom;
     long long walk_cycles;
     int walk_tries, walk_pad;
@@ -67,7 +68,7 @@
     double *tail_x, *tail_y, *tail_z;
     float* tail_i;
     unsigned* label;
-    double *r, *el;
+    double *tail_r, *tail_el;
     unsigned short* col;
     int* pix;
     unsigned char* alive;
@@ -175,4 +176,75 @@
     }
 }
 
-}
+template <int NT>
+__device__ __forceinline__ void block_key_extremes(unsigned long long kmin, unsigned long long kmax,
+                                                   unsigned long long* gmin, unsigned long long* gmax) {
+    __shared__ unsigned long long s_min[NT / 32], s_max[NT / 32];
+    for (int o = 16; o > 0; o >>= 1) {
+        kmin = min(kmin, __shfl_xor_sync(0xffffffffu, kmin, o));
+        kmax = max(kmax, __shfl_xor_sync(0xffffffffu, kmax, o));
+    }
+    if ((threadIdx.x & 31) == 0) { s_min[threadIdx.x >> 5] = kmin; s_max[threadIdx.x >> 5] = kmax; }
+    __syncthreads();
+    if (threadIdx.x == 0) {
+        for (int w = 1; w < NT / 32; ++w) { kmin = min(kmin, s_min[w]); kmax = max(kmax, s_max[w]); }
+        if (kmax >= kmin) { atomicMin(gmin, kmin); atomicMax(gmax, kmax); }
+    }
+    __syncthreads();
+}
+
+__device__ __forceinline__ void orig_el_extremes(const EngineDev& e, int b, int n0, unsigned long long kmin, unsigned long long kmax,
+                                              unsigned long long& mn, unsigned long long& mx) {
+    __shared__ unsigned long long s_el[2];
+    __shared__ int s_ok;
+    if (threadIdx.x < 32) {
+        unsigned long long a, c;
+        const bool ok = el_from_t_extremes(kmin, kmax, a, c);
+        if (threadIdx.x == 0) { s_el[0] = a; s_el[1] = c; s_ok = ok; }
+    }
+    __syncthreads();
+    if (!s_ok) {
+        if (threadIdx.x == 0) { s_el[0] = R3D_EMPTY_U64; s_el[1] = 0ull; atomicAdd(&e.stats[12], 1ull); }
+        __syncthreads();
+        const size_t base = (size_t)b * e.P;
+        const float4* __restrict__ src = e.xyzi + (size_t)b * e.max_points;
+        const unsigned long long a0 = t_key(__dsub_rd(key_t(kmax), kTSlack)), b1 = t_key(__dadd_ru(key_t(kmin), kTSlack));
+        unsigned long long lmin = R3D_EMPTY_U64, lmax = 0ull;
+        for (int p = threadIdx.x; p < n0; p += blockDim.x) {
+            if (!e.alive[base + p]) continue;
+            const float4 v = __ldg(&src[p]);
+            float tf;
+            if (t_screen(v.x, v.y, v.z, tf) && !t_near_max(tf, kmax) && !t_near_min(tf, kmin)) continue;
+            const double z = v.z, t = t_exact(v.x, v.y, z);
+            const unsigned long long k = t_key(t);
+            if (!(k >= a0 && k <= kmax) && !(k >= kmin && k <= b1)) continue;
+            const unsigned long long bits = dbl_bits(acos(t));
+            lmin = min(lmin, bits); lmax = max(lmax, bits);
+        }
+        if (lmax >= lmin) { atomicMin(&s_el[0], lmin); atomicMax(&s_el[1], lmax); }
+        __syncthreads();
+    }
+    mn = s_el[0]; mx = s_el[1];
+    __syncthreads();
+}
+
+static __device__ __noinline__ int exact_row(const ImageGeom& g, double z, double r) { return bin_row(g, elevation(z, r)); }
+
+__device__ __forceinline__ int orig_row(const ImageGeom& g, const FastGeom& fg, float4 v, double& r) {
+    const double z = v.z;
+    r = range3(v.x, v.y, z);
+    float tf;
+    int row;
+    if (!t_screen(v.x, v.y, v.z, tf) || !fast_row_t(fg, g.rows, tf, row)) row = exact_row(g, z, r);
+    return row;
+}
+
+__device__ __forceinline__ bool orig_el_is_extreme(const ScanState& s, float4 v, unsigned long long lo, unsigned long long hi) {
+    float tf;
+    if (t_screen(v.x, v.y, v.z, tf) && !t_near_max(tf, s.t_max_key) && !t_near_min(tf, s.t_min_key)) return false;
+    const double z = v.z;
+    const unsigned long long bits = dbl_bits(elevation(z, range3(v.x, v.y, z)));
+    return bits == lo || bits == hi;
+}
+
+}
diff --git a/pcl_augmentation_b200/csrc/r3d_k_ingest.cuh b/pcl_augmentation_b200/csrc/r3d_k_ingest.cuh
--- a/pcl_augmentation_b200/csrc/r3d_k_ingest.cuh
+++ b/pcl_augmentation_b200/csrc/r3d_k_ingest.cuh
@@ -23,6 +23,7 @@
     s.first = 1; s.extreme_removed = 0; s.d_r0 = 0; s.d_r1 = -1; s.d_c0 = 0; s.d_c1 = -1;
     s.new_min_bits = R3D_EMPTY_U64; s.new_max_bits = 0ull;
     s.min_el_bits = R3D_EMPTY_U64; s.max_el_bits = 0ull;
+    s.t_min_key = R3D_EMPTY_U64; s.t_max_key = 0ull;
     if (e.task == 1) {
         const double* T = e.poses + (size_t)b * 16;
         s.win_x0 = (int)(T[3] - (double)e.ss_move_x) - e.map_window / 2;
diff --git a/pcl_augmentation_b200/csrc/r3d_k_occlusion.cuh b/pcl_augmentation_b200/csrc/r3d_k_occlusion.cuh
--- a/pcl_augmentation_b200/csrc/r3d_k_occlusion.cuh
+++ b/pcl_augmentation_b200/csrc/r3d_k_occlusion.cuh
@@ -361,7 +361,7 @@
                 const unsigned lab = e.obj_label[ob.first + i];
                 e.tail_i[tb + j] = inten;
                 e.label[base + j] = lab;
-                e.r[base + j] = o.r; e.el[base + j] = o.el;
+                e.tail_r[tb + j] = o.r; e.tail_el[tb + j] = o.el;
                 atomicMin(&s_el[0], dbl_bits(o.el)); atomicMax(&s_el[1], dbl_bits(o.el));
                 e.col[base + j] = (unsigned short)o.col;
                 e.pix[base + j] = o.pix;
diff --git a/pcl_augmentation_b200/csrc/r3d_k_prepass.cuh b/pcl_augmentation_b200/csrc/r3d_k_prepass.cuh
--- a/pcl_augmentation_b200/csrc/r3d_k_prepass.cuh
+++ b/pcl_augmentation_b200/csrc/r3d_k_prepass.cuh
@@ -70,7 +70,7 @@
     int* cell = e.gcell + (size_t)b * e.G * e.G;
     int* acell = e.acell + (size_t)b * e.G * e.G;
     int* coff = e.col_off + (size_t)b * (e.cols + 1);
-    unsigned long long lmin = R3D_EMPTY_U64, lmax = 0ull;
+    TExt te;
     const bool excl = grids_exclusive(e);
     const float4* __restrict__ src = e.xyzi + (size_t)b * e.max_points;
     const int q_end = min(p0 + CHUNK, n0);
@@ -87,20 +87,15 @@
             vn = make_float4(1.f, 0.f, 0.f, 0.f); labn = 0u;
             if (q + STREAM_THREADS < q_end && pn < n0) { vn = __ldg(&src[pn]); labn = e.label[base + pn]; }
         }
-        const double x = v.x, y = v.y, z = v.z;
-        const double r = range3(x, y, z);
-        const double el = elevation(z, r);
         int c;
-        if (!fast_col(inv_d_az, err_az, e.cols, v.x, v.y, c)) c = trunc_to_int(__ddiv_rn(az_mod(azimuth(x, y)), d_az));
+        if (!fast_col(inv_d_az, err_az, e.cols, v.x, v.y, c)) c = trunc_to_int(__ddiv_rn(az_mod(azimuth(v.x, v.y)), d_az));
         const int cc = max(0, min(c, e.cols - 1));
+        t_ext_add(te, in, v.x, v.y, v.z);
         if (in) {
-            if (!(r > 0.0) || c < 0 || c >= e.cols) set_error(s, R3D_ERR_ASSERT);
-            e.r[base + p] = r;
-            e.el[base + p] = el;
+            const bool origin = !(fabs((double)v.x) + fabs((double)v.y) + fabs((double)v.z) > 0.0);
+            if (origin || c < 0 || c >= e.cols) set_error(s, R3D_ERR_ASSERT);
             e.col[base + p] = (unsigned short)cc;
             e.alive[base + p] = 1;
-            const unsigned long long bits = dbl_bits(el);
-            lmin = min(lmin, bits); lmax = max(lmax, bits);
         }
         const int gc = grid_coord(e, v.y) * e.G + grid_coord(e, v.x);
         const bool in_a = in && !(e.task == 0 && lab == (unsigned)e.road_label);
@@ -109,24 +104,20 @@
         else { agg_count(acell, gc, in_a); agg_count(cell, gc, in_g); }
         agg_count(coff, cc, in);
     }
-    __shared__ unsigned long long s_min[STREAM_THREADS / 32], s_max[STREAM_THREADS / 32];
-    for (int o = 16; o > 0; o >>= 1) {
-        lmin = min(lmin, __shfl_xor_sync(0xffffffffu, lmin, o));
-        lmax = max(lmax, __shfl_xor_sync(0xffffffffu, lmax, o));
-    }
-    if ((threadIdx.x & 31) == 0) { s_min[threadIdx.x >> 5] = lmin; s_max[threadIdx.x >> 5] = lmax; }
-    __syncthreads();
-    if (threadIdx.x == 0) {
-        for (int w = 1; w < STREAM_THREADS / 32; ++w) { lmin = min(lmin, s_min[w]); lmax = max(lmax, s_max[w]); }
-        if (lmax >= lmin) { atomicMin(&s.min_el_bits, lmin); atomicMax(&s.max_el_bits, lmax); }
-    }
+    block_key_extremes<STREAM_THREADS>(te.kmin, te.kmax, &s.t_min_key, &s.t_max_key);
 }
 
 __global__ void __launch_bounds__(1024) k_bucket_scan3(EngineDev e, int n_scans) {
     const size_t gg = (size_t)e.G * e.G;
     if (blockIdx.y == 0) bucket_scan_body(e.gcell, gg, (int)gg, n_scans);
     else if (blockIdx.y == 1) bucket_scan_body(e.acell, gg, (int)gg, n_scans);
-    else bucket_scan_body(e.col_off, (size_t)e.cols + 1, e.cols, n_scans);
+    else if (blockIdx.y == 2) bucket_scan_body(e.col_off, (size_t)e.cols + 1, e.cols, n_scans);
+    else if (blockIdx.x < n_scans) {
+        ScanState& s = e.st[blockIdx.x];
+        unsigned long long mn, mx;
+        orig_el_extremes(e, blockIdx.x, s.n0, s.t_min_key, s.t_max_key, mn, mx);
+        if (threadIdx.x == 0) { s.min_el_bits = mn; s.max_el_bits = mx; }
+    }
 }
 
 __global__ void __launch_bounds__(STREAM_THREADS) k_scatter_project(EngineDev e, int n_scans) {
@@ -142,6 +133,7 @@
     }
     if (p0 >= n0) return;
     const ImageGeom g = make_geom(e.rows, e.cols, e.cols, bits_dbl(s.max_el_bits), bits_dbl(s.min_el_bits));
+    const FastGeom fg = make_fast_geom(g);
     const size_t base = (size_t)b * e.P;
     int* cell = e.gcell + (size_t)b * e.G * e.G;
     int* acell = e.acell + (size_t)b * e.G * e.G;
@@ -157,15 +149,13 @@
         bool in[2];
         float4 v[2];
         unsigned lab[2];
-        double el[2], r[2];
 #pragma unroll
         for (int u = 0; u < 2; ++u) {
             p[u] = q + u * STREAM_THREADS + threadIdx.x;
             in[u] = p[u] < n0;
-            v[u] = make_float4(1.f, 0.f, 0.f, 0.f); lab[u] = 0u; col[u] = 0; el[u] = 0.0; r[u] = 0.0;
+            v[u] = make_float4(1.f, 0.f, 0.f, 0.f); lab[u] = 0u; col[u] = 0;
             if (in[u]) {
                 v[u] = __ldg(&e.xyzi[(size_t)b * e.max_points + p[u]]); lab[u] = e.label[base + p[u]]; col[u] = e.col[base + p[u]];
-                el[u] = e.el[base + p[u]]; r[u] = e.r[base + p[u]];
             }
         }
         AggTicket ta[2], tg[2], tc[2];
@@ -189,9 +179,10 @@
         for (int u = 0; u < 2; ++u) {
             int pix = -1;
             if (in[u]) {
-                const int row = bin_row(g, el[u]);
+                double r;
+                const int row = orig_row(g, fg, v[u], r);
                 if (row < 0 || row >= g.rows) set_error(s, R3D_ERR_ASSERT);
-                else { pix = row * g.cols + col[u]; atomicMin(&z[pix], dbl_bits(r[u])); }
+                else { pix = row * g.cols + col[u]; atomicMin(&z[pix], dbl_bits(r)); }
                 e.pix[base + p[u]] = pix;
             }
         }
diff --git a/pcl_augmentation_b200/csrc/r3d_k_update_project.cuh b/pcl_augmentation_b200/csrc/r3d_k_update_project.cuh
--- a/pcl_augmentation_b200/csrc/r3d_k_update_project.cuh
+++ b/pcl_augmentation_b200/csrc/r3d_k_update_project.cuh
@@ -45,8 +45,7 @@
                 if (px[u] >= 0 && pix_removed(e, b, s, px[u])) {
                     e.alive[base + p[u]] = 0;
                     if (OCC_COUNTS) adjust_map_point(e, b, s, T, p[u], -1, true);
-                    const unsigned long long bits = dbl_bits(e.el[base + p[u]]);
-                    extreme |= bits == lo || bits == hi;
+                    extreme |= orig_el_is_extreme(s, __ldg(&e.xyzi[(size_t)b * e.max_points + p[u]]), lo, hi);
                 }
         }
     }
@@ -55,7 +54,7 @@
         if (e.alive[base + p] && pix_removed(e, b, s, e.pix[base + p])) {
             e.alive[base + p] = 0;
             if (OCC_COUNTS) adjust_map_point(e, b, s, T, p, -1, true);
-            const unsigned long long bits = dbl_bits(e.el[base + p]);
+            const unsigned long long bits = dbl_bits(e.tail_el[(size_t)b * e.max_inserted + t]);
             extreme |= bits == lo || bits == hi;
         }
     }
@@ -90,6 +89,7 @@
             patch = !full;
             if (full) {
                 s.min_el_bits = R3D_EMPTY_U64; s.max_el_bits = 0ull;
+                s.t_min_key = R3D_EMPTY_U64; s.t_max_key = 0ull;
                 rect[0] = 0; rect[1] = e.rows - 1; rect[2] = 0; rect[3] = e.cols - 1;
             } else {
                 rect[0] = max(s.d_r0 - 4, 0); rect[1] = min(s.d_r1 + 4, e.rows - 1);
@@ -133,38 +133,35 @@
     }
     __syncthreads();
     if (s.apply_flag)
-        for (int p = s.n0 + s.tail_before + threadIdx.x; p < s.n0 + s.n_tail; p += UPDATE_THREADS)
-            if (e.alive[base + p]) atomicMin(&z[e.pix[base + p]], dbl_bits(e.r[base + p]));
+        for (int t = s.tail_before + threadIdx.x; t < s.n_tail; t += UPDATE_THREADS)
+            if (e.alive[base + s.n0 + t]) atomicMin(&z[e.pix[base + s.n0 + t]], dbl_bits(e.tail_r[(size_t)b * e.max_inserted + t]));
 }
 
 __global__ void __launch_bounds__(STREAM_THREADS) k_minmax(EngineDev e, int n_scans) {
-    __shared__ unsigned long long s_min[STREAM_THREADS / 32], s_max[STREAM_THREADS / 32];
     const int n_full = e.work_cnt[0];
     for (int li = blockIdx.y; li < n_full; li += gridDim.y) {
     const int b = e.full_list[li];
     ScanState& s = e.st[b];
-    const int n = s.n0 + s.n_tail;
+    const int n0 = s.n0, n = n0 + s.n_tail;
     const int p0 = blockIdx.x * CHUNK;
     if (p0 >= n) continue;
     const size_t base = (size_t)b * e.P;
+    const float4* __restrict__ src = e.xyzi + (size_t)b * e.max_points;
+    TExt te;
     unsigned long long lmin = R3D_EMPTY_U64, lmax = 0ull;
-    for (int p = p0 + threadIdx.x; p < min(p0 + CHUNK, n); p += STREAM_THREADS) {
-        if (e.alive[base + p]) {
-            const unsigned long long bits = dbl_bits(e.el[base + p]);
+    for (int q = p0; q < min(p0 + CHUNK, n); q += STREAM_THREADS) {
+        const int p = q + threadIdx.x;
+        const bool live = p < n && e.alive[base + p];
+        float4 v = make_float4(1.f, 0.f, 0.f, 0.f);
+        if (live && p < n0) v = __ldg(&src[p]);
+        t_ext_add(te, live && p < n0, v.x, v.y, v.z);
+        if (live && p >= n0) {
+            const unsigned long long bits = dbl_bits(e.tail_el[(size_t)b * e.max_inserted + (p - n0)]);
             lmin = min(lmin, bits); lmax = max(lmax, bits);
         }
     }
-    for (int o = 16; o > 0; o >>= 1) {
-        lmin = min(lmin, __shfl_xor_sync(0xffffffffu, lmin, o));
-        lmax = max(lmax, __shfl_xor_sync(0xffffffffu, lmax, o));
-    }
-    if ((threadIdx.x & 31) == 0) { s_min[threadIdx.x >> 5] = lmin; s_max[threadIdx.x >> 5] = lmax; }
-    __syncthreads();
-    if (threadIdx.x == 0) {
-        for (int w = 1; w < STREAM_THREADS / 32; ++w) { lmin = min(lmin, s_min[w]); lmax = max(lmax, s_max[w]); }
-        if (lmax >= lmin) { atomicMin(&s.min_el_bits, lmin); atomicMax(&s.max_el_bits, lmax); }
-    }
-    __syncthreads();
+    block_key_extremes<STREAM_THREADS>(te.kmin, te.kmax, &s.t_min_key, &s.t_max_key);
+    block_key_extremes<STREAM_THREADS>(lmin, lmax, &s.min_el_bits, &s.max_el_bits);
     }
 }
 
@@ -173,10 +170,15 @@
     for (int li = blockIdx.y; li < n_full; li += gridDim.y) {
         const int b = e.full_list[li];
         ScanState& s = e.st[b];
-        if (blockIdx.x == 0 && threadIdx.x == 0) {
-            e.far_arr[b] = 0;
-            if (s.min_el_bits == R3D_EMPTY_U64) { set_error(s, R3D_ERR_ASSERT); }
-            s.geom = make_geom(e.rows, e.cols, e.cols, bits_dbl(s.max_el_bits), bits_dbl(s.min_el_bits));
+        if (blockIdx.x == 0) {
+            unsigned long long mn, mx;
+            orig_el_extremes(e, b, s.n0, s.t_min_key, s.t_max_key, mn, mx);
+            if (threadIdx.x == 0) {
+                s.min_el_bits = min(s.min_el_bits, mn); s.max_el_bits = max(s.max_el_bits, mx);
+                e.far_arr[b] = 0;
+                if (s.min_el_bits == R3D_EMPTY_U64) { set_error(s, R3D_ERR_ASSERT); }
+                s.geom = make_geom(e.rows, e.cols, e.cols, bits_dbl(s.max_el_bits), bits_dbl(s.min_el_bits));
+            }
         }
         unsigned long long* z = e.zraw + (size_t)b * e.hw;
         for (int i = blockIdx.x * blockDim.x + threadIdx.x; i < e.hw; i += gridDim.x * blockDim.x) z[i] = R3D_EMPTY_U64;
@@ -192,11 +194,20 @@
     const int p0 = blockIdx.x * CHUNK;
     if (p0 >= n) continue;
     const ImageGeom g = make_geom(e.rows, e.cols, e.cols, bits_dbl(s.max_el_bits), bits_dbl(s.min_el_bits));
+    const FastGeom fg = make_fast_geom(g);
+    const int n0 = s.n0;
     const size_t base = (size_t)b * e.P;
     unsigned long long* z = e.zraw + (size_t)b * e.hw;
-    auto one = [&](bool alive, double el, unsigned col, double r) -> int {
+    auto one = [&](bool alive, int p, unsigned col) -> int {
         if (!alive) return -1;
-        const int row = bin_row(g, el);
+        double r;
+        int row;
+        if (p < n0) row = orig_row(g, fg, __ldg(&e.xyzi[(size_t)b * e.max_points + p]), r);
+        else {
+            const size_t t = (size_t)b * e.max_inserted + (p - n0);
+            r = e.tail_r[t];
+            row = bin_row(g, e.tail_el[t]);
+        }
         if (row < 0 || row >= g.rows) { set_error(s, R3D_ERR_ASSERT); return -1; }
         const int pix = row * g.cols + (int)col;
         atomicMin(&z[pix], dbl_bits(r));
@@ -209,17 +220,13 @@
         if (p + 3 < n) {
             const uchar4 a = *reinterpret_cast<const uchar4*>(e.alive + base + p);
             if (!(a.x | a.y | a.z | a.w)) continue;
-            const double2 e01 = *reinterpret_cast<const double2*>(e.el + base + p);
-            const double2 e23 = *reinterpret_cast<const double2*>(e.el + base + p + 2);
             const ushort4 c = *reinterpret_cast<const ushort4*>(e.col + base + p);
-            const double2 r01 = *reinterpret_cast<const double2*>(e.r + base + p);
-            const double2 r23 = *reinterpret_cast<const double2*>(e.r + base + p + 2);
             int4 px;
-            px.x = one(a.x, e01.x, c.x, r01.x); px.y = one(a.y, e01.y, c.y, r01.y);
-            px.z = one(a.z, e23.x, c.z, r23.x); px.w = one(a.w, e23.y, c.w, r23.y);
+            px.x = one(a.x, p, c.x); px.y = one(a.y, p + 1, c.y);
+            px.z = one(a.z, p + 2, c.z); px.w = one(a.w, p + 3, c.w);
             *reinterpret_cast<int4*>(e.pix + base + p) = px;
         } else {
-            for (int q = p; q < n; ++q) e.pix[base + q] = one(e.alive[base + q], e.el[base + q], e.col[base + q], e.r[base + q]);
+            for (int q = p; q < n; ++q) e.pix[base + q] = one(e.alive[base + q], q, e.col[base + q]);
         }
     }
     }
diff --git a/pcl_augmentation_b200/csrc/r3d_k_walk.cuh b/pcl_augmentation_b200/csrc/r3d_k_walk.cuh
--- a/pcl_augmentation_b200/csrc/r3d_k_walk.cuh
+++ b/pcl_augmentation_b200/csrc/r3d_k_walk.cuh
@@ -83,7 +83,7 @@
     ObjBox ob;
     int s_warp[WALK_NWARPS];
     int upd_full, upd_patch, rect[4];
-    unsigned long long el_min, el_max;
+    unsigned long long el_min, el_max, tk_min, tk_max;
     __align__(16) float wclip[WALK_NWARPS][8];
 };
 
@@ -167,10 +167,12 @@
 __device__ R3D_WALK_FN void walk_full_reproject(const EngineDev& e, int b, ScanState& s, WalkCtl& c) {
     const int tid = threadIdx.x, nt = blockDim.x;
     const size_t base = (size_t)b * e.P;
-    const int n = s.n0 + s.n_tail, n4 = (n + 3) >> 2;
+    const int n0 = s.n0, n = n0 + s.n_tail, n4 = (n + 3) >> 2;
     const unsigned* __restrict__ alive4 = reinterpret_cast<const unsigned*>(e.alive + base);
-    const double2* __restrict__ el2 = reinterpret_cast<const double2*>(e.el + base);
-    if (tid == 0) { c.el_min = R3D_EMPTY_U64; c.el_max = 0ull; }
+    const float4* __restrict__ src = e.xyzi + (size_t)b * e.max_points;
+    const double* __restrict__ tel = e.tail_el + (size_t)b * e.max_inserted;
+    const double* __restrict__ tr = e.tail_r + (size_t)b * e.max_inserted;
+    if (tid == 0) { c.el_min = R3D_EMPTY_U64; c.el_max = 0ull; c.tk_min = R3D_EMPTY_U64; c.tk_max = 0ull; }
     unsigned long long* z = e.zraw + (size_t)b * e.hw;
     if ((reinterpret_cast<size_t>(z) & 15) == 0) {
         ulonglong2* z2 = reinterpret_cast<ulonglong2*>(z);
@@ -180,33 +182,41 @@
         for (int i = tid; i < e.hw; i += nt) z[i] = R3D_EMPTY_U64;
     }
     __syncthreads();
+    TExt te;
+    for (int q0 = 0; q0 < n0; q0 += nt) {
+        const int p = q0 + tid;
+        const bool live = p < n0 && e.alive[base + p];
+        const float4 v = live ? __ldg(&src[p]) : make_float4(1.f, 0.f, 0.f, 0.f);
+        t_ext_add(te, live, v.x, v.y, v.z);
+    }
     unsigned long long lmin = R3D_EMPTY_U64, lmax = 0ull;
-#pragma unroll 2
-    for (int q = tid; q < n4; q += nt) {
-        const unsigned a = alive4[q];
-        if (!a) continue;
-        const double2 lo = el2[2 * q], hi = el2[2 * q + 1];
-        const double ev[4] = {lo.x, lo.y, hi.x, hi.y};
-#pragma unroll
-        for (int u = 0; u < 4; ++u)
-            if (((a >> (8 * u)) & 0xFFu) && 4 * q + u < n) { const unsigned long long bits = dbl_bits(ev[u]); lmin = min(lmin, bits); lmax = max(lmax, bits); }
-    }
+    for (int t = tid; t < s.n_tail; t += nt)
+        if (e.alive[base + n0 + t]) { const unsigned long long bits = dbl_bits(tel[t]); lmin = min(lmin, bits); lmax = max(lmax, bits); }
     for (int o = 16; o > 0; o >>= 1) {
         lmin = min(lmin, __shfl_xor_sync(0xffffffffu, lmin, o));
         lmax = max(lmax, __shfl_xor_sync(0xffffffffu, lmax, o));
-    }
-    if ((tid & 31) == 0 && lmax >= lmin) { atomicMin(&c.el_min, lmin); atomicMax(&c.el_max, lmax); }
-    __syncthreads();
-    const unsigned long long mn = c.el_min, mx = c.el_max;
+        te.kmin = min(te.kmin, __shfl_xor_sync(0xffffffffu, te.kmin, o));
+        te.kmax = max(te.kmax, __shfl_xor_sync(0xffffffffu, te.kmax, o));
+    }
+    if ((tid & 31) == 0) {
+        if (lmax >= lmin) { atomicMin(&c.el_min, lmin); atomicMax(&c.el_max, lmax); }
+        if (te.kmax >= te.kmin) { atomicMin(&c.tk_min, te.kmin); atomicMax(&c.tk_max, te.kmax); }
+    }
+    __syncthreads();
+    const unsigned long long tk_min = c.tk_min, tk_max = c.tk_max;
+    unsigned long long omn, omx;
+    orig_el_extremes(e, b, n0, tk_min, tk_max, omn, omx);
+    const unsigned long long mn = min(c.el_min, omn), mx = max(c.el_max, omx);
     if (tid == 0) {
         s.min_el_bits = mn; s.max_el_bits = mx;
+        s.t_min_key = tk_min; s.t_max_key = tk_max;
         e.far_arr[b] = 0;
         if (mn == R3D_EMPTY_U64) set_error(s, R3D_ERR_ASSERT);
         s.geom = make_geom(e.rows, e.cols, e.cols, bits_dbl(mx), bits_dbl(mn));
         atomicAdd(&e.stats[11], 1ull);
     }
     const ImageGeom g = make_geom(e.rows, e.cols, e.cols, bits_dbl(mx), bits_dbl(mn));
-    const double2* __restrict__ r2 = reinterpret_cast<const double2*>(e.r + base);
+    const FastGeom fg = make_fast_geom(g);
     const ushort4* __restrict__ col4 = reinterpret_cast<const ushort4*>(e.col + base);
     int4* pix4 = reinterpret_cast<int4*>(e.pix + base);
 #pragma unroll 2
@@ -214,17 +224,20 @@
         const unsigned a = alive4[q];
         int px[4] = {-1, -1, -1, -1};
         if (a) {
-            const double2 lo = el2[2 * q], hi = el2[2 * q + 1], rl = r2[2 * q], rh = r2[2 * q + 1];
             const ushort4 cc = col4[q];
-            const double ev[4] = {lo.x, lo.y, hi.x, hi.y}, rv[4] = {rl.x, rl.y, rh.x, rh.y};
             const int cv[4] = {cc.x, cc.y, cc.z, cc.w};
 #pragma unroll
-            for (int u = 0; u < 4; ++u)
-                if (((a >> (8 * u)) & 0xFFu) && 4 * q + u < n) {
-                    const int row = bin_row(g, ev[u]);
+            for (int u = 0; u < 4; ++u) {
+                const int p = 4 * q + u;
+                if (((a >> (8 * u)) & 0xFFu) && p < n) {
+                    double r;
+                    int row;
+                    if (p < n0) row = orig_row(g, fg, __ldg(&src[p]), r);
+                    else { r = tr[p - n0]; row = bin_row(g, tel[p - n0]); }
                     if (row < 0 || row >= g.rows) set_error(s, R3D_ERR_ASSERT);
-                    else { px[u] = row * g.cols + cv[u]; atomicMin(&z[px[u]], dbl_bits(rv[u])); }
+                    else { px[u] = row * g.cols + cv[u]; atomicMin(&z[px[u]], dbl_bits(r)); }
                 }
+            }
         }
         pix4[q] = make_int4(px[0], px[1], px[2], px[3]);
     }
@@ -292,8 +305,8 @@
         }
         __syncthreads();
         if (s.apply_flag)
-            for (int p = s.n0 + s.tail_before + tid; p < s.n0 + s.n_tail; p += nt)
-                if (e.alive[base + p]) atomicMin(&z[e.pix[base + p]], dbl_bits(e.r[base + p]));
+            for (int t = s.tail_before + tid; t < s.n_tail; t += nt)
+                if (e.alive[base + s.n0 + t]) atomicMin(&z[e.pix[base + s.n0 + t]], dbl_bits(e.tail_r[(size_t)b * e.max_inserted + t]));
     } else if (c.upd_full) {
         walk_full_reproject(e, b, s, c);
     }
@@ -795,7 +808,10 @@
         if (e.task == 1) for (int i = 0; i <= OCC_FAR_CAP; ++i) occ_far_clear(e, b, i);
         ScanState& s = e.st[b];
         s.first = 0; s.scene_changed = 0;
-        if (reset_range) { s.min_el_bits = R3D_EMPTY_U64; s.max_el_bits = 0ull; }
+        if (reset_range) {
+            s.min_el_bits = R3D_EMPTY_U64; s.max_el_bits = 0ull;
+            s.t_min_key = R3D_EMPTY_U64; s.t_max_key = 0ull;
+        }
         atomicAdd(&e.stats[0], 1ull);
     }
     if (blockIdx.x == 0 && threadIdx.x == 0) { e.work_cnt[0] = n_scans; e.work_cnt[1] = n_scans * tiles; e.stats[8] = 0ull; }
diff --git a/pcl_augmentation_b200/engine.py b/pcl_augmentation_b200/engine.py
--- a/pcl_augmentation_b200/engine.py
+++ b/pcl_augmentation_b200/engine.py
@@ -493,7 +493,7 @@
                 'patched_scans': int(out[3]), 'select_tile': int(out[4]), 'select_global': int(out[5]),
                 'prefilter_survivors': int(out[6]), 'onmap_rotations': int(out[7]), 'max_steps_per_scan': int(out[8]),
                 'candidate_windows': int(out[9]), 'exact_occlusion_counts': int(out[10]),
-                'walker_full_reprojections': int(out[11]),
+                'walker_full_reprojections': int(out[11]), 'el_window_fallbacks': int(out[12]),
                 'walker_cycles': {k: int(out[16 + i]) for i, k in enumerate(
                     ('schedule', 'update', 'setup_prefilter', 'placement', 'occlusion', 'select_insert', 'total'))},
                 'walker_detail': {k: int(out[16 + 7 + i]) for i, k in enumerate(
```
